# ElijahHyndman/PAPTeam_OpticalFlow

Hardware: AMD Instinct MI355X
Metric: Mpix/s per frame-pair (fixed SOR iters) at 1920x1080; max-abs d(u,v) vs ref (higher is better)
Workload: dtype f64

## Files before the change

papteam_opticalflow_amd/csrc/api.hip:

```cpp
#include <algorithm>
#include <chrono>
#include <cmath>
#include <cstdio>
#include <cstdlib>
#include <cstring>
#include <mutex>
#include <random>
#include <thread>

#include "common.h"
#include "flow_internal.h"

namespace papof {

namespace {
thread_local std::string g_last_error;
}

void set_last_error(const char* what, hipError_t e, const char* file, int line) {
    char buf[512];
    std::snprintf(buf, sizeof buf, "%s failed: %s (%s:%d)", what, hipGetErrorString(e), file, line);
    g_last_error = buf;
}
const char* last_error() { return g_last_error.c_str(); }
void set_last_error_text(const std::string& text) { g_last_error = text; }

static double wall() {
    return std::chrono::duration<double>(std::chrono::steady_clock::now().time_since_epoch()).count();
}

size_t arena_bytes_for(int H, int W, int C, int levels, int n_sor_max, double ratio) {
    const size_t np = (size_t)H * W;
    const int fc = (C == 3) ? 5 : (C == 1 ? 3 : C);
    size_t per_level = 0;
    {
        std::vector<Level> L;
        std::vector<PyrPlan> plan;
        if (levels >= 1 && pyramid_plan(H, W, ratio, levels, L, plan) == PAPOF_OK)
            for (const Level& l : L) per_level += ((size_t)l.w * l.h * fc * sizeof(double) + 256) * 3;
    }
    size_t sor_cells = 0, sor_cells_d = 0;
    skew_capacity(H, W, n_sor_max, sor_cells, sor_cells_d);
    size_t planes = 0;
    planes += (size_t)2 * C * 5;
    if (levels > 8) planes += (size_t)2 * C * levels;
    planes += (size_t)2 * C + 2 * C;
    planes += (size_t)7 * fc;
    planes += 8;
    planes += (size_t)3 * C + C;
    planes += (size_t)3 * fc;
    size_t bytes = planes * np * sizeof(double);
    bytes += 3 * (sor_cells + 2 * kLanes) * 16 + (sor_cells_d + 2 * kLanes) * 16 + 10 * np * sizeof(double);
    bytes += per_level + np * fc * sizeof(double);
    bytes += 8 * (std::min<size_t>(kTinyMaxCells, np) * sizeof(double) + 256);
    bytes += (size_t)64 * 4096;
    return bytes;
}

static size_t sor_scratch_bytes(int H, int W, int n_sor) {
    size_t cells = 0, cells_d = 0;
    skew_capacity(H, W, n_sor, cells, cells_d);
    return 4 * (cells + 128) * 16 + (cells_d + 128) * 16;
}

int ensure_arena(papof_handle* h, size_t bytes) {
    if (bytes <= h->arena.cap) return PAPOF_OK;
    PAPOF_HIP(hipStreamSynchronize(h->stream));
    if (h->arena.base) PAPOF_HIP(hipFree(h->arena.base));
    h->arena.base = nullptr;
    h->arena.cap = 0;
    void* p = nullptr;
    hipError_t e = hipMalloc(&p, bytes);
    if (e != hipSuccess) {
        set_last_error("hipMalloc(arena)", e, __FILE__, __LINE__);
        return PAPOF_ENOMEM;
    }
    h->arena.base = static_cast<char*>(p);
    h->arena.cap = bytes;
    return PAPOF_OK;
}

int check_params(const papof_params& P, int levels) {
    if (levels < 1) return PAPOF_EINVAL;
    if (P.n_inner < 1) return PAPOF_EINVAL;
    if (P.n_outer + 0 < 1 || P.n_sor < 1 || P.n_outer_per_level < 0 || P.n_sor_per_level < 0) return PAPOF_EINVAL;
    if (P.sor_mode < PAPOF_SOR_EXACT || P.sor_mode > PAPOF_SOR_JACOBI) return PAPOF_EINVAL;
    if (!(P.alpha > 0) || !(P.omega > 0)) return PAPOF_EINVAL;
    if (P.interpolation != PAPOF_INTERP_BILINEAR && P.interpolation != PAPOF_INTERP_BICUBIC) return PAPOF_EINVAL;
    if (P.noise_model != PAPOF_NOISE_LAPLACIAN && P.noise_model != PAPOF_NOISE_GMIXTURE) return PAPOF_EINVAL;
    return PAPOF_OK;
}

int pyramid_plan(int H, int W, double ratio, int nlev, std::vector<Level>& L, std::vector<PyrPlan>& plan) {
    if (ratio > 0.98 || ratio < 0.4) ratio = 0.75;
    const double base_sigma = 1 / ratio - 1;
    const int n = (int)(std::log(0.25) / std::log(ratio));
    const double n_sigma = base_sigma * n;
    L.assign(nlev, Level{});
    plan.assign(nlev, PyrPlan{});
    L[0].w = W;
    L[0].h = H;
    for (int i = 1; i < nlev; i++) {
        PyrPlan p;
        if (i <= n) {
            p.src_level = 0;
            p.sigma = base_sigma * i;
            p.fsize = (int)(p.sigma * 3);
            p.rate = std::pow(ratio, i);
        } else {
            p.src_level = i - n;
            p.sigma = n_sigma;
            p.fsize = (int)(n_sigma * 3);
            p.rate = (double)std::pow(ratio, i) * W / L[i - n].w;
        }
        p.sw = L[p.src_level].w;
        p.sh = L[p.src_level].h;
        if (p.fsize > kMaxFsize) return PAPOF_EINVAL;
        L[i].w = (int)((double)p.sw * p.rate);
        L[i].h = (int)((double)p.sh * p.rate);
        if (L[i].w < 1 || L[i].h < 1) return PAPOF_EINVAL;
        plan[i] = p;
    }
    return PAPOF_OK;
}

int smooth_and_resize(papof_handle* h, const double* src, double* dst, double* tmp_a, double* tmp_b, const PyrPlan& p, int C,
                      int dh, int dw) {
    const Taps g = gaussian_taps(p.sigma, p.fsize);
    if (g.fsize == 0 && g.t[0] == 1.0) return resize(h, src, dst, p.sh, p.sw, C, dh, dw, p.rate, p.rate, false, 0.0);
    PAPOF_TRY(filter_hv(h, src, tmp_b, tmp_a, p.sh, p.sw, C, g, g));
    return resize(h, tmp_b, dst, p.sh, p.sw, C, dh, dw, p.rate, p.rate, false, 0.0);
}

int reduce_init(papof_handle* h, const papof_tensor* a, const papof_tensor* b, int pairs_a, int pairs_b, int H, int W,
                const std::vector<Level>& L, const std::vector<PyrPlan>& plan, double ratio, double* X, double* Y, double* T,
                size_t t_planes, double*& out) {
    const size_t np0 = (size_t)H * W;
    const int planes = 2 * (pairs_a + pairs_b), levels = (int)L.size();
    double* const parts[2] = {X, X + (size_t)pairs_a * 2 * np0};
    const papof_tensor* const src[2] = {a, b};
    const int n[2] = {pairs_a, pairs_b};
    for (int i = 0; i < 2; i++) {
        if (n[i] == 0) continue;
        if (src[i])
            PAPOF_TRY(ingest_frames(h, *src[i], nullptr, parts[i], H, W, 2, n[i]));
        else
            PAPOF_HIP(hipMemsetAsync(parts[i], 0, (size_t)n[i] * 2 * np0 * sizeof(double), h->stream));
    }
    PAPOF_TRY(init_sanitize(h, X, (size_t)planes * np0));
    out = X;
    if (levels == 1) return PAPOF_OK;
    std::vector<int> chain;
    for (int i = levels - 1; i > 0; i = plan[i].src_level) chain.insert(chain.begin(), i);
    double s = 1.0;
    for (int i = 1; i < levels; i++) s *= ratio;
    double *cur = X, *other = Y;
    for (const int i : chain) {
        const PyrPlan& p = plan[i];
        const bool last = i == levels - 1;
        const Taps g = gaussian_taps(p.sigma, p.fsize);
        if (g.fsize == 0 && g.t[0] == 1.0) {
            PAPOF_TRY(resize(h, cur, other, p.sh, p.sw, planes, L[i].h, L[i].w, p.rate, p.rate, last, last ? s : 0.0));
            std::swap(cur, other);
            continue;
        }
        const size_t ns = (size_t)p.sw * p.sh;
        const int chunk = filter_hv_needs_tmp(g, g) ? (int)std::min<size_t>((size_t)planes, t_planes * np0 / ns) : planes;
        if (chunk < 1) return PAPOF_EINVAL;
        for (int c0 = 0; c0 < planes; c0 += chunk)
            PAPOF_TRY(filter_hv(h, cur + c0 * ns, other + c0 * ns, T, p.sh, p.sw, std::min(chunk, planes - c0), g, g));
        PAPOF_TRY(resize(h, other, cur, p.sh, p.sw, planes, L[i].h, L[i].w, p.rate, p.rate, last, last ? s : 0.0));
    }
    out = cur;
    return PAPOF_OK;
}

int build_pyramid(papof_handle* h, const std::vector<Level>& L, const std::vector<PyrPlan>& plan, int C, bool second,
                  double* tmp_a, double* tmp_b) {
    for (size_t i = 1; i < L.size(); i++) {
        const PyrPlan& p = plan[i];
        const double* src = second ? L[p.src_level].p2 : L[p.src_level].p1;
        double* dst = second ? L[i].p2 : L[i].p1;
        PAPOF_TRY(smooth_and_resize(h, src, dst, tmp_a, tmp_b, p, C, L[i].h, L[i].w));
    }
    return PAPOF_OK;
}

struct SolveBuffers {
    double *im1s, *tmp, *blend, *imdt, *phi;
    SorPlanes sp;
    SorPlanes sp_tiny{};
    double *bgx = nullptr, *bgy = nullptr, *bgxy = nullptr;
    double *gm = nullptr, *gm_scratch = nullptr;
};

int alloc_solve_buffers(Arena& A, int H, int W, int fc, int mode, int n_sor_cap, SolveBuffers& B) {
    const size_t np = (size_t)H * W;
    B.im1s = A.f64(np * fc);
    B.tmp = A.f64(np * fc);
    B.blend = A.f64(np * fc);
    B.imdt = A.f64(np * fc);
    B.phi = A.f64(np);
    PAPOF_TRY(sor_alloc_planes(A, H, W, mode, n_sor_cap, B.sp));
    if (mode == PAPOF_SOR_EXACT)
        PAPOF_TRY(sor_alloc_tiny_planes(A, std::min<size_t>(kTinyMaxCells, (size_t)H * W), B.sp_tiny));
    return A.overflow ? PAPOF_ENOMEM : PAPOF_OK;
}

int alloc_branch_buffers(papof_handle* h, Arena& A, int H, int W, int fc, int interpolation, int noise_model,
                         SolveBuffers& B) {
    const size_t np = (size_t)H * W;
    if (interpolation == PAPOF_INTERP_BICUBIC) {
        B.bgx = A.f64(np * fc);
        B.bgy = A.f64(np * fc);
        B.bgxy = A.f64(np * fc);
    }
    if (noise_model == PAPOF_NOISE_GMIXTURE) {
        B.gm = A.f64(5 * 8);
        B.gm_scratch = A.f64((size_t)gm_scratch_doubles());
        if (A.overflow || fc > 8) return fc > 8 ? PAPOF_EINVAL : PAPOF_ENOMEM;
        double init[40];
        for (int k = 0; k < fc; k++) {
            init[k] = 0.95;
            init[fc + k] = 0.05;
            init[2 * fc + k] = 0.5;
            init[3 * fc + k] = 0.05 * 0.05;
            init[4 * fc + k] = 0.5 * 0.5;
        }
        PAPOF_HIP(hipMemcpyAsync(B.gm, init, sizeof(double) * 5 * fc, hipMemcpyHostToDevice, h->stream));
        PAPOF_HIP(hipStreamSynchronize(h->stream));
    }
    return A.overflow ? PAPOF_ENOMEM : PAPOF_OK;
}

int bicubic_planes(papof_handle* h, const double* f2, int H, int W, int fc, SolveBuffers& B) {
    PAPOF_TRY(central3_planes(h, f2, B.bgx, B.bgy, B.bgxy, H, W, fc));
    return PAPOF_OK;
}

struct LapGuard {
    bool on = false;
    bool exact = false;
    bool collect = false;
    bool nz_known = false;
    unsigned* flags = nullptr;
    double* lap = nullptr;
    double* scratch = nullptr;
    unsigned epoch = 0;
    int slot = 0;
    std::vector<int> slot_level, slot_channels;
    unsigned* wit(int s) const { return on && collect && s >= 0 && s < kLapMaxSlots ? flags + lap_wit_word(s) : nullptr; }
    unsigned* nz(int level) const { return on && collect && nz_known ? flags + lap_nz_word(level) : nullptr; }
    const double* guard() const { return on && exact ? lap : nullptr; }
    int unknown(const unsigned* host_flags) const {
        if (!on || !collect) return 0;
        if (slot > kLapMaxSlots) return 1;
        int n = 0;
        for (int s = 0; s + 1 < slot; s++)
            for (int c = 0; c < slot_channels[s]; c++) {
                const unsigned w = host_flags[lap_wit_word(s) + c];
                const bool witness = w == epoch || w == (epoch ^ kLapNone);
                const bool all_zero = nz_known && host_flags[lap_nz_word(slot_level[s]) + c] != epoch;
                n += !(witness || all_zero);
                if (!(witness || all_zero) && std::getenv("PAPOF_LAP_TRACE"))
                    std::fprintf(stderr, "[lap guard] no proof: slot %d of %d, level %d, channel %d\n", s, slot, slot_level[s], c);
            }
        return n;
    }
};

int smooth_flow(papof_handle* h, const double* f1, const double* f2, double* warp, double*& u, double*& v, double*& ua,
                double*& va, int H, int W, int fc, double alpha, int n_outer, int n_inner, int n_sor, double omega,
                int mode, SolveBuffers& B, PhaseClock& clk, const double* im1s_ready = nullptr,
                bool final_warp = true, unsigned* prog = nullptr, size_t prog_per_solve = 0, double* out_u = nullptr,
                double* out_v = nullptr, bool fold_warp = false, LapGuard* lg = nullptr, int level = 0) {
    const Taps g = smooth5_taps();
    int solve_idx = 0;
    const bool tiny = mode == PAPOF_SOR_EXACT && B.sp_tiny.phi && sor_tiny_fits(h, H, W, n_sor);
    SorPlanes& SP = tiny ? B.sp_tiny : B.sp;
    const double* im1s = im1s_ready;
    if (!im1s) {
        clk.phase(PAPOF_T_PHASE1_GENERATE);
        PAPOF_TRY(filter_hv(h, f1, B.im1s, B.tmp, H, W, fc, g, g));
        im1s = B.im1s;
    }
    const char* const fused_sw = std::getenv("PAPOF_FUSED_SYSTEM");
    const bool fused_env = !(fused_sw && fused_sw[0] == '0');
    const bool fused_system = fused_env && fold_warp && n_inner == 1 && !B.gm && (fc == 5 || fc == 3) &&
                              !(lg && lg->guard()) && !(lg && lg->on && lap_one_block_level(H, W));
    for (int count = 0; count < n_outer; count++) {
        clk.phase(fused_system ? kTimerFused : (int)PAPOF_T_PHASE1_GENERATE);
        if (fused_system)
            PAPOF_TRY(flow_system(h, f1, f2, u, v, im1s, H, W, fc, alpha, omega, SP,
                                  lg && count > 0 ? lg->wit(lg->slot - 1) : nullptr));
        else if (fold_warp)
            PAPOF_TRY(warp_smooth_blend(h, f1, f2, u, v, im1s, B.blend, B.imdt, H, W, fc,
                                        lg && count > 0 && !B.gm ? lg->wit(lg->slot - 1) : nullptr,
                                        B.phi));
        else
            PAPOF_TRY(smooth_hv_blend(h, warp, im1s, B.blend, B.imdt, H, W, fc));
        for (int hh = 0; hh < n_inner; hh++) {
            const SorPlanes* prev = hh == 0 ? nullptr : &SP;
            if ((count == 0 && !fold_warp) || hh > 0) {
                clk.phase(PAPOF_T_PHASE2_DERIVATIVES);
                PAPOF_TRY(compute_phi(h, u, v, prev, B.phi, H, W));
            }
            if (!fused_system) clk.phase(PAPOF_T_PHASE4_LINEARSYSTEM);
            if (!fused_system)
                PAPOF_TRY(assemble_system(h, B.blend, B.imdt, B.phi, u, v, H, W, fc, alpha, omega, SP, nullptr, nullptr,
                                          prev, nullptr, B.gm, lg ? lg->guard() : nullptr));
            h->sor_mark = [](void* c, int on) {
                static_cast<PhaseClock*>(c)->phase(on ? PAPOF_T_PHASE5_SOR : PAPOF_T_PHASE6_UPDATE);
            };
            h->sor_mark_ctx = &clk;
            h->sor_prog_next = prog ? prog + (size_t)solve_idx * prog_per_solve : nullptr;
            solve_idx++;
            const int rc_solve = sor_solve(h, SP, H, W, alpha, omega, n_sor, mode);
            h->sor_prog_next = nullptr;
            h->sor_mark = nullptr;
            h->sor_mark_ctx = nullptr;
            PAPOF_TRY(rc_solve);
        }
        double* const phi_next = count + 1 < n_outer && !fold_warp ? B.phi : nullptr;
        const bool rewarp = !fold_warp && !B.bgx && (final_warp || count + 1 < n_outer || B.gm);
        const bool wit_later = fold_warp && count + 1 < n_outer;
        const bool wit_small = fold_warp && !wit_later && lap_one_block_level(H, W);
        unsigned* const wit = lg && !B.gm && !B.bgx && !wit_later && !wit_small ? lg->wit(lg->slot) : nullptr;
        if (out_u && out_v && count + 1 == n_outer) {
            PAPOF_TRY(update_warp_phi(h, SP, u, v, out_u, out_v, f1, f2, warp, phi_next, H, W, fc, rewarp, 0, -1, wit));
            u = out_u;
            v = out_v;
        } else {
            PAPOF_TRY(update_warp_phi(h, SP, u, v, ua, va, f1, f2, warp, phi_next, H, W, fc, rewarp, 0, -1, wit));
            std::swap(u, ua);
            std::swap(v, va);
        }
        if (B.bgx)
            PAPOF_TRY(bicubic_warp(h, f1, f2, B.bgx, B.bgy, B.bgxy, u, v, warp, H, W, fc, nullptr, true, true));
        if (lg && lg->on && !B.gm && wit_small && lg->wit(lg->slot))
            PAPOF_TRY(lap_small_check(h, f1, f2, u, v, H, W, fc, lg->wit(lg->slot)));
        if (lg && lg->on && !B.gm) {
            lg->slot_level.push_back(level);
            lg->slot_channels.push_back(fc);
            lg->slot++;
            if (lg->exact) {
                if (B.bgx)
                    PAPOF_TRY(est_laplacian_noise(h, f1, warp, nullptr, nullptr, H, W, fc, lg->lap, lg->scratch));
                else
                    PAPOF_TRY(est_laplacian_noise(h, f1, f2, u, v, H, W, fc, lg->lap, lg->scratch));
            }
        }
        if (B.gm) PAPOF_TRY(est_gaussian_mixture(h, f1, warp, H, W, fc, B.gm, B.gm_scratch));
    }
    clk.phase(-1);
    return PAPOF_OK;
}

int feature_channels(int C) { return C == 3 ? 5 : (C == 1 ? 3 : C); }

struct FrameIn {
    const void* d;
    bool u8;
    bool planar = false;
};
int load_frame(papof_handle* h, const FrameIn& f, double* planar, int H, int W, int C) {
    if (f.planar) {
        PAPOF_HIP(hipMemcpyAsync(planar, f.d, (size_t)H * W * C * sizeof(double), hipMemcpyDeviceToDevice, h->stream));
        return PAPOF_OK;
    }
    if (f.u8) return hwc_u8_to_planar(h, static_cast<const unsigned char*>(f.d), planar, H, W, C);
    return hwc_to_planar(h, static_cast<const double*>(f.d), planar, H, W, C);
}

enum SeqOp { kPair, kSeqPrime, kSeqNext };

bool seq_matches(const papof_handle* h, int H, int W, int C, int levels, double ratio, size_t need) {
    const papof_handle::Seq& q = h->seq;
    return q.valid && q.h == H && q.w == W && q.c == C && q.levels == levels && q.ratio == ratio &&
           q.arena_base == h->arena.base && need <= h->arena.cap;
}

int flow_pass(papof_handle* h, const FrameIn& fa, const FrameIn& fb, SeqOp op, int H, int W, int C, int levels,
              const papof_params& P, double* d_vx, double* d_vy, double* d_warp, double* timing, LapGuard* lg,
              const papof_tensor* init = nullptr) {
    const double t_entry = wall();
    PAPOF_TRY(check_params(P, levels));
    double ratio = P.ratio;
    if (ratio > 0.98 || ratio < 0.4) ratio = 0.75;
    std::vector<Level> L;
    std::vector<PyrPlan> plan;
    PAPOF_TRY(pyramid_plan(H, W, P.ratio, levels, L, plan));
    const int n_sor_max = P.n_sor + (levels - 1) * P.n_sor_per_level;
    const size_t need = arena_bytes_for(H, W, C, levels, n_sor_max, P.ratio);
    if (op == kSeqNext && !seq_matches(h, H, W, C, levels, ratio, need)) {
        g_last_error = "sequence push does not continue the primed sequence (shape, levels, ratio or arena changed)";
        return PAPOF_EINVAL;
    }
    const int slot1 = op == kSeqNext ? h->seq.slot : 0;
    h->seq.valid = false;
    PAPOF_TRY(ensure_arena(h, need));
    Arena& A = h->arena;
    A.off = 0;
    A.overflow = false;
    h->events_used = 0;
    const size_t np0 = (size_t)H * W;
    const int fc = feature_channels(C);
    double tm[PAPOF_N_TIMERS + 1];
    std::memset(tm, 0, sizeof tm);
    const size_t tm_bytes = PAPOF_N_TIMERS * sizeof(double);
    const auto keep_seq = [&](int slot) {
        h->seq.valid = true;
        h->seq.h = H;
        h->seq.w = W;
        h->seq.c = C;
        h->seq.levels = levels;
        h->seq.ratio = ratio;
        h->seq.slot = slot;
        h->seq.arena_base = A.base;
    };
    PhaseClock clk{h, true};
    PhaseClock pclk{h, true};
    PhaseClock total{h, true};
    clk.only_sor = pclk.only_sor = (!h->phase_events && P.phase_timing == 0) || P.phase_timing == 2;
    h->sor_launches = 0;
    h->sor_log.clear();
    clk.stamps = true;
    h->stamps_used = 0;
    h->next_stamp = nullptr;
    h->stamp_stream = h->stream;

    total.phase(PAPOF_T_TOTAL);
    for (int i = 0; i < levels; i++) {
        double* slot[2];
        slot[0] = A.f64((size_t)L[i].w * L[i].h * C);
        slot[1] = A.f64((size_t)L[i].w * L[i].h * C);
        L[i].p1 = slot[slot1];
        L[i].p2 = slot[slot1 ^ 1];
    }
    double* tmp_a = A.f64(np0 * C);
    double* tmp_b = A.f64(np0 * C);
    if (A.overflow) return PAPOF_ENOMEM;
    if (op == kSeqPrime) {
        PAPOF_TRY(load_frame(h, fa, L[0].p1, H, W, C));
        PAPOF_TRY(build_pyramid(h, L, plan, C, false, tmp_a, tmp_b));
        PAPOF_HIP(hipStreamSynchronize(h->stream));
        keep_seq(slot1);
        if (timing) std::memset(timing, 0, tm_bytes);
        return PAPOF_OK;
    }

    std::vector<double*> F1(levels), F2(levels), S1(levels);
    for (int k = 0; k < levels; k++) {
        const size_t n = (size_t)L[k].w * L[k].h * fc;
        F1[k] = A.f64(n);
        F2[k] = A.f64(n);
        S1[k] = A.f64(n);
    }
    double* prep_tmp = A.f64(np0 * fc);
    double* gx = A.f64(np0 * C);
    double* gy = A.f64(np0 * C);
    double* gxy = A.f64(np0 * C);
    double* warp = A.f64(np0 * fc);
    double* u = A.f64(2 * np0);
    double* v = u ? u + np0 : nullptr;
    double* u2 = A.f64(2 * np0);
    double* v2 = u2 ? u2 + np0 : nullptr;
    SolveBuffers B;
    {
        const int rc_alloc = alloc_solve_buffers(A, H, W, fc, P.sor_mode, n_sor_max, B);
        if (rc_alloc != PAPOF_OK || A.overflow) return rc_alloc != PAPOF_OK ? rc_alloc : PAPOF_ENOMEM;
    }
    PAPOF_TRY(alloc_branch_buffers(h, A, H, W, fc, P.interpolation, P.noise_model, B));

    struct LevelCounters {
        size_t prog_off = 0, prog_per = 0;
    };
    std::vector<LevelCounters> LP(levels);
    size_t prog_total = 0;
    const bool exact = P.sor_mode == PAPOF_SOR_EXACT;
    if (exact) {
        for (int k = 0; k < levels; k++) {
            LP[k].prog_per = sor_counters_words(L[k].h, L[k].w, P.n_sor + k * P.n_sor_per_level);
            LP[k].prog_off = prog_total;
            prog_total += LP[k].prog_per * (size_t)((P.n_outer + k * P.n_outer_per_level) * P.n_inner);
        }
        PAPOF_TRY(sor_counters_ensure(h, prog_total));
    }

    const bool overlap = h->overlap_prep && P.phase_timing != 1 && h->prep_stream != nullptr;
    hipStream_t const main_stream = h->stream, prep = overlap ? h->prep_stream : h->stream;
    while (h->sync_events.size() < (size_t)levels + 2) {
        hipEvent_t e;
        PAPOF_HIP(hipEventCreateWithFlags(&e, hipEventDisableTiming));
        h->sync_events.push_back(e);
    }
    struct StreamSwap {
        papof_handle* h;
        hipStream_t saved;
        StreamSwap(papof_handle* hh, hipStream_t s) : h(hh), saved(hh->stream) { h->stream = s; }
        ~StreamSwap() { h->stream = saved; }
    };
    bool from_level0 = true;
    for (int i = 1; i < levels; i++) from_level0 = from_level0 && plan[i].src_level == 0;
    const Taps g5 = smooth5_taps();
    const auto build_level = [&](int i, int second) -> int {
        if (i == 0) return PAPOF_OK;
        const PyrPlan& q = plan[i];
        const double* src = second ? L[q.src_level].p2 : L[q.src_level].p1;
        double* dst = second ? L[i].p2 : L[i].p1;
        return smooth_and_resize(h, src, dst, tmp_a, tmp_b, q, C, L[i].h, L[i].w);
    };
    const auto prepare = [&]() -> int {
        StreamSwap on_prep(h, prep);
        pclk.phase(PAPOF_T_ALLOCATION);
        if (exact && !sor_counters_clear(h, 0, prog_total)) return PAPOF_EDEVICE;
        pclk.phase(PAPOF_T_CONSTRUCTION);
        if (op != kSeqNext) PAPOF_TRY(load_frame(h, fa, L[0].p1, H, W, C));
        PAPOF_TRY(load_frame(h, fb, L[0].p2, H, W, C));
        const int first = op == kSeqNext ? 1 : 0;
        if (!from_level0)
            for (int i = 1; i < levels; i++)
                for (int second = first; second < 2; second++) PAPOF_TRY(build_level(i, second));
        for (int k = levels - 1; k >= 0; k--) {
            if (from_level0) {
                pclk.phase(PAPOF_T_CONSTRUCTION);
                for (int second = first; second < 2; second++) PAPOF_TRY(build_level(k, second));
            }
            pclk.phase(PAPOF_T_ALLOCATION);
            PAPOF_TRY(im2feature(h, L[k].p1, F1[k], L[k].h, L[k].w, C, lg ? lg->nz(k) : nullptr));
            PAPOF_TRY(im2feature(h, L[k].p2, F2[k], L[k].h, L[k].w, C, lg ? lg->nz(k) : nullptr));
            pclk.phase(PAPOF_T_PHASE1_GENERATE);
            PAPOF_TRY(filter_hv(h, F1[k], S1[k], prep_tmp, L[k].h, L[k].w, fc, g5, g5));
            pclk.phase(-1);
            if (overlap) PAPOF_HIP(hipEventRecord(h->sync_events[k], prep));
        }
        pclk.phase(PAPOF_T_POSTPROCESSING);
        PAPOF_TRY(central3_planes(h, L[0].p2, gx, gy, gxy, H, W, C));
        pclk.phase(-1);
        if (overlap) PAPOF_HIP(hipEventRecord(h->sync_events[levels], prep));
        return PAPOF_OK;
    };
    papof_handle::HostIO& io = h->hostio;
    const bool hostio = io.active && overlap && h->copy_stream && h->copy_events.size() >= 8;
    const auto prepare_hostio = [&]() -> int {
        StreamSwap on_prep(h, prep);
        hipStream_t const cs = h->copy_stream;
        pclk.phase(PAPOF_T_ALLOCATION);
        if (exact && !sor_counters_clear(h, 0, prog_total)) return PAPOF_EDEVICE;
        if (io.im1) {
            PAPOF_HIP(hipMemcpyAsync(const_cast<void*>(fa.d), io.im1, io.nb_in, hipMemcpyHostToDevice, cs));
            PAPOF_HIP(hipEventRecord(h->copy_events[0], cs));
            PAPOF_HIP(hipStreamWaitEvent(prep, h->copy_events[0], 0));
        }
        pclk.phase(PAPOF_T_CONSTRUCTION);
        if (op != kSeqNext) {
            PAPOF_TRY(load_frame(h, fa, L[0].p1, H, W, C));
            for (int i = 1; i < levels; i++) PAPOF_TRY(build_level(i, 0));
        }
        for (int k = levels - 1; k >= 0; k--) {
            pclk.phase(PAPOF_T_ALLOCATION);
            PAPOF_TRY(im2feature(h, L[k].p1, F1[k], L[k].h, L[k].w, C, lg ? lg->nz(k) : nullptr));
            pclk.phase(PAPOF_T_PHASE1_GENERATE);
            PAPOF_TRY(filter_hv(h, F1[k], S1[k], prep_tmp, L[k].h, L[k].w, fc, g5, g5));
        }
        pclk.phase(-1);
        if (io.im2) {
            PAPOF_HIP(hipMemcpyAsync(const_cast<void*>(fb.d), io.im2, io.nb_in, hipMemcpyHostToDevice, cs));
            PAPOF_HIP(hipEventRecord(h->copy_events[1], cs));
            PAPOF_HIP(hipStreamWaitEvent(prep, h->copy_events[1], 0));
        }
        pclk.phase(PAPOF_T_CONSTRUCTION);
        PAPOF_TRY(load_frame(h, fb, L[0].p2, H, W, C));
        if (!from_level0)
            for (int i = 1; i < levels; i++) PAPOF_TRY(build_level(i, 1));
        for (int k = levels - 1; k >= 0; k--) {
            if (from_level0) {
                pclk.phase(PAPOF_T_CONSTRUCTION);
                PAPOF_TRY(build_level(k, 1));
            }
            pclk.phase(PAPOF_T_ALLOCATION);
            PAPOF_TRY(im2feature(h, L[k].p2, F2[k], L[k].h, L[k].w, C, lg ? lg->nz(k) : nullptr));
            pclk.phase(-1);
            PAPOF_HIP(hipEventRecord(h->sync_events[k], prep));
        }
        pclk.phase(PAPOF_T_POSTPROCESSING);
        PAPOF_TRY(central3_planes(h, L[0].p2, gx, gy, gxy, H, W, C));
        pclk.phase(-1);
        PAPOF_HIP(hipEventRecord(h->sync_events[levels], prep));
        return PAPOF_OK;
    };
    if (io.active && !hostio) {
        if (io.im1) PAPOF_HIP(hipMemcpyAsync(const_cast<void*>(fa.d), io.im1, io.nb_in, hipMemcpyHostToDevice, main_stream));
        if (io.im2) PAPOF_HIP(hipMemcpyAsync(const_cast<void*>(fb.d), io.im2, io.nb_in, hipMemcpyHostToDevice, main_stream));
    }
    if (overlap) {
        PAPOF_HIP(hipEventRecord(h->sync_events[levels + 1], main_stream));
        PAPOF_HIP(hipStreamWaitEvent(prep, h->sync_events[levels + 1], 0));
    }
    {
        const int rc = hostio ? prepare_hostio() : prepare();
        if (rc != PAPOF_OK) {
            if (overlap) hipStreamSynchronize(prep);
            return rc;
        }
    }

    int pw = 0, ph = 0;
    const auto solve_levels = [&]() -> int {
        if (lg && lg->guard())
            PAPOF_HIP(hipMemcpyAsync(lg->lap, h->lap_init_dev, 8 * sizeof(double), hipMemcpyDeviceToDevice, main_stream));
        for (int k = levels - 1; k >= 0; k--) {
            const int lw = L[k].w, lh = L[k].h;
            const size_t np = (size_t)lw * lh;
            clk.phase(-1);
            if (overlap) PAPOF_HIP(hipStreamWaitEvent(main_stream, h->sync_events[k], 0));
            clk.phase(PAPOF_T_ALLOCATION);
            const double *f1 = F1[k], *f2 = F2[k];
            const int n_sor_k = P.n_sor + k * P.n_sor_per_level, n_outer_k = P.n_outer + k * P.n_outer_per_level;
            unsigned* prog_k = nullptr;
            if (exact) prog_k = h->sync_words + 32 + LP[k].prog_off;
            const bool tiny_k = exact && sor_tiny_fits(h, lh, lw, n_sor_k);
            if (!tiny_k) PAPOF_TRY(sor_bind(h, B.sp, lh, lw, n_sor_k));
            double* const out_u = k == 0 ? d_vx : nullptr;
            double* const out_v = k == 0 ? d_vy : nullptr;
            const bool fold_warp = !B.bgx && !B.gm;
            if (k == levels - 1 && init) {
                double* r = nullptr;
                PAPOF_TRY(reduce_init(h, init, nullptr, 1, 0, H, W, L, plan, ratio, u, u2, warp, (size_t)fc, r));
                if (r != u) std::swap(u, u2);
                v = u + np;
                v2 = u2 + np;
                if (B.bgx) {
                    PAPOF_TRY(bicubic_planes(h, f2, lh, lw, fc, B));
                    PAPOF_TRY(bicubic_warp(h, f1, f2, B.bgx, B.bgy, B.bgxy, u, v, warp, lh, lw, fc, nullptr, true, false));
                } else if (!fold_warp) {
                    PAPOF_TRY(warp_bilinear(h, f1, f2, u, v, warp, lh, lw, fc));
                }
            } else if (k == levels - 1) {
                v = u + np;
                v2 = u2 + np;
                PAPOF_HIP(hipMemsetAsync(u, 0, 2 * np * sizeof(double), h->stream));
                if (!fold_warp)
                    PAPOF_HIP(hipMemcpyAsync(warp, f2, np * fc * sizeof(double), hipMemcpyDeviceToDevice, h->stream));
                if (B.bgx) PAPOF_TRY(bicubic_planes(h, f2, lh, lw, fc, B));
            } else {
                const double xr = (double)lw / pw, yr = (double)lh / ph, inv = 1 / ratio;
                PAPOF_TRY(resize(h, u, u2, ph, pw, 2, lh, lw, xr, yr, true, inv));
                std::swap(u, u2);
                v = u + np;
                v2 = u2 + np;
                if (B.bgx) {
                    PAPOF_TRY(bicubic_planes(h, f2, lh, lw, fc, B));
                    PAPOF_TRY(bicubic_warp(h, f1, f2, B.bgx, B.bgy, B.bgxy, u, v, warp, lh, lw, fc, nullptr, true, false));
                } else if (!fold_warp) {
                    PAPOF_TRY(warp_bilinear(h, f1, f2, u, v, warp, lh, lw, fc));
                }
            }
            if (!tiny_k) PAPOF_TRY(sor_reset_planes(h, B.sp));
            PAPOF_TRY(smooth_flow(h, f1, f2, warp, u, v, u2, v2, lh, lw, fc, P.alpha, n_outer_k, P.n_inner, n_sor_k, P.omega,
                                  P.sor_mode, B, clk, S1[k], false, prog_k, exact ? LP[k].prog_per : 0, out_u, out_v,
                                  fold_warp, lg, k));
            pw = lw;
            ph = lh;
        }
        clk.phase(-1);
        if (overlap) PAPOF_HIP(hipStreamWaitEvent(main_stream, h->sync_events[levels], 0));
        clk.phase(PAPOF_T_POSTPROCESSING);
        if (hostio && io.early_out && u == d_vx && v == d_vy) {
            hipStream_t const cs = h->copy_stream;
            PAPOF_HIP(hipEventRecord(h->copy_events[2], main_stream));
            PAPOF_HIP(hipStreamWaitEvent(cs, h->copy_events[2], 0));
            PAPOF_HIP(hipMemcpyAsync(io.vx, d_vx, io.nb_flow, hipMemcpyDeviceToHost, cs));
            PAPOF_HIP(hipMemcpyAsync(io.vy, d_vy, io.nb_flow, hipMemcpyDeviceToHost, cs));
            constexpr int kChunks = 4;
            for (int q = 0; q < kChunks; q++) {
                const Rect rc{0, (int)((long long)H * q / kChunks), W, (int)((long long)H * (q + 1) / kChunks)};
                if (rc.empty()) continue;
                PAPOF_TRY(bicubic_warp(h, L[0].p1, L[0].p2, gx, gy, gxy, u, v, d_warp, H, W, C, &rc));
                PAPOF_HIP(hipEventRecord(h->copy_events[3 + q], main_stream));
                PAPOF_HIP(hipStreamWaitEvent(cs, h->copy_events[3 + q], 0));
                const size_t off = (size_t)rc.y0 * W * C, cnt = (size_t)rc.h() * W * C;
                PAPOF_HIP(hipMemcpyAsync(io.warp + off, d_warp + off, cnt * sizeof(double), hipMemcpyDeviceToHost, cs));
            }
            io.out_issued = true;
            return PAPOF_OK;
        }
        PAPOF_TRY(bicubic_warp(h, L[0].p1, L[0].p2, gx, gy, gxy, u, v, d_warp, H, W, C));
        if (u != d_vx) PAPOF_HIP(hipMemcpyAsync(d_vx, u, np0 * sizeof(double), hipMemcpyDeviceToDevice, h->stream));
        if (v != d_vy) PAPOF_HIP(hipMemcpyAsync(d_vy, v, np0 * sizeof(double), hipMemcpyDeviceToDevice, h->stream));
        return PAPOF_OK;
    };
    const int rc_main = solve_levels();
    if (rc_main != PAPOF_OK) {
        hipStreamSynchronize(main_stream);
        if (overlap) hipStreamSynchronize(prep);
        return rc_main;
    }
    clk.phase(-1);
    PAPOF_TRY(stamp_only(h));
    total.phase(-1);
    h->stamps_fetched = 0;
    {
        const bool flags = lg && lg->on && lg->collect;
        const size_t first = flags ? lap_wit_word(std::min(lg->slot, kLapMaxSlots) - 1) : kLapFlagWords;
        const size_t bytes = (kLapFlagWords - first) * sizeof(unsigned) + (size_t)h->stamps_used * sizeof(unsigned long long);
        if (bytes > 0)
            PAPOF_HIP(hipMemcpyAsync(h->lap_flags_host + first, h->lap_flags_dev + first, bytes, hipMemcpyDeviceToHost, h->stream));
        h->stamps_fetched = h->stamps_used;
    }
    const double t_enqueued = wall();
    PAPOF_HIP(hipStreamSynchronize(h->stream));
    h->host_enqueue_sec = t_enqueued - t_entry;
    h->host_wait_sec = wall() - t_enqueued;
    h->next_stamp = nullptr;
    if (P.sor_mode == PAPOF_SOR_EXACT) PAPOF_TRY(sor_check(h));
    if (clk.err != PAPOF_OK || pclk.err != PAPOF_OK || total.err != PAPOF_OK) return PAPOF_EDEVICE;
    clk.collect(tm);
    pclk.collect(tm);
    total.collect(tm);
    if (clk.sor_span_sec.size() == h->sor_log.size())
        for (size_t i = 0; i < h->sor_log.size(); i++) h->sor_log[i].sec = clk.sor_span_sec[i];
    {
        constexpr double kPsiShare = 0.3;
        const double fused = tm[PAPOF_T_PHASE4_LINEARSYSTEM];
        tm[PAPOF_T_PHASE3_PSIDATA] += kPsiShare * fused;
        tm[PAPOF_T_PHASE4_LINEARSYSTEM] = fused - kPsiShare * fused;
    }
    {
        constexpr double kPhiShare = 0.04;
        const double fused = tm[PAPOF_T_PHASE1_GENERATE];
        tm[PAPOF_T_PHASE2_DERIVATIVES] += kPhiShare * fused;
        tm[PAPOF_T_PHASE1_GENERATE] = fused - kPhiShare * fused;
    }
    {
        const double f = tm[kTimerFused];
        tm[PAPOF_T_PHASE1_GENERATE] += 0.51 * f;
        tm[PAPOF_T_PHASE2_DERIVATIVES] += 0.02 * f;
        tm[PAPOF_T_PHASE3_PSIDATA] += 0.14 * f;
        tm[PAPOF_T_PHASE4_LINEARSYSTEM] += f - 0.51 * f - 0.02 * f - 0.14 * f;
    }
    if (timing) std::memcpy(timing, tm, tm_bytes);
    if (op == kSeqNext) keep_seq(slot1 ^ 1);
    return PAPOF_OK;
}

int flow_device(papof_handle* h, const FrameIn& fa, const FrameIn& fb, SeqOp op, int H, int W, int C, int levels,
                const papof_params& P, double* d_vx, double* d_vy, double* d_warp, double* timing,
                const papof_tensor* init = nullptr) {
    LapGuard lg;
    const int fc = feature_channels(C);
    lg.on = h->lap_guard && op != kSeqPrime && P.noise_model == PAPOF_NOISE_LAPLACIAN && fc <= 8 && levels >= 1 &&
            h->lap_flags_dev != nullptr;
    if (!lg.on) return flow_pass(h, fa, fb, op, H, W, C, levels, P, d_vx, d_vy, d_warp, timing, nullptr, init);
    lg.flags = h->lap_flags_dev;
    lg.lap = h->lap_dev;
    lg.scratch = h->lap_scratch_dev;
    lg.nz_known = (C == 1 || C == 3) && (size_t)levels * 8 <= (size_t)kLapNzWords;
    const bool always_exact = P.interpolation == PAPOF_INTERP_BICUBIC;
    lg.collect = !always_exact;
    lg.exact = always_exact || h->lap_exact;
    const papof_handle::Seq seq0 = h->seq;
    double first_pass_total = 0.0;
    for (int pass = 0; pass < 2; pass++) {
        if (++h->lap_epoch >= kLapNone) {
            PAPOF_HIP(hipMemsetAsync(h->lap_flags_dev, 0, kLapFlagWords * sizeof(unsigned), h->stream));
            h->lap_epoch = 1u;
        }
        lg.epoch = h->lap_epoch;
        lg.slot = 0;
        lg.slot_level.clear();
        lg.slot_channels.clear();
        PAPOF_TRY(flow_pass(h, fa, fb, op, H, W, C, levels, P, d_vx, d_vy, d_warp, timing, &lg, init));
        if (pass == 1 && timing) timing[PAPOF_T_TOTAL] += first_pass_total;
        if (!lg.collect) return PAPOF_OK;
        const int unknown = lg.unknown(h->lap_flags_host);
        if (lg.exact) {
            if (pass == 0) h->lap_exact_calls++;
            h->lap_exact = unknown > 0;
            return PAPOF_OK;
        }
        if (unknown == 0) return PAPOF_OK;
        h->lap_reruns++;
        lg.exact = true;
        if (timing) first_pass_total = timing[PAPOF_T_TOTAL];
        if (h->copy_stream) PAPOF_HIP(hipStreamSynchronize(h->copy_stream));
        h->seq = seq0;
        h->hostio.im1 = nullptr;
        h->hostio.im2 = nullptr;
    }
    return PAPOF_OK;
}

int flow_device_planar(papof_handle* h, const double* f1, const double* f2, int H, int W, int C, int levels,
                       const papof_params& P, double* d_vx, double* d_vy, double* d_warp, double* timing,
                       const papof_tensor* init) {
    FrameIn a{f1, false}, b{f2, false};
    a.planar = b.planar = true;
    return flow_device(h, a, b, kPair, H, W, C, levels, P, d_vx, d_vy, d_warp, timing, init);
}

}

using namespace papof;

extern "C" {

int papof_version(void) { return PAPOF_VERSION; }

void papof_default_params(papof_params* p) {
    if (!p) return;
    p->alpha = 0.012;
    p->ratio = 0.75;
    p->n_outer = 7;
    p->n_outer_per_level = 1;
    p->n_inner = 1;
    p->n_sor = 30;
    p->n_sor_per_level = 3;
    p->omega = 1.8;
    p->sor_mode = PAPOF_SOR_EXACT;
    p->phase_timing = 0;
    p->interpolation = PAPOF_INTERP_BILINEAR;
    p->noise_model = PAPOF_NOISE_LAPLACIAN;
}

const char* papof_strerror(int code) {
    switch (code) {
        case PAPOF_OK: return "ok";
        case PAPOF_EINVAL: return "invalid argument";
        case PAPOF_ENODEVICE: return "no usable gfx950 device";
        case PAPOF_ENOMEM: return "out of memory";
        case PAPOF_EDEVICE: return "HIP runtime error";
        case PAPOF_ETIMEOUT: return "device-side wait timed out";
    }
    return "unknown error";
}

const char* papof_last_error(void) { return last_error(); }

const char* papof_timing_key(int i) {
    static const char* keys[PAPOF_N_TIMERS] = {"Allocation",         "Construction",        "Phase1_Generate",
// ... 43 lines not shown
        set_last_error("hipStreamCreate", e, __FILE__, __LINE__);
        papof_destroy(h);
        return PAPOF_ENODEVICE;
    }
    if (const char* cs = std::getenv("PAPOF_OVERLAP")) h->overlap_prep = std::atoi(cs) != 0;
    if (const char* cs = std::getenv("PAPOF_PHASE_EVENTS")) h->phase_events = std::atoi(cs) != 0;
    if (const char* cs = std::getenv("PAPOF_SOR_DEPTH")) h->sor_depth = std::max(4, std::atoi(cs));
    if (const char* cs = std::getenv("PAPOF_SOR_FUSE")) h->sor_fuse = std::max(1, std::atoi(cs));
    if (const char* cs = std::getenv("PAPOF_SOR_TINY")) h->sor_tiny = std::atoi(cs) != 0;
    if (const char* cs = std::getenv("PAPOF_SOR_GROUP")) h->sor_group = std::max(1, std::atoi(cs));
    if (const char* cs = std::getenv("PAPOF_SOR_XCD")) h->sor_xcd_affine = std::atoi(cs);
    if (const char* cs = std::getenv("PAPOF_RB_DEPTH")) h->rb_depth = std::max(0, std::atoi(cs));
    if (const char* cs = std::getenv("PAPOF_RB_SHAPE")) h->rb_shape = std::max(0, std::atoi(cs));
    if (const char* cs = std::getenv("PAPOF_SOR_RESIDENT")) h->sor_resident = std::max(0, std::atoi(cs));
    if (const char* cs = std::getenv("PAPOF_SOR_DEAD")) h->sor_skip_dead = std::atoi(cs) != 0 ? 1 : 0;
    int rc = sor_probe_dpp(h);
    if (rc != PAPOF_OK) {
        papof_destroy(h);
        return rc;
    }
    {
        const size_t flag_bytes = kLapFlagWords * sizeof(unsigned), bytes = flag_bytes + 4096 * sizeof(unsigned long long);
        const size_t lap_doubles = 16 + (size_t)lap_scratch_doubles();
        std::vector<double> init(8, 0.02);
        if (hipMalloc((void**)&h->lap_flags_dev, bytes) == hipSuccess &&
            hipHostMalloc((void**)&h->lap_flags_host, bytes, hipHostMallocDefault) == hipSuccess &&
            hipMalloc((void**)&h->lap_dev, lap_doubles * sizeof(double)) == hipSuccess &&
            hipMemset(h->lap_flags_dev, 0, flag_bytes) == hipSuccess &&
            hipMemcpy(h->lap_dev + 8, init.data(), 8 * sizeof(double), hipMemcpyHostToDevice) == hipSuccess) {
            h->stamps_dev = reinterpret_cast<unsigned long long*>(h->lap_flags_dev + kLapFlagWords);
            h->stamps = reinterpret_cast<unsigned long long*>(h->lap_flags_host + kLapFlagWords);
            h->stamps_cap = 4096;
            h->lap_init_dev = h->lap_dev + 8;
            h->lap_scratch_dev = h->lap_dev + 16;
            std::memset(h->lap_flags_host, 0, bytes);
        } else {
            g_last_error = "cannot allocate the flag / stamp block of the handle";
            papof_destroy(h);
            return PAPOF_ENOMEM;
        }
        const char* lgv = std::getenv("PAPOF_LAP_GUARD");
        h->lap_guard = !(lgv && lgv[0] == '0');
    }
    *out = h;
    return PAPOF_OK;
}

void papof_destroy(papof_handle* h) {
    if (!h) return;
    hipSetDevice(h->device);
    hipStreamSynchronize(h->stream);
    if (h->prep_stream) hipStreamSynchronize(h->prep_stream);
    for (hipEvent_t e : h->events) hipEventDestroy(e);
    for (hipEvent_t e : h->sync_events) hipEventDestroy(e);
    if (h->prep_stream) hipStreamDestroy(h->prep_stream);
    if (h->copy_stream) {
        hipStreamSynchronize(h->copy_stream);
        hipStreamDestroy(h->copy_stream);
    }
    for (hipEvent_t e : h->copy_events) hipEventDestroy(e);
    if (h->arena.base) hipFree(h->arena.base);
    if (h->sync_words) hipFree(h->sync_words);
    if (h->stage_dev) hipFree(h->stage_dev);
    if (h->tensor_scratch) hipFree(h->tensor_scratch);
    if (h->init_flag_dev) hipFree(h->init_flag_dev);
    if (h->entry_event) hipEventDestroy(h->entry_event);
    if (h->lap_flags_host) hipHostFree(h->lap_flags_host);
    if (h->lap_flags_dev) hipFree(h->lap_flags_dev);
    if (h->lap_dev) hipFree(h->lap_dev);
    hipStreamDestroy(h->stream);
    delete h;
}

void* papof_stream(papof_handle* h) { return h ? (void*)h->stream : nullptr; }

int papof_host_alloc(size_t bytes, void** out) {
    if (!out) return PAPOF_EINVAL;
    *out = nullptr;
    hipError_t e = hipHostMalloc(out, bytes ? bytes : 1, hipHostMallocDefault);
    if (e != hipSuccess) {
        set_last_error("hipHostMalloc", e, __FILE__, __LINE__);
        *out = nullptr;
        return e == hipErrorNoDevice || e == hipErrorInvalidDevice ? PAPOF_ENODEVICE : PAPOF_ENOMEM;
    }
    return PAPOF_OK;
}

int papof_host_free(void* p) {
    if (!p) return PAPOF_OK;
    PAPOF_HIP(hipHostFree(p));
    return PAPOF_OK;
}

int papof_dev_alloc(papof_handle* h, size_t bytes, void** out) {
    if (!h || !out) return PAPOF_EINVAL;
    PAPOF_HIP(hipSetDevice(h->device));
    hipError_t e = hipMalloc(out, bytes ? bytes : 1);
    if (e != hipSuccess) {
        set_last_error("hipMalloc", e, __FILE__, __LINE__);
        return PAPOF_ENOMEM;
    }
    return PAPOF_OK;
}

int papof_dev_free(papof_handle* h, void* p) {
    if (!h) return PAPOF_EINVAL;
    PAPOF_HIP(hipSetDevice(h->device));
    PAPOF_HIP(hipFree(p));
    return PAPOF_OK;
}

int papof_dev_upload(papof_handle* h, void* dst, const void* src, size_t bytes) {
    if (!h || !dst || !src) return PAPOF_EINVAL;
    PAPOF_HIP(hipSetDevice(h->device));
    PAPOF_HIP(hipMemcpyAsync(dst, src, bytes, hipMemcpyHostToDevice, h->stream));
    PAPOF_HIP(hipStreamSynchronize(h->stream));
    return PAPOF_OK;
}

int papof_dev_download(papof_handle* h, void* dst, const void* src, size_t bytes) {
    if (!h || !dst || !src) return PAPOF_EINVAL;
    PAPOF_HIP(hipSetDevice(h->device));
    PAPOF_HIP(hipMemcpyAsync(dst, src, bytes, hipMemcpyDeviceToHost, h->stream));
    PAPOF_HIP(hipStreamSynchronize(h->stream));
    return PAPOF_OK;
}

namespace {

int device_call(papof_handle* h, const FrameIn& fa, const FrameIn& fb, SeqOp op, int height, int width, int c,
                int pyramid_levels, const papof_params* params, double* d_vx, double* d_vy, double* d_warpI2,
                double* timing_sec) {
    if (!h || height < 1 || width < 1 || c < 1) return PAPOF_EINVAL;
    if (op != kSeqNext && !fa.d) return PAPOF_EINVAL;
    if (op != kSeqPrime && (!fb.d || !d_vx || !d_vy || !d_warpI2)) return PAPOF_EINVAL;
    papof_params P;
    if (params)
        P = *params;
    else
        papof_default_params(&P);
    PAPOF_HIP(hipSetDevice(h->device));
    return flow_device(h, fa, fb, op, height, width, c, pyramid_levels, P, d_vx, d_vy, d_warpI2, timing_sec);
}

SeqOp seq_op_for(papof_handle* h, int H, int W, int C, int levels, const papof_params* params) {
    papof_params P;
    if (params)
        P = *params;
    else
        papof_default_params(&P);
    double ratio = P.ratio;
    if (ratio > 0.98 || ratio < 0.4) ratio = 0.75;
    if (levels < 1) return kSeqPrime;
    const size_t need = arena_bytes_for(H, W, C, levels, P.n_sor + (levels - 1) * P.n_sor_per_level, P.ratio);
    return seq_matches(h, H, W, C, levels, ratio, need) ? kSeqNext : kSeqPrime;
}

}

int papof_flow_device(papof_handle* h, const double* d_im1, const double* d_im2, int height, int width, int c,
                      int pyramid_levels, const papof_params* params, double* d_vx, double* d_vy, double* d_warpI2,
                      double timing_sec[PAPOF_N_TIMERS]) {
    return device_call(h, FrameIn{d_im1, false}, FrameIn{d_im2, false}, kPair, height, width, c, pyramid_levels,
                       params, d_vx, d_vy, d_warpI2, timing_sec);
}

int papof_flow_device_u8(papof_handle* h, const unsigned char* d_im1, const unsigned char* d_im2, int height,
                         int width, int c, int pyramid_levels, const papof_params* params, double* d_vx,
                         double* d_vy, double* d_warpI2, double timing_sec[PAPOF_N_TIMERS]) {
    return device_call(h, FrameIn{d_im1, true}, FrameIn{d_im2, true}, kPair, height, width, c, pyramid_levels, params,
                       d_vx, d_vy, d_warpI2, timing_sec);
}

int papof_set_stream_overlap(papof_handle* h, int on) {
    if (!h) return PAPOF_EINVAL;
    h->overlap_prep = on != 0;
    return PAPOF_OK;
}

int papof_seq_reset(papof_handle* h) {
    if (!h) return PAPOF_EINVAL;
    h->seq.valid = false;
    return PAPOF_OK;
}

int papof_seq_push_device(papof_handle* h, const void* d_frame, int is_u8, int height, int width, int c,
                          int pyramid_levels, const papof_params* params, double* d_vx, double* d_vy,
                          double* d_warpI2, double timing_sec[PAPOF_N_TIMERS], int* have_flow) {
    if (!h || !d_frame || !have_flow) return PAPOF_EINVAL;
    *have_flow = 0;
    const SeqOp op = seq_op_for(h, height, width, c, pyramid_levels, params);
    const FrameIn f{d_frame, is_u8 != 0};
    PAPOF_TRY(device_call(h, f, f, op, height, width, c, pyramid_levels, params, d_vx, d_vy, d_warpI2, timing_sec));
    *have_flow = op == kSeqNext ? 1 : 0;
    return PAPOF_OK;
}

namespace {

int ensure_host_stage(papof_handle* h, size_t dev_bytes) {
    if (dev_bytes > h->stage_dev_bytes) {
        PAPOF_HIP(hipStreamSynchronize(h->stream));
        if (h->stage_dev) PAPOF_HIP(hipFree(h->stage_dev));
        h->stage_dev = nullptr;
        h->stage_dev_bytes = 0;
        hipError_t e = hipMalloc((void**)&h->stage_dev, dev_bytes);
        if (e != hipSuccess) {
            set_last_error("hipMalloc(stage)", e, __FILE__, __LINE__);
            return PAPOF_ENOMEM;
        }
        h->stage_dev_bytes = dev_bytes;
    }
    return PAPOF_OK;
}

int flow_host(papof_handle* h, const void* im1, const void* im2, bool u8, SeqOp op, int height, int width, int c,
              int pyramid_levels, const papof_params* params, double* vx, double* vy, double* warpI2,
              double* timing_sec) {
    if (!h || height < 1 || width < 1 || c < 1 || pyramid_levels < 1) return PAPOF_EINVAL;
    if (op != kSeqNext && !im1) return PAPOF_EINVAL;
    if (op != kSeqPrime && (!im2 || !vx || !vy || !warpI2)) return PAPOF_EINVAL;
    const double t0 = wall();
    PAPOF_HIP(hipSetDevice(h->device));
    const size_t np = (size_t)height * width, nb_img = np * c * sizeof(double), nb_flow = np * sizeof(double);
    const size_t nb_in = np * c * (u8 ? 1 : sizeof(double));
    PAPOF_TRY(ensure_host_stage(h, 3 * nb_img + 2 * nb_flow));
    double* d1 = h->stage_dev;
    double* d2 = d1 + np * c;
    double* dw = d2 + np * c;
    double* dx = dw + np * c;
    double* dy = dx + np;
    double tm[PAPOF_N_TIMERS];
    std::memset(tm, 0, sizeof tm);
    bool use_io = op != kSeqPrime && h->overlap_prep && h->prep_stream;
    if (use_io && !h->copy_stream) {
        if (hipStreamCreateWithFlags(&h->copy_stream, hipStreamNonBlocking) != hipSuccess) h->copy_stream = nullptr;
        while (h->copy_stream && h->copy_events.size() < 8) {
            hipEvent_t e = nullptr;
            if (hipEventCreateWithFlags(&e, hipEventDisableTiming) != hipSuccess) break;
            h->copy_events.push_back(e);
        }
    }
    use_io = use_io && h->copy_stream && h->copy_events.size() >= 8;
    if (use_io) {
        papof_params Pq;
        if (params)
            Pq = *params;
        else
            papof_default_params(&Pq);
        use_io = Pq.phase_timing != 1;
    }
    if (use_io) {
        h->hostio = papof_handle::HostIO{};
        h->hostio.active = true;
        h->hostio.im1 = op != kSeqNext ? im1 : nullptr;
        h->hostio.im2 = im2;
        h->hostio.nb_in = nb_in;
    } else {
        if (op != kSeqNext) PAPOF_HIP(hipMemcpyAsync(d1, im1, nb_in, hipMemcpyHostToDevice, h->stream));
        if (op != kSeqPrime) PAPOF_HIP(hipMemcpyAsync(d2, im2, nb_in, hipMemcpyHostToDevice, h->stream));
    }
    const auto is_pinned = [](const void* p) {
        hipPointerAttribute_t a;
        if (hipPointerGetAttributes(&a, p) != hipSuccess) {
            (void)hipGetLastError();
            return false;
        }
        return a.type == hipMemoryTypeHost;
    };
    std::thread prefault;
    const bool out_pinned = op != kSeqPrime && is_pinned(warpI2) && is_pinned(vx) && is_pinned(vy);
    if (use_io) {
        h->hostio.vx = vx;
        h->hostio.vy = vy;
        h->hostio.warp = warpI2;
        h->hostio.nb_flow = nb_flow;
        h->hostio.nb_img = nb_img;
        h->hostio.early_out = out_pinned;
    }
    if (op != kSeqPrime && np * sizeof(double) >= (size_t(1) << 20) && !out_pinned)
        prefault = std::thread([=] {
            const auto touch = [](double* p, size_t bytes) {
                volatile char* q = reinterpret_cast<volatile char*>(p);
                for (size_t o = 0; o < bytes; o += 4096) q[o] = 0;
                if (bytes) q[bytes - 1] = 0;
            };
            touch(warpI2, nb_img);
            touch(vx, nb_flow);
            touch(vy, nb_flow);
        });
    const int rc_dev = device_call(h, FrameIn{d1, u8}, FrameIn{d2, u8}, op, height, width, c, pyramid_levels, params, dx,
                                   dy, dw, tm);
    const bool out_issued = use_io && h->hostio.out_issued;
    h->hostio.active = false;
    if (use_io && h->copy_stream && hipStreamSynchronize(h->copy_stream) != hipSuccess && rc_dev == PAPOF_OK) {
        if (prefault.joinable()) prefault.join();
        return PAPOF_EDEVICE;
    }
    if (prefault.joinable()) prefault.join();
    PAPOF_TRY(rc_dev);
    if (out_issued) {
        if (timing_sec) {
            tm[PAPOF_T_TOTAL] = wall() - t0;
            std::memcpy(timing_sec, tm, sizeof tm);
        }
        return PAPOF_OK;
    }
// ... 732 lines not shown
```

papteam_opticalflow_amd/csrc/common.h:

```cpp
#pragma once
#include <cstdlib>

#include <hip/hip_runtime.h>

#include <algorithm>
#include <cmath>
#include <cstddef>
#include <cstdint>
#include <initializer_list>
#include <string>
#include <vector>

#include "../../include/papof.h"

namespace papof {

constexpr int kLanes = 64;
constexpr int kMaxFsize = 8;

struct Rect {
    int x0, y0, x1, y1;
    __host__ __device__ bool empty() const { return x1 <= x0 || y1 <= y0; }
    __host__ __device__ int w() const { return x1 - x0; }
    __host__ __device__ int h() const { return y1 - y0; }
// ... 17 lines not shown
    const double *a = im1 + o, *b = im2 + o;
    im1 = back ? b : a;
    im2 = back ? a : b;
    return back ? o + bk.fr : o;
}

struct Taps {
    double t[2 * kMaxFsize + 1];
    int fsize;
};

void set_last_error(const char* what, hipError_t e, const char* file, int line);
const char* last_error();

#define PAPOF_HIP(expr)                                              \
    do {                                                             \
        hipError_t _e = (expr);                                      \
        if (_e != hipSuccess) {                                      \
            ::papof::set_last_error(#expr, _e, __FILE__, __LINE__);  \
            return PAPOF_EDEVICE;                                    \
        }                                                            \
    } while (0)

#define PAPOF_TRY(expr)              \
    do {                             \
        int _rc = (expr);            \
        if (_rc != PAPOF_OK) return _rc; \
    } while (0)

struct Arena {
    char* base = nullptr;
    size_t cap = 0, off = 0, peak = 0;
    bool overflow = false;
    void* alloc(size_t bytes) {
        size_t o = (off + 255) & ~size_t(255);
        if (o + bytes > cap) {
            overflow = true;
            return nullptr;
        }
        off = o + bytes;
        if (off > peak) peak = off;
        return base + o;
    }
    double* f64(size_t n) { return static_cast<double*>(alloc(n * sizeof(double))); }
    size_t mark() const { return off; }
    void release(size_t m) { off = m; }
};

constexpr int kLapNzWords = 32 * 8, kLapMaxSlots = 1024;
constexpr size_t kLapFlagWords = (size_t)kLapMaxSlots * 8 + kLapNzWords;
inline size_t lap_wit_word(int slot) { return (size_t)(kLapMaxSlots - 1 - slot) * 8; }
inline size_t lap_nz_word(int level) { return (size_t)kLapMaxSlots * 8 + (size_t)level * 8; }
constexpr unsigned kLapNone = 0x80000000u;
constexpr int kSorMaxDepth = 32;
constexpr int kBandRows = kLanes - 2;

struct SkewDims {
    int nb;
    int ns;
    int rt, qt;
    int hp;
    int npos;
    size_t n;
    int n_sor;
    int npos_d;
    size_t nd;
    int group;
    int dpar;
    size_t nh;
    int fuse;
    int band_rows, koff, poff;
};
constexpr int kFusedRows = kLanes - 3;
inline SkewDims skew_dims(int h, int w, int n_sor, int group = 1, int fuse = 1) {
    SkewDims d;
    d.fuse = (fuse == 2 && group <= 1) ? 2 : 1;
    d.group = d.fuse == 2 ? 1 : (group < 1 ? 1 : group);
    d.ns = w + kLanes - 1;
    d.n_sor = n_sor;
    d.npos_d = d.ns + 2 * kSorMaxDepth + 72;
    if (d.fuse == 2) {
        const int last = (n_sor + 1) / 2 - 1;
        d.band_rows = kFusedRows;
        d.nb = (h + 2 * last + 1 + kFusedRows - 1) / kFusedRows;
        d.qt = n_sor + 3;
        d.rt = (d.qt + 7) / 8 * 8;
        d.hp = (d.rt + kFusedRows * d.nb + 4 + 7) / 8 * 8;
        d.npos = d.qt + d.ns + 2 * kSorMaxDepth + 2 + kFusedRows * (d.nb - 1) + 2;
        d.dpar = last & 1;
        d.koff = 2 * last + 1;
        d.poff = 3;
        d.nh = 0;
    } else {
        d.band_rows = kBandRows;
        d.nb = (h + n_sor - 1 + kBandRows - 1) / kBandRows;
        d.qt = n_sor + 1;
        d.rt = (d.qt + 7) / 8 * 8;
        d.hp = (d.rt + kBandRows * d.nb + 2 + 7) / 8 * 8;
        d.npos = d.qt + d.ns + 2 * kSorMaxDepth + 2 + kBandRows * (d.nb - 1) + 2;
        d.dpar = d.group == 1 ? ((n_sor - 1) & 1) : (((n_sor + d.group - 1) / d.group - 1) & 1);
        d.koff = n_sor - 1;
        d.poff = 1;
        d.nh = d.group == 1 ? 0 : (size_t)n_sor * d.nb * d.npos_d;
    }
    d.n = (size_t)d.npos * d.hp;
    d.nd = (size_t)2 * d.npos_d * d.nb * kLanes;
    return d;
}
inline void skew_capacity(int h, int w, int n_sor, size_t& cells, size_t& cells_d) {
    const SkewDims a = skew_dims(h, w, n_sor, 2), b = skew_dims(h, w, n_sor, 1, 2);
    cells = a.n > b.n ? a.n : b.n;
    cells_d = (a.nd + a.nh) > (b.nd + b.nh) ? (a.nd + a.nh) : (b.nd + b.nh);
}

struct SorPlanes {
    double *phi, *xy, *a1, *a2, *b1, *b2;
    double *du, *dv;
    double *du2, *dv2;
    bool skew;
    SkewDims sd;
    size_t cap_cells, cap_cells_d;
};

}

struct papof_handle {
    int device = 0;
    hipStream_t stream = nullptr;
    papof::Arena arena;
    unsigned* sync_words = nullptr;
    size_t sync_cap = 0;
    std::vector<hipEvent_t> events;
    size_t events_used = 0;
    int cu_count = 0;
    double* stage_dev = nullptr;
    size_t stage_dev_bytes = 0;
    double* tensor_scratch = nullptr;
    size_t tensor_scratch_bytes = 0;
    hipEvent_t entry_event = nullptr;
    unsigned* init_flag_dev = nullptr;
    bool use_dpp = false;
    int sor_depth = 0;
    unsigned long long* sor_dbg = nullptr;
    void (*sor_mark)(void*, int) = nullptr;
    void* sor_mark_ctx = nullptr;
    int sor_fuse = 0;
    int sor_group = 0;
    int rb_depth = 0;
    int rb_shape = 0;
    int sor_tiny = 1;
    int sor_resident = 0;
    int sor_skip_dead = 1;
    unsigned* sor_prog_next = nullptr;
    int sor_launches = 0;
    struct SorSolveLog {
        int H, W, n_sor, kind, depth, launches;
        double sec;
    };
    std::vector<SorSolveLog> sor_log;
    hipStream_t prep_stream = nullptr;
    unsigned* lap_flags_dev = nullptr;
    unsigned* lap_flags_host = nullptr;
    double* lap_dev = nullptr;
    double* lap_init_dev = nullptr;
    double* lap_scratch_dev = nullptr;
    bool lap_guard = true;
    bool lap_exact = false;
    unsigned lap_epoch = 0;
    int lap_reruns = 0, lap_exact_calls = 0;
    double host_enqueue_sec = 0.0, host_wait_sec = 0.0;
    struct HostIO {
        bool active = false;
        const void *im1 = nullptr, *im2 = nullptr;
        size_t nb_in = 0;
        double *vx = nullptr, *vy = nullptr, *warp = nullptr;
        size_t nb_flow = 0, nb_img = 0;
        bool early_out = false;
        bool out_issued = false;
    } hostio;
    hipStream_t copy_stream = nullptr;
    std::vector<hipEvent_t> copy_events;
    std::vector<hipEvent_t> sync_events;
    bool overlap_prep = true;
    unsigned long long* stamps_dev = nullptr;
    unsigned long long* stamps = nullptr;
    int stamps_cap = 0, stamps_used = 0, stamps_fetched = 0;
    unsigned long long* next_stamp = nullptr;
    hipStream_t stamp_stream = nullptr;
    bool phase_events = true;
    int sor_xcd_affine = 1;
    struct Seq {
        bool valid = false;
        int h = 0, w = 0, c = 0, levels = 0, slot = 0;
        double ratio = 0;
        const char* arena_base = nullptr;
    } seq;
};

namespace papof {

inline unsigned long long* take_stamp(papof_handle* h) {
    if (h->stamp_stream && h->stream != h->stamp_stream) return nullptr;
    unsigned long long* s = h->next_stamp;
    h->next_stamp = nullptr;
    return s;
}
int stamp_only(papof_handle* h);

inline bool described(const papof_tensor* t, std::initializer_list<int> dtypes, std::initializer_list<int> axes, bool positive) {
    if (!t || !t->data || std::find(dtypes.begin(), dtypes.end(), t->dtype) == dtypes.end()) return false;
    for (int i : axes)
        if (t->stride[i] < 0 || (positive && t->stride[i] == 0)) return false;
    return true;
}
inline bool valid_alphas(double a1, double a2) { return std::isfinite(a1) && std::isfinite(a2) && a1 >= 0 && a2 >= 0; }
inline long long dtype_bytes(int dtype) { return dtype == PAPOF_DTYPE_U8 ? 1 : dtype == PAPOF_DTYPE_F32 ? 4 : 8; }

int hwc_to_planar(papof_handle* h, const double* hwc, double* planar, int H, int W, int C, int frames = 1);
int hwc_u8_to_planar(papof_handle* h, const unsigned char* hwc, double* planar, int H, int W, int C, int frames = 1);
int planar_to_hwc(papof_handle* h, const double* planar, double* hwc, int H, int W, int C);
int ingest_frames(papof_handle* h, const papof_tensor& a, const papof_tensor* b, double* planar, int H, int W, int C,
                  int frames);
int emit_outputs(papof_handle* h, const double* src, const papof_tensor& dst, bool comp_major, int H, int W, int K, int pairs);
int init_check(papof_handle* h, const papof_tensor& t, int pairs, int H, int W, unsigned* flag);
int init_sanitize(papof_handle* h, double* planar, size_t n);
int fb_check(papof_handle* h, hipStream_t st, const papof_tensor& fw, const papof_tensor& bw, const papof_tensor& mask,
             int pairs, int H, int W, double a1, double a2);
int filter_h(papof_handle* h, const double* src, double* dst, int H, int W, int planes, const Taps& f,
             const Rect* rc = nullptr);
int filter_v(papof_handle* h, const double* src, double* dst, int H, int W, int planes, const Taps& f,
             const Rect* rc = nullptr);
int filter_hv(papof_handle* h, const double* src, double* dst, double* tmp, int H, int W, int planes, const Taps& fh,
              const Taps& fv);
bool filter_hv_needs_tmp(const Taps& fh, const Taps& fv);
int resize(papof_handle* h, const double* src, double* dst, int sh, int sw, int planes, int dh, int dw, double xr,
           double yr, bool use_post, double post, const Rect* rc = nullptr);
int im2feature(papof_handle* h, const double* im, double* feat, int H, int W, int C, unsigned* nz = nullptr, int frames = 1,
               size_t nz_stride = 0);
int central3_planes(papof_handle* h, const double* src, double* gx, double* gy, double* gxy, int H, int W, int planes);
int warp_bilinear(papof_handle* h, const double* im1, const double* im2, const double* vx, const double* vy,
                  double* out, int H, int W, int planes, const Rect* rc = nullptr);
int smooth_v_blend(papof_handle* h, const double* tmp, const double* im1s, double* blend, double* imdt, int H,
                   int W, int planes, const Rect* rc = nullptr);
int smooth_hv_blend(papof_handle* h, const double* warp, const double* im1s, double* blend, double* imdt, int H,
                    int W, int planes, int row0 = 0, int row1 = -1);
int warp_smooth_blend(papof_handle* h, const double* im1, const double* im2, const double* u, const double* v,
                      const double* im1s, double* blend, double* imdt, int H, int W, int planes, unsigned* wit = nullptr,
                      double* phi_out = nullptr);
int compute_phi(papof_handle* h, const double* u, const double* v, const SorPlanes* prev, double* phi, int H, int W,
                const Rect* rc = nullptr);
int assemble_system(papof_handle* h, const double* blend, const double* imdt, const double* phi, const double* u,
                    const double* v, int H, int W, int planes, double alpha, double omega, const SorPlanes& out,
                    double* opt_imdx2, double* opt_imdy2, const SorPlanes* prev, const Rect* rc = nullptr,
                    const double* gm = nullptr, const double* lap = nullptr);
int flow_system(papof_handle* h, const double* im1, const double* im2, const double* u, const double* v, const double* im1s,
                int H, int W, int planes, double alpha, double omega, const SorPlanes& out, unsigned* wit = nullptr,
                int row0 = 0, int row1 = -1,
                int batch = 1, const BatchK* bk = nullptr);
int lap_scratch_doubles();
int lap_rows_check(papof_handle* h, const double* im1, const double* im2, const double* u, const double* v, int H, int W,
                   int C, int r0, int r1, unsigned* wit, unsigned* val, unsigned mark);
bool lap_one_block_level(int H, int W);
int lap_small_check(papof_handle* h, const double* im1, const double* im2, const double* u, const double* v, int H, int W,
                    int C, unsigned* wit, int batch = 1, const BatchK* bk = nullptr);
int est_laplacian_noise(papof_handle* h, const double* im1, const double* im2, const double* u, const double* v, int H,
                        int W, int C, double* lap, double* scratch);
int gm_scratch_doubles();
int est_gaussian_mixture(papof_handle* h, const double* im1, const double* im2, int H, int W, int C, double* gm,
                         double* scratch);
int laplacian(papof_handle* h, const double* in, const double* weight, double* out, int H, int W);
int update_and_warp(papof_handle* h, const SorPlanes& sp, double* u, double* v, const double* im1,
                    const double* im2, double* warp, int H, int W, int planes, bool do_warp = true);
int bicubic_warp(papof_handle* h, const double* im1, const double* im2, const double* gx, const double* gy,
                 const double* gxy, const double* vx, const double* vy, double* out_hwc, int H, int W, int C,
                 const Rect* rc = nullptr, bool planar_out = false, bool clamp = true, int batch = 1, const BatchK* bk = nullptr);
int flow_quantize16(papof_handle* h, const double* vx, const double* vy, unsigned short* q, size_t n);
int flow_dequantize16(papof_handle* h, const unsigned short* q, double* vx, double* vy, size_t n);
int flow_to_bgr(papof_handle* h, const double* vx, const double* vy, size_t n, double* partial, unsigned char* bgr);
int update_warp_phi(papof_handle* h, const SorPlanes& sp, const double* u, const double* v, double* u_out, double* v_out,
                    const double* im1, const double* im2, double* warp, double* phi_out, int H, int W, int planes,
                    bool do_warp = true, int row0 = 0, int row1 = -1, unsigned* wit = nullptr, int batch = 1,
                    const BatchK* bk = nullptr);
int update_flow(papof_handle* h, const SorPlanes& sp, double* u, double* v, int H, int W, const Rect& r);
int sor_prep(papof_handle* h, const double* phi, const double* imdxy, const double* imdx2, const double* imdy2,
             const double* rhs1, const double* rhs2, int H, int W, double alpha, double omega, const SorPlanes& out);
int sor_unpack(papof_handle* h, const SorPlanes& sp, double* du, double* dv, int H, int W);
Taps gaussian_taps(double sigma, int fsize);
Taps smooth5_taps();
Taps deriv5_taps();
Taps central3_taps();

struct SorBatch {
    int n;
    size_t coef, d, prog, tiny;
};
int sor_solve(papof_handle* h, const SorPlanes& sp, int H, int W, double alpha, double omega, int n_sor, int mode,
              const SorBatch* bt = nullptr);
int sor_blocked_depth(const papof_handle* h, int mode, int H, int W);
int sor_blocked_launch(papof_handle* h, const SorPlanes& sp, int H, int W, double alpha, double omega, int mode, int g,
                       int hs0, const Rect& out, const double* su, const double* sv, double* du, double* dv);
int sor_plan(const papof_handle* h, int H, int W, int n_sor, int mode, int* launches, int* depth);
int sor_check(papof_handle* h);
bool sor_strips_supported(const papof_handle* h, const SorPlanes& sp, int n_sor);
int sor_strips_begin(papof_handle* h, const SorPlanes& sp, int n_sor, int n_solves);
struct SorSplit {
    double* peer_du;
    unsigned* peer_prog;
    bool top_cut, bot_cut;
};
int sor_solve_bands(papof_handle* h, const SorPlanes& sp, int H, int W, double alpha, double omega, int n_sor,
                    unsigned* prog, int b0, int b1, const SorSplit* split = nullptr);
int sor_bind_plain(papof_handle* h, SorPlanes& sp, int H, int W, int n_sor);
constexpr size_t kTinyMaxCells = 8192;
bool sor_tiny_fits(const papof_handle* h, int H, int W, int n_sor);
bool sor_tiny_shape(int H, int W, int* cells_per_tile, int* waves);
int sor_alloc_tiny_planes(Arena& A, size_t cells, SorPlanes& sp);
size_t sor_counters_words(int H, int W, int n_sor);
int sor_counters_ensure(papof_handle* h, size_t words);
unsigned* sor_counters_clear(papof_handle* h, size_t offset_words, size_t words);
int sor_alloc_planes(Arena& A, int H, int W, int mode, int n_sor_cap, SorPlanes& sp);
int sor_bind(papof_handle* h, SorPlanes& sp, int H, int W, int n_sor);
int sor_group_size(const papof_handle* h, int H, int W, int n_sor);
int sor_reset_planes(papof_handle* h, const SorPlanes& sp);
int sor_reset_planes_batch(papof_handle* h, const SorPlanes& sp, int batch, size_t stride);
int sor_probe_dpp(papof_handle* h);

}
```

papteam_opticalflow_amd/csrc/flow_internal.h:

```cpp
#pragma once

#include <string>
#include <utility>
#include <vector>

#include "common.h"

namespace papof {

void set_last_error_text(const std::string& text);

constexpr int kTimerFused = PAPOF_N_TIMERS;
struct PhaseClock {
    papof_handle* h;
    bool on;
    std::vector<std::pair<int, std::pair<size_t, size_t>>> spans;
    size_t open = 0;
    int open_idx = -1;
    int err = PAPOF_OK;
    bool only_sor = false;
    bool stamps = false;
    std::vector<std::pair<int, int>> marks;
    std::vector<double> sor_span_sec;
    std::vector<int> sor_owner;
    size_t new_event() {
        if (h->events_used == h->events.size()) {
            hipEvent_t e;
            if (hipEventCreate(&e) != hipSuccess) {
                err = PAPOF_EDEVICE;
                return 0;
            }
            h->events.push_back(e);
        }
        hipEventRecord(h->events[h->events_used], h->stream);
        return h->events_used++;
    }
    void phase(int idx) {
        if (!on) return;
        if (stamps) {
            if (open_idx == PAPOF_T_PHASE5_SOR) {
                const size_t e = new_event();
                spans.push_back({PAPOF_T_PHASE5_SOR, {open, e}});
            }
            if (idx == PAPOF_T_PHASE5_SOR) {
                open = new_event();
                sor_owner.push_back(marks.empty() ? PAPOF_T_PHASE4_LINEARSYSTEM : marks.back().second);
            }
            const bool sor_edge = idx == PAPOF_T_PHASE5_SOR;
            open_idx = idx;
            if (only_sor || !h->stamps_dev || sor_edge) return;
            if (h->next_stamp && !marks.empty()) {
                marks.back().second = idx;
            } else if (h->stamps_used < h->stamps_cap) {
                const int slot = h->stamps_used++;
                h->next_stamp = h->stamps_dev + slot;
                marks.push_back({slot, idx});
            }
            return;
        }
        if (only_sor && idx != PAPOF_T_PHASE5_SOR && idx != PAPOF_T_TOTAL) {
            if (open_idx < 0) return;
            idx = -1;
        }
        const size_t e = new_event();
        if (open_idx >= 0) spans.push_back({open_idx, {open, e}});
        open = e;
        open_idx = idx;
    }
    void collect(double* t) {
        if (!on) return;
        for (auto& s : spans) {
            float ms = 0;
            if (hipEventElapsedTime(&ms, h->events[s.second.first], h->events[s.second.second]) == hipSuccess)
                t[s.first] += ms * 1e-3;
            if (s.first == PAPOF_T_PHASE5_SOR) sor_span_sec.push_back(ms * 1e-3);
        }
        for (size_t i = 0; i + 1 < marks.size(); i++) {
            const int idx = marks[i].second;
            if (marks[i + 1].first >= h->stamps_fetched) break;
            const unsigned long long a = h->stamps[marks[i].first], b = h->stamps[marks[i + 1].first];
            if (idx >= 0 && idx != PAPOF_T_PHASE5_SOR && b >= a) t[idx] += (double)(b - a) * 1e-8;
        }
        if (stamps && !marks.empty()) {
            for (size_t i = 0; i < sor_span_sec.size() && i < sor_owner.size(); i++)
                if (sor_owner[i] >= 0) t[sor_owner[i]] -= sor_span_sec[i];
            for (int own : {(int)PAPOF_T_PHASE4_LINEARSYSTEM, kTimerFused})
                if (t[own] < 0.0) t[own] = 0.0;
        }
    }
};

struct Level {
    int w, h;
    double *p1, *p2;
};


struct PyrPlan {
    int sw, sh, src_level, fsize;
    double sigma, rate;
};


size_t arena_bytes_for(int H, int W, int C, int levels, int n_sor_max, double ratio);
int ensure_arena(papof_handle* h, size_t bytes);
int check_params(const papof_params& P, int levels);
int pyramid_plan(int H, int W, double ratio, int nlev, std::vector<Level>& L, std::vector<PyrPlan>& plan);
int build_pyramid(papof_handle* h, const std::vector<Level>& L, const std::vector<PyrPlan>& plan, int C, bool second,
                  double* tmp_a, double* tmp_b);
int smooth_and_resize(papof_handle* h, const double* src, double* dst, double* tmp_a, double* tmp_b, const PyrPlan& p, int C,
                      int dh, int dw);
int feature_channels(int C);
int flow_batch_host(papof_handle* h, int n_pairs, int sequence, const void* const* frames, bool u8, int H, int W, int C, int levels,
                    const papof_params* params, double* const* vx, double* const* vy, double* const* warpI2, double* timing_sec);
int flow_device_planar(papof_handle* h, const double* f1, const double* f2, int H, int W, int C, int levels,
                       const papof_params& P, double* d_vx, double* d_vy, double* d_warp, double* timing,
                       const papof_tensor* init = nullptr);
int reduce_init(papof_handle* h, const papof_tensor* a, const papof_tensor* b, int pairs_a, int pairs_b, int H, int W,
                const std::vector<Level>& L, const std::vector<PyrPlan>& plan, double ratio, double* X, double* Y, double* T,
                size_t t_planes, double*& out);

}
```

papteam_opticalflow_amd/csrc/kernels.hip:

```cpp
#include "common.h"
#include "sampler.h"

#include <cmath>

namespace papof {

namespace {

constexpr int BX = 64, BY = 4;

inline dim3 grid2d(int W, int H, int planes = 1) { return dim3((W + BX - 1) / BX, (H + BY - 1) / BY, planes); }
inline Rect region(const Rect* rc, int W, int H) { return rc ? *rc : Rect{0, 0, W, H}; }
inline dim3 grid2d(const Rect& r, int planes = 1) { return grid2d(r.x1 - r.x0, r.y1 - r.y0, planes); }

__device__ __forceinline__ void stamp_now(unsigned long long* s) {
    if (s && (blockIdx.x | blockIdx.y | blockIdx.z | threadIdx.x | threadIdx.y) == 0u) *s = __builtin_amdgcn_s_memrealtime();
}
__global__ void k_stamp(unsigned long long* s) { stamp_now(s); }

__device__ __forceinline__ int clampi(int x, int n) {
    x = x < 0 ? 0 : x;
    return x > n - 1 ? n - 1 : x;
}

// ... 184 lines not shown
        const int r = c / (BX + 2 * F), cc = c - r * (BX + 2 * F);
        raw[r][cc] = plane[(size_t)clampi(i0 + r - F, H) * W + clampi(j0 + cc - F, W)];
    }
    __syncthreads();
    for (int r = threadIdx.y; r < kHvsRows + 2 * F; r += BY) {
        double acc = 0.0;
#pragma unroll
        for (int l = -F; l <= F; l++) acc += raw[r][threadIdx.x + F + l] * fh.t[l + F];
        hs[r][threadIdx.x] = acc;
    }
    __syncthreads();
    const int j = j0 + threadIdx.x;
    if (j >= W) return;
    for (int r = threadIdx.y; r < kHvsRows; r += BY) {
        const int i = i0 + r;
        if (i >= H) break;
        double acc = 0.0;
#pragma unroll
        for (int l = -F; l <= F; l++) acc += hs[r + l + F][threadIdx.x] * fv.t[l + F];
        dst[blockIdx.z * np + (size_t)i * W + j] = acc;
    }
}

struct BilinearTaps {
    int o[4];
    double s[4];
};

__device__ __forceinline__ BilinearTaps bilinear_taps(int W, int H, double x, double y) {
    BilinearTaps b;
    const int xx = (int)x, yy = (int)y;
    double dx = x - xx, dy = y - yy;
    dx = dx > 1 ? 1.0 : dx;
    dx = dx < 0 ? 0.0 : dx;
    dy = dy > 1 ? 1.0 : dy;
    dy = dy < 0 ? 0.0 : dy;
#pragma unroll
    for (int m = 0; m <= 1; m++)
#pragma unroll
        for (int n = 0; n <= 1; n++) {
            const int u = clampi(xx + m, W), v = clampi(yy + n, H);
            b.o[m * 2 + n] = v * W + u;
            b.s[m * 2 + n] = fabs((double)(1 - m) - dx) * fabs((double)(1 - n) - dy);
        }
    return b;
}

__device__ __forceinline__ double bilinear_apply(const double* __restrict__ p, const BilinearTaps& b) {
    double acc = 0.0;
#pragma unroll
    for (int t = 0; t < 4; t++) acc += p[b.o[t]] * b.s[t];
    return acc;
}

__global__ void k_resize(const double* __restrict__ src, double* __restrict__ dst, int sh, int sw, int dh, int dw,
                         double xr, double yr, int use_post, double post, Rect rc, unsigned long long* stamp) {
    stamp_now(stamp);
    int tbx, tby;
    if (!xcd_tile((rc.x1 - rc.x0 + BX - 1) / BX, (rc.y1 - rc.y0 + BY - 1) / BY, tbx, tby)) return;
    const int j = rc.x0 + tbx * BX + threadIdx.x, i = rc.y0 + tby * BY + threadIdx.y;
    if (j >= rc.x1 || i >= rc.y1) return;
    const double x = (double)(j + 1) / xr - 1;
    const double y = (double)(i + 1) / yr - 1;
    const BilinearTaps b = bilinear_taps(sw, sh, x, y);
    double r = bilinear_apply(src + blockIdx.z * (size_t)sh * sw, b);
    if (use_post) r *= post;
    dst[blockIdx.z * (size_t)dh * dw + (size_t)i * dw + j] = r;
}

template <int C>
__device__ __forceinline__ double gray_at(const double* __restrict__ im, size_t np, size_t o) {
    if (C == 3) return im[o] * .299 + im[np + o] * .587 + im[2 * np + o] * .114;
    return im[o];
}

template <int C>
__global__ void k_im2feature(const double* __restrict__ im, double* __restrict__ feat, int H, int W, Taps d) {
    const int j = blockIdx.x * BX + threadIdx.x, i = blockIdx.y * BY + threadIdx.y;
    if (j >= W || i >= H) return;
    const size_t np = (size_t)H * W, o = (size_t)i * W + j;
    double gx = 0.0, gy = 0.0;
#pragma unroll
    for (int l = -2; l <= 2; l++) gx += gray_at<C>(im, np, (size_t)i * W + clampi(j + l, W)) * d.t[l + 2];
#pragma unroll
    for (int l = -2; l <= 2; l++) gy += gray_at<C>(im, np, (size_t)clampi(i + l, H) * W + j) * d.t[l + 2];
    feat[o] = gray_at<C>(im, np, o);
    feat[np + o] = gx;
    feat[2 * np + o] = gy;
    if (C == 3) {
        feat[3 * np + o] = im[np + o] - im[o];
        feat[4 * np + o] = im[np + o] - im[2 * np + o];
    }
}

#ifndef PAPOF_V_FEATROWS
#define PAPOF_V_FEATROWS 16
#endif
constexpr int kFeatRows = PAPOF_V_FEATROWS;
template <int C, bool BATCH = false>
__global__ __launch_bounds__(256) void k_im2feature_tiled(const double* __restrict__ im, double* __restrict__ feat, int H,
                                                          int W, Taps d, unsigned* __restrict__ nz, unsigned mark,
                                                          size_t b_im, size_t b_feat, size_t b_nz) {
    __shared__ double g[kFeatRows + 4][BX + 4];
    int tx, ty;
    if (!xcd_tile((W + BX - 1) / BX, (H + kFeatRows - 1) / kFeatRows, tx, ty)) return;
    const int j0 = tx * BX, i0 = ty * kFeatRows;
    const size_t np = (size_t)H * W;
    if (BATCH) {
        im += blockIdx.y * b_im;
        feat += blockIdx.y * b_feat;
        if (nz != nullptr) nz += blockIdx.y * b_nz;
    }
    for (int c = threadIdx.y * BX + threadIdx.x; c < (kFeatRows + 4) * (BX + 4); c += BX * BY) {
        const int r = c / (BX + 4), cc = c - r * (BX + 4);
        g[r][cc] = gray_at<C>(im, np, (size_t)clampi(i0 + r - 2, H) * W + clampi(j0 + cc - 2, W));
    }
    __syncthreads();
    const int j = j0 + threadIdx.x;
    bool any[5] = {false, false, false, false, false};
    if (j < W) {
        for (int r = threadIdx.y; r < kFeatRows; r += BY) {
            const int i = i0 + r;
            if (i >= H) break;
            const size_t o = (size_t)i * W + j;
            double gx = 0.0, gy = 0.0;
#pragma unroll
            for (int l = -2; l <= 2; l++) gx += g[r + 2][threadIdx.x + 2 + l] * d.t[l + 2];
#pragma unroll
            for (int l = -2; l <= 2; l++) gy += g[r + 2 + l][threadIdx.x + 2] * d.t[l + 2];
            const double f0 = g[r + 2][threadIdx.x + 2];
            feat[o] = f0;
            feat[np + o] = gx;
            feat[2 * np + o] = gy;
            any[0] |= f0 != 0.0;
            any[1] |= gx != 0.0;
            any[2] |= gy != 0.0;
            if (C == 3) {
                const double gg = im[np + o];
                const double f3 = gg - im[o], f4 = gg - im[2 * np + o];
                feat[3 * np + o] = f3;
                feat[4 * np + o] = f4;
                any[3] |= f3 != 0.0;
                any[4] |= f4 != 0.0;
            }
        }
    }
    if (nz != nullptr) {
#pragma unroll
        for (int k = 0; k < (C == 3 ? 5 : 3); k++)
            if (__ballot(any[k]) != 0ull && threadIdx.x == 0) nz[k] = mark;
    }
}

__global__ void k_central3_all(const double* __restrict__ src, double* __restrict__ gx, double* __restrict__ gy,
                               double* __restrict__ gxy, int H, int W, Taps c3) {
    int tbx, tby;
    if (!xcd_tile((W + BX - 1) / BX, (H + BY - 1) / BY, tbx, tby)) return;
    const int j = tbx * BX + threadIdx.x, i = tby * BY + threadIdx.y;
    if (j >= W || i >= H) return;
    const size_t np = (size_t)H * W;
    const double* p = src + blockIdx.z * np;
    const auto hrow = [&](int ii) {
        const double* row = p + (size_t)ii * W;
        double acc = 0.0;
#pragma unroll
        for (int l = -1; l <= 1; l++) acc += row[clampi(j + l, W)] * c3.t[l + 1];
        return acc;
    };
    const double hx[3] = {hrow(clampi(i - 1, H)), hrow(i), hrow(clampi(i + 1, H))};
    double vy = 0.0, vxy = 0.0;
#pragma unroll
    for (int l = -1; l <= 1; l++) vy += p[(size_t)clampi(i + l, H) * W + j] * c3.t[l + 1];
#pragma unroll
    for (int l = -1; l <= 1; l++) vxy += hx[l + 1] * c3.t[l + 1];
    const size_t o = blockIdx.z * np + (size_t)i * W + j;
    gx[o] = hx[1];
    gy[o] = vy;
    gxy[o] = vxy;
}

__device__ __forceinline__ void warp_pixel(const double* __restrict__ im1, const double* __restrict__ im2,
                                           double* __restrict__ out, double fx, double fy, int i, int j, int H,
                                           int W, int planes) {
    const size_t np = (size_t)H * W, o = (size_t)i * W + j;
    const double y = i + fy;
    const double x = j + fx;
    if (x < 0 || x > W - 1 || y < 0 || y > H - 1) {
        for (int k = 0; k < planes; k++) out[k * np + o] = im1[k * np + o];
        return;
    }
    const BilinearTaps b = bilinear_taps(W, H, x, y);
    for (int k = 0; k < planes; k++) out[k * np + o] = bilinear_apply(im2 + k * np, b);
}

__global__ void k_warp(const double* __restrict__ im1, const double* __restrict__ im2, const double* __restrict__ vx,
                       const double* __restrict__ vy, double* __restrict__ out, int H, int W, int planes, Rect rc,
                       unsigned long long* stamp) {
    stamp_now(stamp);
    const int j = rc.x0 + blockIdx.x * BX + threadIdx.x, i = rc.y0 + blockIdx.y * BY + threadIdx.y;
    if (j >= rc.x1 || i >= rc.y1) return;
    const size_t o = (size_t)i * W + j;
    warp_pixel(im1, im2, out, vx[o], vy[o], i, j, H, W, planes);
}

__global__ void k_smooth_v_blend(const double* __restrict__ tmp, const double* __restrict__ im1s,
                                 double* __restrict__ blend, double* __restrict__ imdt, int H, int W, Taps g, Rect rc) {
    const int j = rc.x0 + blockIdx.x * BX + threadIdx.x, i = rc.y0 + blockIdx.y * BY + threadIdx.y;
    if (j >= rc.x1 || i >= rc.y1) return;
    const size_t np = (size_t)H * W, o = blockIdx.z * np + (size_t)i * W + j;
    const double* p = tmp + blockIdx.z * np + j;
    double s2 = 0.0;
#pragma unroll
    for (int l = -2; l <= 2; l++) s2 += p[(size_t)clampi(i + l, H) * W] * g.t[l + 2];
    const double s1 = im1s[o];
    double t = s1;
    t *= 0.4;
    t += s2 * 0.6;
    blend[o] = t;
    imdt[o] = s2 - s1;
}

constexpr int kFuseRows = 16;
__global__ __launch_bounds__(256) void k_smooth_hv_blend(const double* __restrict__ warp,
                                                         const double* __restrict__ im1s,
                                                         double* __restrict__ blend, double* __restrict__ imdt, int H,
                                                         int W, Taps g, unsigned long long* stamp, int row0, int row1) {
    __shared__ double hs[kFuseRows + 4][BX];
    stamp_now(stamp);
    const int j = blockIdx.x * BX + threadIdx.x, i0 = row0 + blockIdx.y * kFuseRows;
    const size_t np = (size_t)H * W;
    const double* src = warp + blockIdx.z * np;
    if (j < W) {
        for (int r = threadIdx.y; r < kFuseRows + 4; r += BY) {
            const double* row = src + (size_t)clampi(i0 + r - 2, H) * W;
            double acc = 0.0;
#pragma unroll
            for (int l = -2; l <= 2; l++) acc += row[clampi(j + l, W)] * g.t[l + 2];
            hs[r][threadIdx.x] = acc;
        }
    }
    __syncthreads();
    if (j >= W) return;
    for (int r = threadIdx.y; r < kFuseRows; r += BY) {
        const int i = i0 + r;
        if (i >= row1) break;
        const size_t o = blockIdx.z * np + (size_t)i * W + j;
        double s2 = 0.0;
#pragma unroll
        for (int l = -2; l <= 2; l++) s2 += hs[r + l + 2][threadIdx.x] * g.t[l + 2];
        const double s1 = im1s[o];
        double t = s1;
        t *= 0.4;
        t += s2 * 0.6;
        blend[o] = t;
        imdt[o] = s2 - s1;
    }
}

__device__ __forceinline__ double warp_value(const double* __restrict__ im1, const double* __restrict__ im2, double fx,
                                             double fy, int i, int j, int H, int W) {
    const double y = i + fy;
    const double x = j + fx;
    if (x < 0 || x > W - 1 || y < 0 || y > H - 1) return im1[(size_t)i * W + j];
    return bilinear_apply(im2, bilinear_taps(W, H, x, y));
}
#ifndef PAPOF_V_WSROWS
#define PAPOF_V_WSROWS 16
#endif
#ifndef PAPOF_V_WSBATCH
#define PAPOF_V_WSBATCH 3
#endif
constexpr int kWsBatch = PAPOF_V_WSBATCH;
constexpr int kWsRows = PAPOF_V_WSROWS;
__global__ __launch_bounds__(256) void k_warp_smooth_blend(const double* __restrict__ im1, const double* __restrict__ im2,
                                                           const double* __restrict__ u, const double* __restrict__ v,
                                                           const double* __restrict__ im1s, double* __restrict__ blend,
                                                           double* __restrict__ imdt, int H, int W, Taps g,
                                                           unsigned long long* stamp, unsigned* __restrict__ wit,
                                                           double wit_thr, unsigned mark, double* __restrict__ phi_out) {
    __shared__ double raw[kWsRows + 4][BX + 4];
    __shared__ double hs[kWsRows + 4][BX];
    stamp_now(stamp);
    const int j0 = blockIdx.x * BX, i0 = blockIdx.y * kWsRows;
    const size_t np = (size_t)H * W;
    const double *p1 = im1 + blockIdx.z * np, *p2 = im2 + blockIdx.z * np;
    const bool exhaustive = wit != nullptr && gridDim.x == 1u && gridDim.y == 1u;
    bool ex_hit = false, ex_valid = false;
    const bool sampler = wit != nullptr && !exhaustive && threadIdx.y == 0u &&
                         (gridDim.x * gridDim.y <= 256u || ((blockIdx.x + 5u * blockIdx.y) & 15u) == 0u);
    constexpr int kWitStride = (kWsRows + 4) * (BX + 4) / 64;
    const int wr = (int)(threadIdx.x * kWitStride) / (BX + 4), wc = (int)(threadIdx.x * kWitStride) - wr * (BX + 4);
    double own1 = 0.0;
    if (sampler) own1 = p1[(size_t)clampi(i0 + wr - 2, H) * W + clampi(j0 + wc - 2, W)];
    constexpr int kCells = (kWsRows + 4) * (BX + 4), kPer = (kCells + BX * BY - 1) / (BX * BY);
    const int tid = threadIdx.y * BX + threadIdx.x;
#pragma unroll
    for (int q0 = 0; q0 < kPer; q0 += kWsBatch) {
        double fx[kWsBatch], fy[kWsBatch], val[kWsBatch][4];
        int off[kWsBatch];
#pragma unroll
        for (int q = 0; q < kWsBatch; q++) {
            const int c = min(tid + (q0 + q) * BX * BY, kCells - 1);
            const int r = c / (BX + 4), cc = c - r * (BX + 4);
            const int i = clampi(i0 + r - 2, H), j = clampi(j0 + cc - 2, W);
            off[q] = i * W + j;
            fx[q] = u[off[q]];
            fy[q] = v[off[q]];
        }
        bool outside[kWsBatch];
#pragma unroll
        for (int q = 0; q < kWsBatch; q++) {
            const int c = min(tid + (q0 + q) * BX * BY, kCells - 1);
            const int r = c / (BX + 4), cc = c - r * (BX + 4);
            const int i = clampi(i0 + r - 2, H), j = clampi(j0 + cc - 2, W);
            double y = i + fy[q], x = j + fx[q];
            outside[q] = x < 0 || x > W - 1 || y < 0 || y > H - 1;
            if (outside[q]) {
                x = j;
                y = i;
            }
            const int x0 = (int)x, y0 = (int)y;
            const int x1 = min(x0 + 1, W - 1), y1 = min(y0 + 1, H - 1);
            val[q][0] = p2[y0 * W + x0];
            val[q][1] = p2[y1 * W + x0];
            val[q][2] = p2[y0 * W + x1];
            val[q][3] = p2[y1 * W + x1];
            fx[q] = x - x0;
// ... 243 lines not shown
        } else if (I.lap != nullptr && I.lap[k] < 1E-20) {
            psi = 0.0;
        } else {
            psi = 1 / (2 * sqrt(t + 0.001 * 0.001));
        }
        const double pgx = psi * gx, pgy = psi * gy;
        if (planes == 1) {
            sxy = pgx * gy;
            sx2 = pgx * gx;
            sy2 = pgy * gy;
            stx = pgx * gt;
            sty = pgy * gt;
        } else {
            sxy += pgx * gy;
            sx2 += pgx * gx;
            sy2 += pgy * gy;
            stx += pgx * gt;
            sty += pgy * gt;
        }
    };
    if (PLANES > 0) {
#pragma unroll
        for (int k = 0; k < PLANES; k++) channel(k);
    } else {
#pragma unroll 1
        for (int k = 0; k < planes; k++) channel(k);
    }
    if (planes > 1) {
        sxy = sxy / planes;
        sx2 = sx2 / planes;
        sy2 = sy2 / planes;
        stx = stx / planes;
        sty = sty / planes;
    }
    SystemCell c;
    if (EDGE) {
        c.b1 = -stx - alpha * laplacian_at(u, phi, i, j, H, W);
        c.b2 = -sty - alpha * laplacian_at(v, phi, i, j, H, W);
        sor_diagonals(phi, i, j, H, W, sx2, sy2, alpha, omega, c.a1, c.a2);
    } else {
        const double pc = phi[o], pl = phi[o - 1], pu = phi[o - W];
        const double uc = u[o], vc = v[o];
        double lu = 0.0, lv = 0.0;
        lu -= (u[o + 1] - uc) * pc;
        lu += (uc - u[o - 1]) * pl;
        lu -= (u[o + W] - uc) * pc;
        lu += (uc - u[o - W]) * pu;
        lv -= (v[o + 1] - vc) * pc;
        lv += (vc - v[o - 1]) * pl;
        lv -= (v[o + W] - vc) * pc;
        lv += (vc - v[o - W]) * pu;
        c.b1 = -stx - alpha * lu;
        c.b2 = -sty - alpha * lv;
        double coeff = 0.0;
        coeff += pl;
        coeff += pc;
        coeff += pu;
        coeff += pc;
        coeff *= alpha;
        c.a1 = omega / (sx2 + alpha * 0.05 + coeff);
        c.a2 = omega / (sy2 + alpha * 0.05 + coeff);
    }
    c.phi = phi[o];
    c.xy = sxy;
    c.x2 = sx2;
    c.y2 = sy2;
    return c;
}

__global__ void k_assemble(const double* __restrict__ blend, const double* __restrict__ imdt,
                           const double* __restrict__ phi, const double* __restrict__ u,
                           const double* __restrict__ v, int H, int W, int planes, double alpha, double omega,
                           double* __restrict__ o_phi, double* __restrict__ o_xy, double* __restrict__ o_a1,
                           double* __restrict__ o_a2, double* __restrict__ o_b1, double* __restrict__ o_b2,
                           double* __restrict__ o_x2, double* __restrict__ o_y2, Taps d, Increment I, Rect rc,
                           unsigned long long* stamp) {
    stamp_now(stamp);
    const int j = rc.x0 + blockIdx.x * BX + threadIdx.x, i = rc.y0 + blockIdx.y * BY + threadIdx.y;
    if (j >= rc.x1 || i >= rc.y1) return;
    const size_t o = (size_t)i * W + j;
    const SystemCell c = assemble_cell(blend, imdt, phi, u, v, i, j, H, W, planes, alpha, omega, d, I);
    o_phi[o] = c.phi;
    o_xy[o] = c.xy;
    o_a1[o] = c.a1;
    o_a2[o] = c.a2;
    o_b1[o] = c.b1;
    o_b2[o] = c.b2;
    if (o_x2) o_x2[o] = c.x2;
    if (o_y2) o_y2[o] = c.y2;
}

#ifndef PAPOF_V_ASMCOLS
#define PAPOF_V_ASMCOLS 16
#endif
constexpr int kTileJ = PAPOF_V_ASMCOLS;
#ifndef PAPOF_V_ASMROWS
#define PAPOF_V_ASMROWS 16
#endif
constexpr int kAsmRows = PAPOF_V_ASMROWS;
struct double2s {
    double x, y;
};
template <int PLANES, bool FAST>
__global__ __launch_bounds__(256) void k_assemble_skew(const double* __restrict__ blend,
                                                       const double* __restrict__ imdt,
                                                       const double* __restrict__ phi, const double* __restrict__ u,
                                                       const double* __restrict__ v, int H, int W, int planes,
                                                       double alpha, double omega, SkewIdx sk,
                                                       double2s* __restrict__ pa, double2s* __restrict__ pb,
                                                       double2s* __restrict__ pc, double* __restrict__ o_x2,
                                                       double* __restrict__ o_y2, Taps d, Increment I,
                                                       unsigned long long* stamp, int row0, int row1) {
    __shared__ double stage[6][kAsmRows][kTileJ + 1];
    stamp_now(stamp);
    const int ib = row0 + blockIdx.y * kAsmRows, j0 = blockIdx.x * kTileJ, tid = threadIdx.x;
    const bool interior = ib >= 2 && ib + kAsmRows + 2 <= H && j0 >= 2 && j0 + kTileJ + 2 <= W;
    for (int c = tid; c < kAsmRows * kTileJ; c += 256) {
        const int r = c / kTileJ, jj = c - r * kTileJ;
        const int i = ib + r, j = j0 + jj;
        if (i < row1 && j < W) {
            const SystemCell s =
                interior ? assemble_cell<false, PLANES, FAST>(blend, imdt, phi, u, v, i, j, H, W, planes, alpha, omega, d, I)
                         : assemble_cell<true, PLANES, FAST>(blend, imdt, phi, u, v, i, j, H, W, planes, alpha, omega, d, I);
            stage[0][r][jj] = s.phi;
            stage[1][r][jj] = s.xy;
            stage[2][r][jj] = s.a1;
            stage[3][r][jj] = s.a2;
            stage[4][r][jj] = s.b1;
            stage[5][r][jj] = s.b2;
            if (o_x2) o_x2[(size_t)i * W + j] = s.x2;
            if (o_y2) o_y2[(size_t)i * W + j] = s.y2;
        }
    }
    __syncthreads();
    const int g = tid / kTileJ, jj = tid - g * kTileJ;
    const int j = j0 + jj;
    if (j >= W) return;
    for (int pp = g; pp <= kAsmRows + kTileJ - 2; pp += 256 / kTileJ) {
        const int r = pp - jj;
        if (r < 0 || r >= kAsmRows) continue;
        const int i = ib + r;
        if (i >= row1) continue;
        const size_t q = skew_cell(i, j, sk);
        pa[q] = double2s{stage[0][r][jj], stage[1][r][jj]};
        pb[q] = double2s{stage[2][r][jj], stage[3][r][jj]};
        pc[q] = double2s{stage[4][r][jj], stage[5][r][jj]};
    }
}

constexpr int kFT = 16, kFH = 4, kFW = kFT + 2 * kFH;
struct SixPlanes {
    double* q[6];
};
template <int PLANES, bool SKEW, bool BATCH = false>
__global__ __launch_bounds__(256, 1) void k_flow_system(const double* __restrict__ im1, const double* __restrict__ im2,
                                                     const double* __restrict__ u, const double* __restrict__ v,
                                                     const double* __restrict__ im1s, int H, int W, double alpha,
                                                     double omega, SkewIdx sk, SixPlanes out, Taps g, Taps d,
                                                     unsigned long long* stamp, unsigned* __restrict__ wit, double wit_thr,
                                                     unsigned mark, int row0, int row1, BatchK bk) {
    if (BATCH) {
        const size_t p = blockIdx.y;
        im1s += batch_frames(bk, p, im1, im2);
        u += p * bk.uv;
        v += p * bk.uv;
        if (wit != nullptr) wit += p * bk.wit;
#pragma unroll
        for (int q = 0; q < 6; q++) out.q[q] += p * bk.sp;
    }
    constexpr int NT = kFT * kFT, HWc = kFT + 2 * kFH;
    __shared__ double raw[kFW][HWc + 1];
    __shared__ double hs[kFW][kFT + 4 + 1];
    __shared__ double bl[kFT + 4][kFT + 4 + 1];
    __shared__ double it[kFT][kFT + 1];
    __shared__ double ph[kFT + 1][kFT + 1 + 1];
    __shared__ double stage[6][kFT][kFT + 1];
    stamp_now(stamp);
    const int ntx = (W + kFT - 1) / kFT, ntiles = ntx * ((row1 - row0 + kFT - 1) / kFT), per = (ntiles + 7) >> 3;
    const int vt = (int)(blockIdx.x & 7u) * per + (int)(blockIdx.x >> 3);
    if ((int)(blockIdx.x >> 3) >= per || vt >= ntiles) return;
    const int tby = vt / ntx, tbx = vt - tby * ntx;
    const int ib = row0 + tby * kFT, j0 = tbx * kFT, tid = threadIdx.x;
    const size_t np = (size_t)H * W;
    const int vy0 = max(0, row0 - kFH), vy1 = min(H, row1 + kFH);
    const bool interior = ib >= vy0 + kFH && ib + kFT <= row1 && ib + kFT + kFH <= vy1 && j0 >= kFH && j0 + kFT + kFH <= W;
    constexpr int kPer = (kFW * HWc + NT - 1) / NT;
    int t_o[kPer], t_x0[kPer], t_y0[kPer];
    double t_dx[kPer], t_dy[kPer];
    bool t_in[kPer], t_out[kPer];
#pragma unroll
    for (int q = 0; q < kPer; q++) {
        const int c = tid + q * NT, r = c / HWc, cc = c - r * HWc;
        const int i = ib - kFH + r, j = j0 - kFH + cc;
        t_in[q] = c < kFW * HWc && i >= vy0 && i < vy1 && j >= 0 && j < W;
        t_o[q] = t_in[q] ? i * W + j : 0;
        double x = 0.0, y = 0.0;
        t_out[q] = false;
        if (t_in[q]) {
            y = i + v[t_o[q]];
            x = j + u[t_o[q]];
            t_out[q] = x < 0 || x > W - 1 || y < 0 || y > H - 1;
            if (t_out[q]) {
                x = j;
                y = i;
            }
        }
        t_x0[q] = (int)x;
        t_y0[q] = (int)y;
        t_dx[q] = x - t_x0[q];
        t_dy[q] = y - t_y0[q];
    }
    for (int c = tid; c < (kFT + 1) * (kFT + 1); c += NT) {
        const int r = c / (kFT + 1), cc = c - r * (kFT + 1);
        const int i = ib - 1 + r, j = j0 - 1 + cc;
        if (i < 0 || i >= min(H, row1) || j < 0 || j >= W) continue;
        const size_t o = (size_t)i * W + j;
        const double uc = u[o], vc = v[o];
        double ur = 0.0, vr = 0.0, ud = 0.0, vd = 0.0;
        if (j < W - 1) {
            ur = u[o + 1];
            vr = v[o + 1];
        }
        if (i < H - 1) {
            ud = u[o + W];
            vd = v[o + W];
        }
        const double ux = j < W - 1 ? ur - uc : 0.0;
        const double uy = i < H - 1 ? ud - uc : 0.0;
        const double vx = j < W - 1 ? vr - vc : 0.0;
        const double vy = i < H - 1 ? vd - vc : 0.0;
        const double tt = ux * ux + uy * uy + vx * vx + vy * vy;
        ph[r][cc] = 0.5 / sqrt(tt + 0.001 * 0.001);
    }
    const int orow = tid / kFT, ocol = tid - orow * kFT;
    const int oi = ib + orow, oj = j0 + ocol;
    const bool own = oi < row1 && oj < W;
    double sxy = 0.0, sx2 = 0.0, sy2 = 0.0, stx = 0.0, sty = 0.0;
    const bool sampler = wit != nullptr && tid < 64 &&
                         (ntiles <= 256 || ((tbx + 5 * tby) & 15) == 0);
    constexpr int kP3 = ((kFT + 4) * (kFT + 4) + NT - 1) / NT;
    double gv[kPer][4], s1v[kP3], wv = 0.0;
    const auto load_gathers = [&](int k) {
        const double *p1 = im1 + k * np, *p2 = im2 + k * np;
#pragma unroll
        for (int q = 0; q < kPer; q++) {
            const double* src = t_out[q] ? p1 : p2;
            const int x0 = t_x0[q], y0 = t_y0[q], x1 = min(x0 + 1, W - 1), y1 = min(y0 + 1, H - 1);
            gv[q][0] = src[y0 * W + x0];
            gv[q][1] = src[y1 * W + x0];
            gv[q][2] = src[y0 * W + x1];
            gv[q][3] = src[y1 * W + x1];
        }
        if (sampler) wv = p1[t_o[0]];
    };
    const auto load_s1 = [&](int k) {
        const double* ps = im1s + k * np;
#pragma unroll
        for (int q = 0; q < kP3; q++) {
            const int c = min(tid + q * NT, (kFT + 4) * (kFT + 4) - 1), r = c / (kFT + 4), cc = c - r * (kFT + 4);
            s1v[q] = ps[(size_t)clampi(ib - 2 + r, H) * W + clampi(j0 - 2 + cc, W)];
        }
    };
    load_gathers(0);
    load_s1(0);
#pragma unroll 1
    for (int k = 0; k < PLANES; k++) {
        bool hit = false;
#pragma unroll
        for (int q = 0; q < kPer; q++) {
            const int c = tid + q * NT, r = c / HWc, cc = c - r * HWc;
            const double dx = t_dx[q], dy = t_dy[q], ex = 1.0 - dx, ey = 1.0 - dy;
            double res = 0.0;
            res += gv[q][0] * (ex * ey);
            res += gv[q][1] * (ex * dy);
            res += gv[q][2] * (dx * ey);
            res += gv[q][3] * (dx * dy);
            res = t_out[q] ? gv[q][0] : res;
            if (t_in[q]) raw[r][cc] = res;
            if (sampler && q == 0) {
                const double dd = fabs(wv - res);
                hit = t_in[q] && dd >= wit_thr && dd < 1000000;
            }
        }
        if (sampler) {
            const unsigned long long hits = __ballot(hit);
            if (hits != 0ull && tid == 0) wit[k] = mark;
        }
        if (k + 1 < PLANES) load_gathers(k + 1);
        __syncthreads();
        if (interior) {
            for (int c = tid; c < kFW * (kFT + 4); c += NT) {
                const int r = c / (kFT + 4), cc = c - r * (kFT + 4);
                double acc = 0.0;
#pragma unroll
                for (int l = -2; l <= 2; l++) acc += raw[r][cc + 2 + l] * g.t[l + 2];
                hs[r][cc] = acc;
            }
        } else {
            for (int c = tid; c < kFW * (kFT + 4); c += NT) {
                const int r = c / (kFT + 4), cc = c - r * (kFT + 4);
                const int i = ib - kFH + r, j = j0 - 2 + cc;
                if (i < 0 || i >= H || j < 0 || j >= W) continue;
                double acc = 0.0;
#pragma unroll
                for (int l = -2; l <= 2; l++) acc += raw[r][clampi(j + l, W) - (j0 - kFH)] * g.t[l + 2];
                hs[r][cc] = acc;
            }
        }
        __syncthreads();
#pragma unroll
        for (int q = 0; q < kP3; q++) {
            const int c = tid + q * NT, r = c / (kFT + 4), cc = c - r * (kFT + 4);
            const int i = ib - 2 + r, j = j0 - 2 + cc;
            if (c >= (kFT + 4) * (kFT + 4) || i < 0 || i >= H || j < 0 || j >= W) continue;
            double s2 = 0.0;
            if (interior) {
#pragma unroll
                for (int l = -2; l <= 2; l++) s2 += hs[r + 2 + l][cc] * g.t[l + 2];
            } else {
#pragma unroll
                for (int l = -2; l <= 2; l++) s2 += hs[clampi(i + l, H) - (ib - kFH)][cc] * g.t[l + 2];
            }
            const double s1 = s1v[q];
            double t = s1;
            t *= 0.4;
            t += s2 * 0.6;
            bl[r][cc] = t;
            if (r >= 2 && r < kFT + 2 && cc >= 2 && cc < kFT + 2) it[r - 2][cc - 2] = s2 - s1;
        }
        if (k + 1 < PLANES) load_s1(k + 1);
        __syncthreads();
        if (own) {
            double gx = 0.0, gy = 0.0;
            if (interior) {
#pragma unroll
                for (int l = -2; l <= 2; l++) gx += bl[orow + 2][ocol + 2 + l] * d.t[l + 2];
#pragma unroll
                for (int l = -2; l <= 2; l++) gy += bl[orow + 2 + l][ocol + 2] * d.t[l + 2];
            } else {
#pragma unroll
                for (int l = -2; l <= 2; l++) gx += bl[orow + 2][clampi(oj + l, W) - (j0 - 2)] * d.t[l + 2];
#pragma unroll
                for (int l = -2; l <= 2; l++) gy += bl[clampi(oi + l, H) - (ib - 2)][ocol + 2] * d.t[l + 2];
            }
            const double gt = it[orow][ocol];
            double t = gt;
            t *= t;
            const double psi = 1 / (2 * sqrt(t + 0.001 * 0.001));
            const double pgx = psi * gx, pgy = psi * gy;
            if (PLANES == 1) {
                sxy = pgx * gy;
                sx2 = pgx * gx;
                sy2 = pgy * gy;
                stx = pgx * gt;
                sty = pgy * gt;
            } else {
                sxy += pgx * gy;
                sx2 += pgx * gx;
                sy2 += pgy * gy;
                stx += pgx * gt;
                sty += pgy * gt;
            }
        }
    }
    if (own) {
        if (PLANES > 1) {
            sxy = sxy / PLANES;
            sx2 = sx2 / PLANES;
            sy2 = sy2 / PLANES;
            stx = stx / PLANES;
            sty = sty / PLANES;
        }
        const int i = oi, j = oj;
        const size_t o = (size_t)i * W + j;
        const double pc_ = ph[orow + 1][ocol + 1];
        const double pl = j > 0 ? ph[orow + 1][ocol] : 0.0, pu = i > 0 ? ph[orow][ocol + 1] : 0.0;
        const double uc = u[o], vc = v[o];
        double lu = 0.0, lv = 0.0;
        if (j < W - 1) {
            lu -= (u[o + 1] - uc) * pc_;
            if (j > 0) lu += (uc - u[o - 1]) * pl;
        }
        if (i < H - 1) {
            lu -= (u[o + W] - uc) * pc_;
            if (i > 0) lu += (uc - u[o - W]) * pu;
        }
        if (j < W - 1) {
            lv -= (v[o + 1] - vc) * pc_;
            if (j > 0) lv += (vc - v[o - 1]) * pl;
        }
        if (i < H - 1) {
            lv -= (v[o + W] - vc) * pc_;
            if (i > 0) lv += (vc - v[o - W]) * pu;
        }
        double coeff = 0.0;
        if (j > 0) coeff += pl;
        if (j < W - 1) coeff += pc_;
        if (i > 0) coeff += pu;
        if (i < H - 1) coeff += pc_;
        coeff *= alpha;
        const double a1 = omega / (sx2 + alpha * 0.05 + coeff), a2 = omega / (sy2 + alpha * 0.05 + coeff);
        const double b1 = -stx - alpha * lu, b2 = -sty - alpha * lv;
        if (SKEW) {
            stage[0][orow][ocol] = pc_;
            stage[1][orow][ocol] = sxy;
            stage[2][orow][ocol] = a1;
            stage[3][orow][ocol] = a2;
            stage[4][orow][ocol] = b1;
            stage[5][orow][ocol] = b2;
        } else {
            out.q[0][o] = pc_;
            out.q[1][o] = sxy;
            out.q[2][o] = a1;
            out.q[3][o] = a2;
            out.q[4][o] = b1;
            out.q[5][o] = b2;
        }
    }
    if (!SKEW) return;
    double2s* const pa = reinterpret_cast<double2s*>(out.q[0]);
    double2s* const pb = reinterpret_cast<double2s*>(out.q[2]);
    double2s* const pc = reinterpret_cast<double2s*>(out.q[4]);
    __syncthreads();
    const int grp = tid / kFT, jj = tid - grp * kFT, j = j0 + jj;
    if (j >= W) return;
    for (int pp = grp; pp <= 2 * kFT - 2; pp += kFT) {
        const int r = pp - jj;
        if (r < 0 || r >= kFT) continue;
        const int i = ib + r;
        if (i >= row1) continue;
        const size_t q = skew_cell(i, j, sk);
        pa[q] = double2s{stage[0][r][jj], stage[1][r][jj]};
        pb[q] = double2s{stage[2][r][jj], stage[3][r][jj]};
        pc[q] = double2s{stage[4][r][jj], stage[5][r][jj]};
    }
}

template <bool SKEW>
__global__ void k_sor_prep(const double* __restrict__ phi, const double* __restrict__ imdxy,
                           const double* __restrict__ imdx2, const double* __restrict__ imdy2,
                           const double* __restrict__ rhs1, const double* __restrict__ rhs2, int H, int W,
                           double alpha, double omega, SkewIdx sk, double* __restrict__ o_phi,
                           double* __restrict__ o_xy, double* __restrict__ o_a1, double* __restrict__ o_a2,
                           double* __restrict__ o_b1, double* __restrict__ o_b2) {
    const int j = blockIdx.x * BX + threadIdx.x, i = blockIdx.y * BY + threadIdx.y;
    if (j >= W || i >= H) return;
    const size_t o = (size_t)i * W + j;
    double a1, a2;
    sor_diagonals(phi, i, j, H, W, imdx2[o], imdy2[o], alpha, omega, a1, a2);
    const size_t q = sor_index<SKEW>(i, j, W, sk);
    o_phi[q] = phi[o];
    o_xy[q] = imdxy[o];
    o_a1[q] = a1;
    o_a2[q] = a2;
    o_b1[q] = rhs1[o];
    o_b2[q] = rhs2[o];
}

template <bool SKEW>
__global__ void k_sor_unpack(const double* __restrict__ sdu, const double* __restrict__ sdv,
                             double* __restrict__ du, double* __restrict__ dv, int H, int W, SkewIdx sk) {
    const int j = blockIdx.x * BX + threadIdx.x, i = blockIdx.y * BY + threadIdx.y;
    if (j >= W || i >= H) return;
    const size_t o = (size_t)i * W + j;
    if (SKEW) {
        const size_t q = 2 * dudv_cell(i, j, sk);
        du[o] = sdu[q];
        dv[o] = sdu[q + 1];
    } else {
        du[o] = sdu[o];
        dv[o] = sdv[o];
    }
}

__global__ void k_update_warp(const double* __restrict__ sdu, const double* __restrict__ sdv, double* __restrict__ u,
                              double* __restrict__ v, const double* __restrict__ im1,
                              const double* __restrict__ im2, double* __restrict__ warp, int H, int W, int planes, Rect rc,
                              int do_warp, unsigned long long* stamp) {
    stamp_now(stamp);
    const int j = rc.x0 + blockIdx.x * BX + threadIdx.x, i = rc.y0 + blockIdx.y * BY + threadIdx.y;
    if (j >= rc.x1 || i >= rc.y1) return;
    const size_t o = (size_t)i * W + j;
    double fu = u[o], fv = v[o];
    fu += sdu[o];
    fv += sdv[o];
    u[o] = fu;
    v[o] = fv;
    if (do_warp) warp_pixel(im1, im2, warp, fu, fv, i, j, H, W, planes);
}

template <bool SKEW, bool BATCH = false>
__global__ void k_update_warp_phi(const double* __restrict__ sdu, const double* __restrict__ sdv, SkewIdx sk,
                                  const double* __restrict__ u, const double* __restrict__ v,
                                  double* __restrict__ u_out, double* __restrict__ v_out,
                                  const double* __restrict__ im1, const double* __restrict__ im2,
                                  double* __restrict__ warp, double* __restrict__ phi_out, int H, int W, int planes,
                                  int do_warp, unsigned long long* stamp, int row0, int row1, unsigned* __restrict__ wit,
                                  double wit_thr, unsigned mark, BatchK bk) {
    stamp_now(stamp);
    if (BATCH) {
        const size_t p = blockIdx.y;
        sdu += p * bk.d;
        sdv += p * bk.d;
        u += p * bk.uv;
        v += p * bk.uv;
        u_out += p * bk.uv;
        v_out += p * bk.uv;
        batch_frames(bk, p, im1, im2);
        if (wit != nullptr) wit += p * bk.wit;
    }
    int tbx, tby;
    if (!xcd_tile((W + BX - 1) / BX, (row1 - row0 + BY - 1) / BY, tbx, tby)) return;
    const int j = tbx * BX + threadIdx.x, i = row0 + tby * BY + threadIdx.y;
    if (j >= W || i >= row1) return;
    const size_t o = (size_t)i * W + j;
    const auto inc = [&](int ii, int jj, double& a, double& b) {
        if (SKEW) {
            const double2s c = reinterpret_cast<const double2s*>(sdu)[dudv_cell(ii, jj, sk)];
            a = c.x;
            b = c.y;
        } else {
            a = sdu[(size_t)ii * W + jj];
            b = sdv[(size_t)ii * W + jj];
        }
    };
    double a, b;
    inc(i, j, a, b);
    double fu = u[o], fv = v[o];
    fu += a;
    fv += b;
    u_out[o] = fu;
    v_out[o] = fv;
    if (wit != nullptr) {
        const int bw = min(W - tbx * BX, BX), bh = min(row1 - (row0 + tby * BY), BY);
        const int lin = threadIdx.y * bw + threadIdx.x;
        const size_t np = (size_t)H * W;
        if (np <= 65536) {
            for (int k = bw * bh >= planes ? lin % planes : lin; k < planes; k += bw * bh) {
                const double w = warp_value(im1 + k * np, im2 + k * np, fu, fv, i, j, H, W);
                const double d = fabs(im1[k * np + o] - w);
                if (d >= wit_thr && d < 1000000) wit[k] = mark;
            }
        } else if (((tbx + 5 * tby) & 15) == 0)
        for (int k = lin; k < planes; k += bw * bh) {
            const double w = warp_value(im1 + k * np, im2 + k * np, fu, fv, i, j, H, W);
            const double d = fabs(im1[k * np + o] - w);
            if (d >= wit_thr && d < 1000000) wit[k] = mark;
        }
    }
    if (phi_out != nullptr) {
        double ur = 0.0, vr = 0.0, ud = 0.0, vd = 0.0;
        if (j < W - 1) {
            inc(i, j + 1, a, b);
            ur = u[o + 1];
            vr = v[o + 1];
            ur += a;
            vr += b;
        }
        if (i < H - 1) {
            inc(i + 1, j, a, b);
            ud = u[o + W];
            vd = v[o + W];
            ud += a;
            vd += b;
        }
        const double ux = j < W - 1 ? ur - fu : 0.0;
        const double uy = i < H - 1 ? ud - fu : 0.0;
        const double vx = j < W - 1 ? vr - fv : 0.0;
        const double vy = i < H - 1 ? vd - fv : 0.0;
        const double t = ux * ux + uy * uy + vx * vx + vy * vy;
        phi_out[o] = 0.5 / sqrt(t + 0.001 * 0.001);
    }
    if (do_warp) warp_pixel(im1, im2, warp, fu, fv, i, j, H, W, planes);
}

__global__ void k_update_warp_skew(const double2s* __restrict__ pd, double* __restrict__ u, double* __restrict__ v,
                                   const double* __restrict__ im1, const double* __restrict__ im2,
                                   double* __restrict__ warp, int H, int W, int planes, SkewIdx sk,
                                   unsigned long long* stamp, int do_warp) {
    stamp_now(stamp);
    const int j = blockIdx.x * BX + threadIdx.x, i = blockIdx.y * BY + threadIdx.y;
    if (j >= W || i >= H) return;
    const size_t o = (size_t)i * W + j;
    const double2s c = pd[dudv_cell(i, j, sk)];
    double fu = u[o], fv = v[o];
    fu += c.x;
    fv += c.y;
    u[o] = fu;
    v[o] = fv;
    if (do_warp) warp_pixel(im1, im2, warp, fu, fv, i, j, H, W, planes);
}

template <bool BATCH>
__global__ void k_bicubic(const double* __restrict__ im1, const double* __restrict__ im2,
                          const double* __restrict__ gx, const double* __restrict__ gy,
                          const double* __restrict__ gxy, const double* __restrict__ vx,
                          const double* __restrict__ vy, double* __restrict__ out, int H, int W, int C, Rect rc,
                          unsigned long long* stamp, int planar_out, int clamp, BatchK bk) {
    if (BATCH) {
        const size_t p = blockIdx.y;
        const ptrdiff_t o1 = (ptrdiff_t)batch_frames(bk, p, im1, im2);
        const ptrdiff_t o2 = bk.bw != 0 && p >= bk.bw ? o1 - 2 * (ptrdiff_t)bk.fr : o1;
        gx += o2;
        gy += o2;
        gxy += o2;
        vx += p * bk.uv;
        vy += p * bk.uv;
        out += p * bk.out;
    }
    stamp_now(stamp);
    int tbx, tby;
    if (!xcd_tile((rc.x1 - rc.x0 + BX - 1) / BX, (rc.y1 - rc.y0 + BY - 1) / BY, tbx, tby)) return;
    const int j = rc.x0 + tbx * BX + threadIdx.x, i = rc.y0 + tby * BY + threadIdx.y;
    if (j >= rc.x1 || i >= rc.y1) return;
    const size_t np = (size_t)H * W, o = (size_t)i * W + j;
    const size_t ostride = planar_out ? np : 1, obase = planar_out ? o : o * C;
    const double x = j + vx[o];
    const double y = i + vy[o];
    if (x < 0 || x > W - 1 || y < 0 || y > H - 1) {
        for (int k = 0; k < C; k++) {
            double r = im1[k * np + o];
            if (clamp) {
                r = r < 0 ? 0.0 : r;
                r = r > 1 ? 1.0 : r;
            }
            out[obase + k * ostride] = r;
        }
        return;
    }
    int x0 = (int)x, y0 = (int)y;
    int x1 = x0 + 1, y1 = y0 + 1;
    x0 = clampi(x0, W);
    x1 = clampi(x1, W);
    y0 = clampi(y0, H);
    y1 = clampi(y1, H);
    const double dx = x - x0, dy = y - y0;
    const double dx2 = dx * dx, dy2 = dy * dy;
    const double dx3 = dx * dx2, dy3 = dy * dy2;
    const size_t a = (size_t)y0 * W + x0, b = (size_t)y0 * W + x1, c = (size_t)y1 * W + x0, d = (size_t)y1 * W + x1;
    for (int k = 0; k < C; k++) {
        const double *f = im2 + k * np, *px = gx + k * np, *py = gy + k * np, *pz = gxy + k * np;
        const double fA = f[a], fB = f[b], fC = f[c], fD = f[d];
        const double xA = px[a], xB = px[b], xC = px[c], xD = px[d];
        const double yA = py[a], yB = py[b], yC = py[c], yD = py[d];
        const double zA = pz[a], zB = pz[b], zC = pz[c], zD = pz[d];
        const double c00 = fA;
        const double c10 = xA;
        const double c20 = -3 * fA + 3 * fB - 2 * xA - xB;
        const double c30 = 2 * fA - 2 * fB + xA + xB;
        const double c01 = yA;
        const double c11 = zA;
        const double c21 = -3 * yA + 3 * yB - 2 * zA - zB;
        const double c31 = 2 * yA - 2 * yB + zA + zB;
        const double c02 = -3 * fA + 3 * fC - 2 * yA - yC;
        const double c12 = -3 * xA + 3 * xC - 2 * zA - zC;
        const double c22 = 9 * fA - 9 * fB - 9 * fC + 9 * fD + 6 * xA + 3 * xB - 6 * xC - 3 * xD + 6 * yA - 6 * yB +
                           3 * yC - 3 * yD + 4 * zA + 2 * zB + 2 * zC + zD;
        const double c32 = -6 * fA + 6 * fB + 6 * fC - 6 * fD - 3 * xA - 3 * xB + 3 * xC + 3 * xD - 4 * yA + 4 * yB -
                           2 * yC + 2 * yD - 2 * zA - 2 * zB - zC - zD;
        const double c03 = 2 * fA - 2 * fC + yA + yC;
        const double c13 = 2 * xA - 2 * xC + zA + zC;
        const double c23 = -6 * fA + 6 * fB + 6 * fC - 6 * fD - 4 * xA - 2 * xB + 4 * xC + 2 * xD - 3 * yA + 3 * yB -
                           3 * yC + 3 * yD - 2 * zA - zB - 2 * zC - zD;
        const double c33 = 4 * fA - 4 * fB - 4 * fC + 4 * fD + 2 * xA + 2 * xB - 2 * xC - 2 * xD + 2 * yA - 2 * yB +
                           2 * yC - 2 * yD + zA + zB + zC + zD;
        double r = c00 + c01 * dy + c02 * dy2 + c03 * dy3 + c10 * dx + c11 * dx * dy + c12 * dx * dy2 +
                   c13 * dx * dy3 + c20 * dx2 + c21 * dx2 * dy + c22 * dx2 * dy2 + c23 * dx2 * dy3 + c30 * dx3 +
                   c31 * dx3 * dy + c32 * dx3 * dy2 + c33 * dx3 * dy3;
        if (clamp) {
            r = r < 0 ? 0.0 : r;
            r = r > 1 ? 1.0 : r;
        }
        out[obase + k * ostride] = r;
    }
}

__global__ void k_flow_quantize16(const double* __restrict__ vx, const double* __restrict__ vy,
                                  unsigned short* __restrict__ q, size_t n) {
    const size_t i = (size_t)blockIdx.x * blockDim.x + threadIdx.x;
    if (i >= n) return;
    double a = vx[i], b = vy[i];
    a = (a < -200) ? -200.0 : a;
    a = (a > 200) ? 200.0 : a;
    b = (b < -200) ? -200.0 : b;
    b = (b > 200) ? 200.0 : b;
    q[i * 2] = (unsigned short)((a + 200) * 160);
    q[i * 2 + 1] = (unsigned short)((b + 200) * 160);
}

__global__ void k_flow_dequantize16(const unsigned short* __restrict__ q, double* __restrict__ vx,
                                    double* __restrict__ vy, size_t n) {
    const size_t i = (size_t)blockIdx.x * blockDim.x + threadIdx.x;
    if (i >= n) return;
    vx[i] = (double)q[i * 2] / 160 - 200;
    vy[i] = (double)q[i * 2 + 1] / 160 - 200;
}

__global__ void k_flow_mag_minmax(const double* __restrict__ vx, const double* __restrict__ vy, size_t n,
                                  double* __restrict__ partial) {
    __shared__ double smin[256], smax[256];
    double lo = INFINITY, hi = -INFINITY;
    for (size_t i = (size_t)blockIdx.x * blockDim.x + threadIdx.x; i < n; i += (size_t)gridDim.x * blockDim.x) {
        const double m = sqrt(vx[i] * vx[i] + vy[i] * vy[i]);
        lo = m < lo ? m : lo;
        hi = m > hi ? m : hi;
    }
    smin[threadIdx.x] = lo;
    smax[threadIdx.x] = hi;
    __syncthreads();
    for (int s = 128; s > 0; s >>= 1) {
        if ((int)threadIdx.x < s) {
            smin[threadIdx.x] = fmin(smin[threadIdx.x], smin[threadIdx.x + s]);
            smax[threadIdx.x] = fmax(smax[threadIdx.x], smax[threadIdx.x + s]);
        }
        __syncthreads();
    }
    if (threadIdx.x == 0) {
        partial[2 * blockIdx.x] = smin[0];
        partial[2 * blockIdx.x + 1] = smax[0];
    }
}

__global__ void k_flow_bgr(const double* __restrict__ vx, const double* __restrict__ vy, size_t n,
                           const double* __restrict__ partial, int nblocks, unsigned char* __restrict__ bgr) {
    const size_t i = (size_t)blockIdx.x * blockDim.x + threadIdx.x;
    if (i >= n) return;
    double lo = INFINITY, hi = -INFINITY;
    for (int b = 0; b < nblocks; b++) {
        lo = fmin(lo, partial[2 * b]);
        hi = fmax(hi, partial[2 * b + 1]);
    }
    const double x = vx[i], y = vy[i];
    const double mag = sqrt(x * x + y * y);
    double ang = atan2(y, x);
    if (ang < 0) ang += 2 * M_PI;
    const unsigned char H = (unsigned char)(int)(ang * 180 / M_PI / 2);
    const double scale = hi > lo ? 255.0 / (hi - lo) : 0.0;
    const unsigned char V = (unsigned char)(int)((mag - lo) * scale);
    const float v = V * (1.f / 255.f);
    float h = H * (6.f / 180.f);
    int sector = (int)floorf(h);
    h -= sector;
    sector = ((sector % 6) + 6) % 6;
    const float tab[4] = {v, 0.f, v * (1.f - h), v * h};
    const int sd[6][3] = {{1, 3, 0}, {1, 0, 2}, {3, 0, 1}, {0, 2, 1}, {0, 1, 3}, {2, 1, 0}};
    bgr[i * 3] = (unsigned char)(int)rintf(tab[sd[sector][0]] * 255.f);
    bgr[i * 3 + 1] = (unsigned char)(int)rintf(tab[sd[sector][1]] * 255.f);
    bgr[i * 3 + 2] = (unsigned char)(int)rintf(tab[sd[sector][2]] * 255.f);
}

}

Taps gaussian_taps(double sigma, int fsize) {
    Taps f{};
    f.fsize = fsize;
    double sum = 0;
    const double s2 = sigma * sigma * 2;
    for (int i = -fsize; i <= fsize; i++) {
        f.t[i + fsize] = std::exp(-(double)(i * i) / s2);
        sum += f.t[i + fsize];
    }
    for (int i = 0; i < 2 * fsize + 1; i++) f.t[i] /= sum;
    return f;
}

Taps smooth5_taps() {
    Taps f{};
    f.fsize = 2;
    const double g[5] = {0.02, 0.11, 0.74, 0.11, 0.02};
    for (int i = 0; i < 5; i++) f.t[i] = g[i];
    return f;
}

Taps deriv5_taps() {
    Taps f{};
    f.fsize = 2;
    const double d[5] = {1, -8, 0, 8, -1};
    for (int i = 0; i < 5; i++) {
        f.t[i] = d[i];
        f.t[i] /= 12;
    }
    return f;
}

Taps central3_taps() {
    Taps f{};
    f.fsize = 1;
    f.t[0] = -0.5;
    f.t[1] = 0;
    f.t[2] = 0.5;
    return f;
}

#define LAUNCH_CHECK() PAPOF_HIP(hipGetLastError())

int hwc_to_planar(papof_handle* h, const double* hwc, double* planar, int H, int W, int C, int frames) {
    hipLaunchKernelGGL(k_hwc_to_planar, grid2d(W, H, frames), dim3(BX, BY), 0, h->stream, hwc, planar, H, W, C);
    LAUNCH_CHECK();
    return PAPOF_OK;
}

int hwc_u8_to_planar(papof_handle* h, const unsigned char* hwc, double* planar, int H, int W, int C, int frames) {
    hipLaunchKernelGGL(k_hwc_u8_to_planar, grid2d(W, H, frames), dim3(BX, BY), 0, h->stream, hwc, planar, H, W, C);
    LAUNCH_CHECK();
    return PAPOF_OK;
}

int ingest_frames(papof_handle* h, const papof_tensor& a, const papof_tensor* b, double* planar, int H, int W, int C,
                  int frames) {
    const long long total = (long long)frames * H * W * C, blocks = (total + 255) / 256;
    if (total <= 0) return PAPOF_OK;
    if (blocks > 0x7fffffffLL) return PAPOF_EINVAL;
    hipLaunchKernelGGL(k_ingest_frames, dim3((unsigned)blocks), dim3(256), 0, h->stream, a, b ? *b : a, b ? 1 : 0, planar,
                       (long long)H, (long long)W, (long long)C, total);
    LAUNCH_CHECK();
    return PAPOF_OK;
}

int init_check(papof_handle* h, const papof_tensor& t, int pairs, int H, int W, unsigned* flag) {
    const long long total = (long long)pairs * H * W * 2, blocks = (total + 255) / 256;
    if (total <= 0) return PAPOF_OK;
    if (blocks > 0x7fffffffLL) return PAPOF_EINVAL;
    hipLaunchKernelGGL(k_init_check, dim3((unsigned)blocks), dim3(256), 0, h->stream, t, (long long)H, (long long)W, total,
                       flag);
    LAUNCH_CHECK();
    return PAPOF_OK;
// ... 67 lines not shown
    LAUNCH_CHECK();
    return PAPOF_OK;
}

int filter_hv(papof_handle* h, const double* src, double* dst, double* tmp, int H, int W, int planes, const Taps& fh,
              const Taps& fv) {
    if (fh.fsize > kHvMaxF || fv.fsize > kHvMaxF) {
        if (!tmp) return PAPOF_EINVAL;
        PAPOF_TRY(filter_h(h, src, tmp, H, W, planes, fh));
        return filter_v(h, tmp, dst, H, W, planes, fv);
    }
    const dim3 grid((W + BX - 1) / BX, (H + kHvRows - 1) / kHvRows, planes), block(BX, BY);
    const int f = fh.fsize == fv.fsize ? fh.fsize : -1;
    if (PAPOF_V_HVSTAGED && f >= 1 && f <= 3) {
        const dim3 sgrid(xcd_grid((W + BX - 1) / BX, (H + kHvsRows - 1) / kHvsRows), 1, planes);
        if (f == 1)
            hipLaunchKernelGGL(k_filter_hv_staged<1>, sgrid, block, 0, h->stream, src, dst, H, W, fh, fv);
        else if (f == 2)
            hipLaunchKernelGGL(k_filter_hv_staged<2>, sgrid, block, 0, h->stream, src, dst, H, W, fh, fv);
        else
            hipLaunchKernelGGL(k_filter_hv_staged<3>, sgrid, block, 0, h->stream, src, dst, H, W, fh, fv);
        LAUNCH_CHECK();
        return PAPOF_OK;
    }
    if (f == 1)
        hipLaunchKernelGGL(k_filter_hv<1>, grid, block, 0, h->stream, src, dst, H, W, fh, fv);
    else if (f == 2)
        hipLaunchKernelGGL(k_filter_hv<2>, grid, block, 0, h->stream, src, dst, H, W, fh, fv);
    else if (f == 3)
        hipLaunchKernelGGL(k_filter_hv<3>, grid, block, 0, h->stream, src, dst, H, W, fh, fv);
    else
        hipLaunchKernelGGL(k_filter_hv<-1>, grid, block, 0, h->stream, src, dst, H, W, fh, fv);
    LAUNCH_CHECK();
    return PAPOF_OK;
}

int resize(papof_handle* h, const double* src, double* dst, int sh, int sw, int planes, int dh, int dw, double xr,
           double yr, bool use_post, double post, const Rect* rc) {
    const Rect r = region(rc, dw, dh);
    if (r.empty()) return PAPOF_OK;
    hipLaunchKernelGGL(k_resize, dim3(xcd_grid((r.x1 - r.x0 + BX - 1) / BX, (r.y1 - r.y0 + BY - 1) / BY), 1, planes), dim3(BX, BY), 0, h->stream, src, dst, sh, sw, dh, dw, xr, yr,
                       use_post ? 1 : 0, post, r, take_stamp(h));
    LAUNCH_CHECK();
    return PAPOF_OK;
}

int im2feature(papof_handle* h, const double* im, double* feat, int H, int W, int C, unsigned* nz, int frames, size_t nz_stride) {
    const size_t np = (size_t)H * W;
    if (C == 3) {
        hipLaunchKernelGGL((frames > 1 ? k_im2feature_tiled<3, true> : k_im2feature_tiled<3, false>), dim3(xcd_grid((W + BX - 1) / BX, (H + kFeatRows - 1) / kFeatRows), frames), dim3(BX, BY), 0,
                           h->stream, im, feat, H, W, deriv5_taps(), nz, h->lap_epoch, 3 * np, 5 * np, nz_stride);
    } else if (C == 1) {
        hipLaunchKernelGGL((frames > 1 ? k_im2feature_tiled<1, true> : k_im2feature_tiled<1, false>), dim3(xcd_grid((W + BX - 1) / BX, (H + kFeatRows - 1) / kFeatRows), frames), dim3(BX, BY), 0,
                           h->stream, im, feat, H, W, deriv5_taps(), nz, h->lap_epoch, np, 3 * np, nz_stride);
    } else {
        if (frames != 1) return PAPOF_EINVAL;
        PAPOF_HIP(hipMemcpyAsync(feat, im, sizeof(double) * (size_t)H * W * C, hipMemcpyDeviceToDevice, h->stream));
        return PAPOF_OK;
    }
    LAUNCH_CHECK();
    return PAPOF_OK;
}

int warp_bilinear(papof_handle* h, const double* im1, const double* im2, const double* vx, const double* vy,
                  double* out, int H, int W, int planes, const Rect* rc) {
    const Rect r = region(rc, W, H);
    if (r.empty()) return PAPOF_OK;
    hipLaunchKernelGGL(k_warp, grid2d(r), dim3(BX, BY), 0, h->stream, im1, im2, vx, vy, out, H, W, planes, r,
                       take_stamp(h));
    LAUNCH_CHECK();
    return PAPOF_OK;
}

int smooth_v_blend(papof_handle* h, const double* tmp, const double* im1s, double* blend, double* imdt, int H,
                   int W, int planes, const Rect* rc) {
    const Rect r = region(rc, W, H);
    if (r.empty()) return PAPOF_OK;
    hipLaunchKernelGGL(k_smooth_v_blend, grid2d(r, planes), dim3(BX, BY), 0, h->stream, tmp, im1s, blend, imdt, H, W,
                       smooth5_taps(), r);
    LAUNCH_CHECK();
    return PAPOF_OK;
}

static SkewIdx skew_idx(const SorPlanes& sp) {
    return SkewIdx{sp.sd.hp, sp.sd.qt, sp.sd.rt, sp.sd.nb, sp.sd.npos_d, sp.sd.dpar, sp.sd.band_rows, sp.sd.koff, sp.sd.poff};
}

static Increment increment_of(const SorPlanes* prev, const double* gm = nullptr, const double* lap = nullptr) {
    if (!prev) return Increment{nullptr, nullptr, 0, SkewIdx{0, 0, 0, 0, 0, 0, 0}, gm, lap};
    return Increment{prev->du, prev->dv, prev->skew ? 1 : 0, prev->skew ? skew_idx(*prev) : SkewIdx{0, 0, 0, 0, 0, 0, 0},
                     gm, lap};
}

int smooth_hv_blend(papof_handle* h, const double* warp, const double* im1s, double* blend, double* imdt, int H,
                    int W, int planes, int row0, int row1) {
    if (row1 < 0) row1 = H;
    if (row0 < 0 || row1 > H) return PAPOF_EINVAL;
    if (row1 <= row0) return PAPOF_OK;
    hipLaunchKernelGGL(k_smooth_hv_blend, dim3((W + BX - 1) / BX, (row1 - row0 + kFuseRows - 1) / kFuseRows, planes),
                       dim3(BX, BY), 0, h->stream, warp, im1s, blend, imdt, H, W, smooth5_taps(), take_stamp(h), row0,
                       row1);
    LAUNCH_CHECK();
    return PAPOF_OK;
}

int warp_smooth_blend(papof_handle* h, const double* im1, const double* im2, const double* u, const double* v,
                      const double* im1s, double* blend, double* imdt, int H, int W, int planes, unsigned* wit,
                      double* phi_out) {
    hipLaunchKernelGGL(k_warp_smooth_blend, dim3((W + BX - 1) / BX, (H + kWsRows - 1) / kWsRows, planes), dim3(BX, BY), 0,
                       h->stream, im1, im2, u, v, im1s, blend, imdt, H, W, smooth5_taps(), take_stamp(h), wit,
                       2e-20 * (double)H * (double)W, h->lap_epoch, phi_out);
    LAUNCH_CHECK();
    return PAPOF_OK;
}

int compute_phi(papof_handle* h, const double* u, const double* v, const SorPlanes* prev, double* phi, int H, int W,
                const Rect* rc) {
    const Rect r = region(rc, W, H);
    if (r.empty()) return PAPOF_OK;
    hipLaunchKernelGGL(k_phi, grid2d(r), dim3(BX, BY), 0, h->stream, u, v, increment_of(prev), phi, H, W, r,
                       take_stamp(h));
    LAUNCH_CHECK();
    return PAPOF_OK;
}

int assemble_system(papof_handle* h, const double* blend, const double* imdt, const double* phi, const double* u,
                    const double* v, int H, int W, int planes, double alpha, double omega, const SorPlanes& out,
                    double* opt_imdx2, double* opt_imdy2, const SorPlanes* prev, const Rect* rc, const double* gm,
                    const double* lap) {
    const Increment I = increment_of(prev, gm, lap);
    const Rect r = region(rc, W, H);
    if (r.empty()) return PAPOF_OK;
    if (out.skew) {
        if (rc && (r.x0 != 0 || r.x1 != W)) return PAPOF_EINVAL;
        const bool fast = I.du == nullptr && I.gm == nullptr && I.lap == nullptr;
        const auto kern = planes == 5   ? (fast ? k_assemble_skew<5, true> : k_assemble_skew<5, false>)
                          : planes == 3 ? (fast ? k_assemble_skew<3, true> : k_assemble_skew<3, false>)
                                        : k_assemble_skew<0, false>;
        hipLaunchKernelGGL(kern, dim3((W + kTileJ - 1) / kTileJ, (r.y1 - r.y0 + kAsmRows - 1) / kAsmRows),
                           dim3(256), 0, h->stream, blend, imdt, phi, u, v, H, W, planes, alpha, omega, skew_idx(out),
                           (double2s*)out.phi, (double2s*)out.a1, (double2s*)out.b1, opt_imdx2, opt_imdy2,
                           deriv5_taps(), I, take_stamp(h), r.y0, r.y1);
    } else {
        hipLaunchKernelGGL(k_assemble, grid2d(r), dim3(BX, BY), 0, h->stream, blend, imdt, phi, u, v, H, W, planes,
                           alpha, omega, out.phi, out.xy, out.a1, out.a2, out.b1, out.b2, opt_imdx2, opt_imdy2,
                           deriv5_taps(), I, r, take_stamp(h));
    }
    LAUNCH_CHECK();
    return PAPOF_OK;
}

int flow_system(papof_handle* h, const double* im1, const double* im2, const double* u, const double* v, const double* im1s,
                int H, int W, int planes, double alpha, double omega, const SorPlanes& out, unsigned* wit, int row0, int row1,
                int batch, const BatchK* bk) {
    if (planes != 5 && planes != 3) return PAPOF_EINVAL;
    if (row1 < 0) row1 = H;
    if (row0 < 0 || row1 > H) return PAPOF_EINVAL;
    if (row1 <= row0) return PAPOF_OK;
    const int ntiles = ((W + kFT - 1) / kFT) * ((row1 - row0 + kFT - 1) / kFT);
    const dim3 grid(8 * ((ntiles + 7) / 8), batch);
    const SixPlanes six{{out.phi, out.xy, out.a1, out.a2, out.b1, out.b2}};
    const BatchK bk0{0, 0, 0, 0, 0, 0};
    const auto kern = batch > 1 ? (out.skew ? (planes == 5 ? k_flow_system<5, true, true> : k_flow_system<3, true, true>)
                                            : (planes == 5 ? k_flow_system<5, false, true> : k_flow_system<3, false, true>))
                                : (out.skew ? (planes == 5 ? k_flow_system<5, true> : k_flow_system<3, true>)
                                            : (planes == 5 ? k_flow_system<5, false> : k_flow_system<3, false>));
    hipLaunchKernelGGL(kern, grid, dim3(kFT * kFT), 0, h->stream, im1, im2, u, v, im1s, H, W, alpha, omega,
                       out.skew ? skew_idx(out) : SkewIdx{0, 0, 0, 0, 0, 0, 0, 0, 0}, six, smooth5_taps(), deriv5_taps(),
                       take_stamp(h), wit, 2e-20 * (double)H * (double)W, h->lap_epoch, row0, row1, bk ? *bk : bk0);
    LAUNCH_CHECK();
    return PAPOF_OK;
}

int laplacian(papof_handle* h, const double* in, const double* weight, double* out, int H, int W) {
    hipLaunchKernelGGL(k_laplacian, grid2d(W, H), dim3(BX, BY), 0, h->stream, in, weight, out, H, W);
    LAUNCH_CHECK();
    return PAPOF_OK;
}

int update_and_warp(papof_handle* h, const SorPlanes& sp, double* u, double* v, const double* im1,
                    const double* im2, double* warp, int H, int W, int planes, bool do_warp) {
    if (sp.skew) {
        hipLaunchKernelGGL(k_update_warp_skew, grid2d(W, H), dim3(BX, BY), 0, h->stream, (const double2s*)sp.du, u, v,
                           im1, im2, warp, H, W, planes, skew_idx(sp), take_stamp(h), do_warp ? 1 : 0);
    } else {
        hipLaunchKernelGGL(k_update_warp, grid2d(W, H), dim3(BX, BY), 0, h->stream, sp.du, sp.dv, u, v, im1, im2, warp,
                           H, W, planes, Rect{0, 0, W, H}, do_warp ? 1 : 0, take_stamp(h));
    }
    LAUNCH_CHECK();
    return PAPOF_OK;
}

int update_warp_phi(papof_handle* h, const SorPlanes& sp, const double* u, const double* v, double* u_out, double* v_out,
                    const double* im1, const double* im2, double* warp, double* phi_out, int H, int W, int planes,
                    bool do_warp, int row0, int row1, unsigned* wit, int batch, const BatchK* bk) {
    const double wit_thr = 2e-20 * (double)H * (double)W;
    const BatchK bk0{0, 0, 0, 0, 0, 0};
    if (batch > 1 && (warp || phi_out || do_warp)) return PAPOF_EINVAL;
    if (u == u_out || v == v_out) return PAPOF_EINVAL;
    if (row1 < 0) row1 = H;
    if (row0 < 0 || row1 > H) return PAPOF_EINVAL;
    if (row1 <= row0) return PAPOF_OK;
    const dim3 grid(xcd_grid((W + BX - 1) / BX, (row1 - row0 + BY - 1) / BY), batch);
    if (sp.skew)
        hipLaunchKernelGGL((batch > 1 ? k_update_warp_phi<true, true> : k_update_warp_phi<true, false>), grid, dim3(BX, BY), 0,
                           h->stream, sp.du, sp.dv, skew_idx(sp),
                           u, v, u_out, v_out, im1, im2, warp, phi_out, H, W, planes, do_warp ? 1 : 0, take_stamp(h),
                           row0, row1, wit, wit_thr, h->lap_epoch, bk ? *bk : bk0);
    else
        hipLaunchKernelGGL((batch > 1 ? k_update_warp_phi<false, true> : k_update_warp_phi<false, false>), grid, dim3(BX, BY), 0, h->stream, sp.du, sp.dv,
                           SkewIdx{0, 0, 0, 0, 0, 0, 0, 0, 0}, u, v, u_out, v_out, im1, im2, warp, phi_out, H, W, planes,
                           do_warp ? 1 : 0, take_stamp(h), row0, row1, wit, wit_thr, h->lap_epoch, bk ? *bk : bk0);
    LAUNCH_CHECK();
    return PAPOF_OK;
}

int update_flow(papof_handle* h, const SorPlanes& sp, double* u, double* v, int H, int W, const Rect& r) {
    if (sp.skew) return PAPOF_EINVAL;
    if (r.empty()) return PAPOF_OK;
    hipLaunchKernelGGL(k_update_warp, grid2d(r), dim3(BX, BY), 0, h->stream, sp.du, sp.dv, u, v, nullptr, nullptr, nullptr,
                       H, W, 0, r, 0, take_stamp(h));
    LAUNCH_CHECK();
    return PAPOF_OK;
}

int flow_quantize16(papof_handle* h, const double* vx, const double* vy, unsigned short* q, size_t n) {
    if (!n) return PAPOF_OK;
    hipLaunchKernelGGL(k_flow_quantize16, dim3((unsigned)((n + 255) / 256)), dim3(256), 0, h->stream, vx, vy, q, n);
    LAUNCH_CHECK();
    return PAPOF_OK;
}

int flow_dequantize16(papof_handle* h, const unsigned short* q, double* vx, double* vy, size_t n) {
    if (!n) return PAPOF_OK;
    hipLaunchKernelGGL(k_flow_dequantize16, dim3((unsigned)((n + 255) / 256)), dim3(256), 0, h->stream, q, vx, vy, n);
    LAUNCH_CHECK();
    return PAPOF_OK;
}

int flow_to_bgr(papof_handle* h, const double* vx, const double* vy, size_t n, double* partial ,
                unsigned char* bgr) {
    if (!n) return PAPOF_OK;
    const int nblocks = 256;
    hipLaunchKernelGGL(k_flow_mag_minmax, dim3(nblocks), dim3(256), 0, h->stream, vx, vy, n, partial);
    hipLaunchKernelGGL(k_flow_bgr, dim3((unsigned)((n + 255) / 256)), dim3(256), 0, h->stream, vx, vy, n, partial,
                       nblocks, bgr);
    LAUNCH_CHECK();
    return PAPOF_OK;
}

int bicubic_warp(papof_handle* h, const double* im1, const double* im2, const double* gx, const double* gy,
                 const double* gxy, const double* vx, const double* vy, double* out_hwc, int H, int W, int C,
                 const Rect* rc, bool planar_out, bool clamp, int batch, const BatchK* bk) {
    const Rect r = region(rc, W, H);
    if (r.empty()) return PAPOF_OK;
    const BatchK bk0{0, 0, 0, 0, 0, 0};
    hipLaunchKernelGGL(batch > 1 ? k_bicubic<true> : k_bicubic<false>, dim3(xcd_grid((r.x1 - r.x0 + BX - 1) / BX, (r.y1 - r.y0 + BY - 1) / BY), batch), dim3(BX, BY), 0, h->stream, im1, im2, gx, gy, gxy, vx, vy, out_hwc, H, W,
                       C, r, take_stamp(h), planar_out ? 1 : 0, clamp ? 1 : 0, bk ? *bk : bk0);
    LAUNCH_CHECK();
    return PAPOF_OK;
}

constexpr int kGmBlocks = 256, kGmThreads = 256, kGmMaxC = 8;
static __global__ __launch_bounds__(kGmThreads) void k_gm_partial(const double* __restrict__ im1,
                                                           const double* __restrict__ im2, size_t np, int C,
                                                           const double* __restrict__ gm, double* __restrict__ partial) {
    __shared__ double red[kGmThreads];
    double acc[kGmMaxC][4];
    for (int k = 0; k < kGmMaxC; k++) acc[k][0] = acc[k][1] = acc[k][2] = acc[k][3] = 0.0;
    for (size_t o = (size_t)blockIdx.x * kGmThreads + threadIdx.x; o < np; o += (size_t)kGmBlocks * kGmThreads) {
#pragma unroll
        for (int k = 0; k < kGmMaxC; k++) {
            if (k >= C) break;
            double t = im1[k * np + o] - im2[k * np + o];
            t *= t;
            const double alpha_k = gm[k], sigma = gm[C + k], beta = gm[2 * C + k], s2 = gm[3 * C + k], b2 = gm[4 * C + k];
            double w1 = exp(-t / (2 * s2)) / (2 * 3.1415927 * sigma) * alpha_k;
            double w2 = exp(-t / (2 * b2)) / (2 * 3.1415927 * beta) * (1 - alpha_k);
            const double s = w1 + w2;
            w1 /= s;
            w2 /= s;
            acc[k][0] += w1;
            acc[k][1] += w2;
            acc[k][2] += w1 * t;
            acc[k][3] += w2 * t;
        }
    }
    for (int k = 0; k < C; k++)
        for (int q = 0; q < 4; q++) {
            red[threadIdx.x] = acc[k][q];
            __syncthreads();
            for (int s = kGmThreads / 2; s > 0; s >>= 1) {
                if ((int)threadIdx.x < s) red[threadIdx.x] += red[threadIdx.x + s];
                __syncthreads();
            }
            if (threadIdx.x == 0) partial[((size_t)blockIdx.x * kGmMaxC + k) * 4 + q] = red[0];
            __syncthreads();
        }
}

static __global__ void k_gm_mstep(const double* __restrict__ partial, int C, double prior, double* __restrict__ gm) {
    const int k = threadIdx.x;
    if (k >= C) return;
    double t1 = 0.0, t2 = 0.0, s1 = 0.05, s2 = 0.5;
    for (int b = 0; b < kGmBlocks; b++) {
        const double* p = partial + ((size_t)b * kGmMaxC + k) * 4;
        t1 += p[0];
        t2 += p[1];
        s1 += p[2];
        s2 += p[3];
    }
    const double alpha = t1 / (t1 + t2) * (1 - prior) + 0.95 * prior;
    const double sigma = sqrt(s1 / t1);
    const double beta = sqrt(s2 / t2) * (1 - prior) + 0.3 * prior;
    gm[k] = alpha;
    gm[C + k] = sigma;
    gm[2 * C + k] = beta;
    gm[3 * C + k] = sigma * sigma;
    gm[4 * C + k] = beta * beta;
}

int gm_scratch_doubles() { return kGmBlocks * kGmMaxC * 4; }

int est_gaussian_mixture(papof_handle* h, const double* im1, const double* im2, int H, int W, int C, double* gm,
                         double* scratch) {
    if (C > kGmMaxC) return PAPOF_EINVAL;
    for (int it = 0; it < 3; it++) {
        hipLaunchKernelGGL(k_gm_partial, dim3(kGmBlocks), dim3(kGmThreads), 0, h->stream, im1, im2, (size_t)H * W, C, gm,
                           scratch);
        hipLaunchKernelGGL(k_gm_mstep, dim3(1), dim3(64), 0, h->stream, scratch, C, 0.9, gm);
    }
    LAUNCH_CHECK();
    return PAPOF_OK;
}

constexpr int kLapBlocks = 256, kLapThreads = 256, kLapMaxC = 8;
static __global__ __launch_bounds__(kLapThreads) void k_lap_partial(const double* __restrict__ im1,
                                                             const double* __restrict__ im2,
                                                             const double* __restrict__ u, const double* __restrict__ v,
                                                             int H, int W, int C, double* __restrict__ partial) {
    __shared__ double red[kLapThreads];
    const size_t np = (size_t)H * W;
    double acc[kLapMaxC][2];
    for (int k = 0; k < kLapMaxC; k++) acc[k][0] = acc[k][1] = 0.0;
    for (size_t o = (size_t)blockIdx.x * kLapThreads + threadIdx.x; o < np; o += (size_t)kLapBlocks * kLapThreads) {
        const int i = (int)(o / W), j = (int)(o - (size_t)i * W);
        const double fu = u ? u[o] : 0.0, fv = u ? v[o] : 0.0;
#pragma unroll
        for (int k = 0; k < kLapMaxC; k++) {
            if (k >= C) break;
            const double w = u ? warp_value(im1 + k * np, im2 + k * np, fu, fv, i, j, H, W) : im2[k * np + o];
            const double d = fabs(im1[k * np + o] - w);
            if (d > 0 && d < 1000000) {
                acc[k][0] += d;
                acc[k][1] += 1.0;
            }
        }
    }
    for (int k = 0; k < C; k++)
        for (int q = 0; q < 2; q++) {
            red[threadIdx.x] = acc[k][q];
            __syncthreads();
            for (int s = kLapThreads / 2; s > 0; s >>= 1) {
                if ((int)threadIdx.x < s) red[threadIdx.x] += red[threadIdx.x + s];
                __syncthreads();
            }
            if (threadIdx.x == 0) partial[((size_t)blockIdx.x * kLapMaxC + k) * 2 + q] = red[0];
            __syncthreads();
        }
}
static __global__ void k_lap_finish(const double* __restrict__ partial, int C, double* __restrict__ lap) {
    const int k = threadIdx.x;
    if (k >= C) return;
    double s = 0.0, n = 0.0;
    for (int b = 0; b < kLapBlocks; b++) {
        s += partial[((size_t)b * kLapMaxC + k) * 2];
        n += partial[((size_t)b * kLapMaxC + k) * 2 + 1];
    }
    lap[k] = n == 0 ? 0.001 : s / n;
}
static __global__ __launch_bounds__(256) void k_lap_small(const double* __restrict__ im1, const double* __restrict__ im2,
                                                       const double* __restrict__ u, const double* __restrict__ v, int H,
                                                       int W, unsigned* __restrict__ wit, double wit_thr, unsigned mark,
                                                       BatchK bk) {
    const int np = H * W;
    {
        const size_t p = blockIdx.y;
        batch_frames(bk, p, im1, im2);
        u += p * bk.uv;
        v += p * bk.uv;
        wit += p * bk.wit;
    }
    const double *p1 = im1 + (size_t)blockIdx.x * np, *p2 = im2 + (size_t)blockIdx.x * np;
    bool hit = false, valid = false;
    for (int o = threadIdx.x; o < np; o += 256) {
        const int i = o / W, j = o - i * W;
        const double d = fabs(p1[o] - warp_value(p1, p2, u[o], v[o], i, j, H, W));
        valid = valid || (d > 0 && d < 1000000);
        hit = hit || (d >= wit_thr && d < 1000000);
    }
    const int any_hit = __syncthreads_or(hit ? 1 : 0), any_valid = __syncthreads_or(valid ? 1 : 0);
    if (threadIdx.x == 0 && (any_hit || !any_valid)) wit[blockIdx.x] = any_hit ? mark : (mark ^ kLapNone);
}
static __global__ __launch_bounds__(256) void k_lap_rows(const double* __restrict__ im1, const double* __restrict__ im2,
                                                      const double* __restrict__ u, const double* __restrict__ v, int H,
                                                      int W, int r0, int r1, unsigned* __restrict__ wit,
                                                      unsigned* __restrict__ val, double wit_thr, unsigned mark) {
    const size_t np = (size_t)H * W;
    const double *p1 = im1 + blockIdx.y * np, *p2 = im2 + blockIdx.y * np;
    bool hit = false, valid = false;
    const int n = (r1 - r0) * W;
    for (int c = blockIdx.x * 256 + threadIdx.x; c < n; c += gridDim.x * 256) {
        const int i = r0 + c / W, j = c - (c / W) * W;
        const size_t o = (size_t)i * W + j;
        const double d = fabs(p1[o] - warp_value(p1, p2, u[o], v[o], i, j, H, W));
// ... 72 lines not shown
```

papteam_opticalflow_amd/csrc/sor.hip:

```cpp
#include <algorithm>
#include <cstdio>
#include <cstdlib>
#include <cstring>
#include <type_traits>

#include "common.h"

namespace papof {

namespace {

#ifndef PAPOF_V_DM6
#define PAPOF_V_DM6 4
#endif
#ifndef PAPOF_V_DM8
#define PAPOF_V_DM8 5
#endif
#ifndef PAPOF_V_FDM6
#define PAPOF_V_FDM6 3
#endif
#ifndef PAPOF_V_FDM8
#define PAPOF_V_FDM8 4
#endif
#ifndef PAPOF_V_FMIDPOLL
// ... 1444 lines not shown
            PAPOF_BLOCKED(PAPOF_SOR_JACOBI, 4, 6);
        else
            PAPOF_BLOCKED(PAPOF_SOR_JACOBI, 8, 4);
    }
#undef PAPOF_BLOCKED
    PAPOF_HIP(hipGetLastError());
    return PAPOF_OK;
}


struct TinyShape {
    int c, nw;
    int waves;
};
#define PAPOF_TINY_SHAPES(X) X(1, 16) X(2, 16) X(3, 12) X(5, 8) X(6, 8)
static bool tiny_shape(int H, int W, TinyShape& best) {
#define PAPOF_TINY_CAND(CC, NWW) {CC, NWW, 0},
    static const TinyShape cand[] = {PAPOF_TINY_SHAPES(PAPOF_TINY_CAND)};
#undef PAPOF_TINY_CAND
    if (H < 1 || W < 1 || (size_t)H * W > kTinyMaxCells) return false;
    for (TinyShape t : cand) {
        const int Q = (W + t.c - 1) / t.c, QP = (Q + 1) / 2;
        if ((long long)H * QP > t.nw * 64) continue;
        if ((size_t)(H + 2) * 2 * t.c * (QP + 2) * 16 > (size_t)150 * 1024) continue;
        t.waves = (H * QP + 63) / 64;
        best = t;
        return true;
    }
    return false;
}

bool sor_tiny_shape(int H, int W, int* cells_per_tile, int* waves) {
    TinyShape t{0, 0, 0};
    const bool ok = tiny_shape(H, W, t);
    if (cells_per_tile) *cells_per_tile = ok ? t.c : 0;
    if (waves) *waves = ok ? t.waves : 0;
    return ok;
}

bool sor_tiny_fits(const papof_handle* h, int H, int W, int n_sor) {
    TinyShape t;
    return (!h || h->sor_tiny) && n_sor >= 1 && tiny_shape(H, W, t);
}

static int sor_tiny_solve(papof_handle* h, const SorPlanes& sp, int H, int W, double alpha, double omega, int n_sor,
                          int batch = 1, size_t bstride = 0) {
    TinyShape t;
    if (sp.skew || n_sor < 1 || !tiny_shape(H, W, t)) return PAPOF_EINVAL;
    TinyArgs A;
    A.phi = sp.phi;
    A.xy = sp.xy;
    A.a1 = sp.a1;
    A.a2 = sp.a2;
    A.b1 = sp.b1;
    A.b2 = sp.b2;
    A.du = sp.du;
    A.dv = sp.dv;
    A.H = H;
    A.W = W;
    A.K = n_sor;
    A.Q = (W + t.c - 1) / t.c;
    A.QP = (A.Q + 1) / 2;
    A.nalpha = -alpha;
    A.om1 = 1 - omega;
    A.bstride = batch > 1 ? bstride : 0;
    const size_t lds = (size_t)(H + 2) * 2 * t.c * (A.QP + 2) * 16;
#define PAPOF_TINY(CC, NWW)                                                                                           \
    do {                                                                                                              \
        static bool attr_set = false;                                                                                 \
        if (!attr_set) {                                                                                              \
            PAPOF_HIP(hipFuncSetAttribute((const void*)k_sor_tiny<CC, NWW>, hipFuncAttributeMaxDynamicSharedMemorySize, \
                                          150 * 1024));                                                               \
            attr_set = true;                                                                                          \
        }                                                                                                             \
        hipLaunchKernelGGL((k_sor_tiny<CC, NWW>), dim3(batch), dim3(t.waves * 64), lds, h->stream, A);                    \
    } while (0)
#define PAPOF_TINY_CASE(CC, NWW) \
    if (t.c == CC) PAPOF_TINY(CC, NWW);
    PAPOF_TINY_SHAPES(PAPOF_TINY_CASE)
#undef PAPOF_TINY_CASE
#undef PAPOF_TINY
    PAPOF_HIP(hipGetLastError());
    return PAPOF_OK;
}

int sor_group_size(const papof_handle* h, int H, int W, int n_sor);
static int sor_fuse_size(const papof_handle* h, int H, int W, int n_sor, int group);

struct BlockedPlan {
    int q, n_launch, base, rem;
};
static BlockedPlan blocked_plan(const papof_handle* h, int mode, int H, int W, int units) {
    const BlockedShape bs = blocked_shape(h, mode, H, W);
    const bool one_block = W <= 2 * kLanes && H <= bs.nw * bs.rpt;
    BlockedPlan p;
    p.q = (mode == PAPOF_SOR_REDBLACK && units % 2 == 0) ? 2 : 1;
    const int n_units = units / p.q;
    const int depth = one_block ? n_units : std::max(1, sor_blocked_depth(h, mode, H, W) / p.q);
    p.n_launch = (n_units + depth - 1) / depth;
    p.base = n_units / p.n_launch;
    p.rem = n_units % p.n_launch;
    return p;
}

static int sor_blocked_solve(papof_handle* h, const SorPlanes& sp, int H, int W, double alpha, double omega, int mode,
                             int units) {
    if (!sp.du2 || !sp.dv2) return PAPOF_EINVAL;
    const BlockedPlan bp = blocked_plan(h, mode, H, W, units);
    const Rect all{0, 0, W, H};
    const double *su = nullptr, *sv = nullptr;
    bool to_main = (bp.n_launch & 1) != 0;
    int done = 0;
    for (int l = 0; l < bp.n_launch; l++) {
        const int g = bp.q * (bp.base + (l < bp.rem ? 1 : 0));
        double *du = to_main ? sp.du : sp.du2, *dv = to_main ? sp.dv : sp.dv2;
        PAPOF_TRY(sor_blocked_launch(h, sp, H, W, alpha, omega, mode, g, done, all, su, sv, du, dv));
        su = du;
        sv = dv;
        done += g;
        to_main = !to_main;
    }
    return PAPOF_OK;
}

int sor_plan(const papof_handle* h, int H, int W, int n_sor, int mode, int* launches, int* depth) {
    if (!h || H < 1 || W < 1 || n_sor < 1) return PAPOF_EINVAL;
    int nl = 0, d = 0;
    if (mode == PAPOF_SOR_EXACT) {
        const int group = sor_group_size(h, H, W, n_sor);
        const SkewDims sd = skew_dims(H, W, n_sor, group, sor_fuse_size(h, H, W, n_sor, group));
        const bool aff = h->sor_xcd_affine && (sd.nb <= 8 || (h->sor_xcd_affine > 1 && sd.group == 1));
        const int per = aff ? 8 * ((sd.nb + 7) / 8) : sd.nb;
        const int units = sd.group > 1 ? (n_sor + sd.group - 1) / sd.group : (sd.fuse == 2 ? (n_sor + 1) / 2 : n_sor);
        const int chunk = std::max(1, resident_tasks(h) / (per * std::max(1, sd.group)));
        nl = (units + chunk - 1) / chunk;
        d = sd.fuse == 2 ? 2 : sd.group;
    } else if (mode == PAPOF_SOR_REDBLACK || mode == PAPOF_SOR_JACOBI) {
        const BlockedPlan bp = blocked_plan(h, mode, H, W, mode == PAPOF_SOR_REDBLACK ? 2 * n_sor : n_sor);
        nl = bp.n_launch;
        d = bp.q * (bp.base + (bp.rem ? 1 : 0));
    } else {
        return PAPOF_EINVAL;
    }
    if (launches) *launches = nl;
    if (depth) *depth = d;
    return PAPOF_OK;
}

int sor_solve(papof_handle* h, const SorPlanes& sp, int H, int W, double alpha, double omega, int n_sor, int mode,
              const SorBatch* bt) {
    const double nalpha = -alpha, om1 = 1 - omega;
    if (n_sor <= 0) return PAPOF_EINVAL;
    const int batch = bt ? bt->n : 1;
    if (batch < 1 || (bt && mode != PAPOF_SOR_EXACT)) return PAPOF_EINVAL;
    const auto mark = [&](int on) {
        if (h->sor_mark) h->sor_mark(h->sor_mark_ctx, on);
    };
    const auto log_solve = [&](int kind, int depth, int launches) {
        if (h->sor_log.size() >= 4096) h->sor_log.clear();
        h->sor_log.push_back(papof_handle::SorSolveLog{H, W, n_sor, kind, depth, launches, 0.0});
    };
    if (mode == PAPOF_SOR_EXACT && !sp.skew) {
        mark(1);
        PAPOF_TRY(sor_tiny_solve(h, sp, H, W, alpha, omega, n_sor, batch, bt ? bt->tiny : 0));
        mark(0);
        log_solve(6, 0, 1);
        return PAPOF_OK;
    }
    if (mode == PAPOF_SOR_EXACT) {
        const SkewDims sd = skew_dims(H, W, n_sor, sp.sd.group, sp.sd.fuse);
        if (sd.fuse != sp.sd.fuse || sd.hp != sp.sd.hp || sd.npos != sp.sd.npos || sd.qt != sp.sd.qt || sd.nb != sp.sd.nb ||
            sd.n_sor != sp.sd.n_sor || sd.n > sp.cap_cells || sd.nd + sd.nh > sp.cap_cells_d)
            return PAPOF_EINVAL;
        if ((sd.n + kLanes) * 16 >= (size_t(1) << 30) || (sd.nd + sd.nh) * 16 >= (size_t(1) << 30))
            return PAPOF_EINVAL;
        if (bt && (sd.fuse != 1 || sd.group != 1 || !h->sor_prog_next)) return PAPOF_EINVAL;
        const size_t words = (size_t)sd.nb * n_sor * kProgStride + kProgStride;
        if (!bt && words > h->sync_cap) {
            PAPOF_HIP(hipStreamSynchronize(h->stream));
            if (h->sync_words) PAPOF_HIP(hipFree(h->sync_words));
            h->sync_words = nullptr;
            h->sync_cap = 0;
            const size_t cap = (words + 1023) & ~size_t(1023);
            PAPOF_HIP(hipMalloc((void**)&h->sync_words, cap * sizeof(unsigned)));
            h->sync_cap = cap;
            PAPOF_HIP(hipMemsetAsync(h->sync_words, 0, cap * sizeof(unsigned), h->stream));
        }
        unsigned* prog = h->sync_words + kProgStride;
        if (h->sor_prog_next) {
            prog = h->sor_prog_next;
            h->sor_prog_next = nullptr;
        } else {
            const size_t nbytes = (size_t)sd.nb * n_sor * kProgStride * sizeof(unsigned);
            PAPOF_HIP(hipMemsetAsync(prog, 0, nbytes, h->stream));
        }
        ExactArgs A;
        A.phi = sp.phi;
        A.xy = sp.xy;
        A.a1 = sp.a1;
        A.a2 = sp.a2;
        A.b1 = sp.b1;
        A.b2 = sp.b2;
        A.du = sp.du;
        A.dv = sp.dv;
        A.prog = prog;
        A.abort = h->sync_words;
        A.H = H;
        A.W = W;
        A.nb = sd.nb;
        A.ns = sd.ns;
        A.hp = sd.hp;
        A.npos = sd.npos;
        A.qt = sd.qt;
        A.rt = sd.rt;
        A.npos_d = sd.npos_d;
        A.n_sor = n_sor;
        A.nalpha = nalpha;
        A.om1 = om1;
        A.k0 = 0;
        A.b0 = 0;
        A.nbl = sd.nb;
        A.peer_du = nullptr;
        A.peer_prog = nullptr;
        A.top_cut = A.bot_cut = 0;
        A.skip_dead = h->sor_skip_dead;
        A.bs_coef = bt ? bt->coef : 0;
        A.bs_d = bt ? bt->d : 0;
        A.bs_prog = bt ? bt->prog : 0;
        A.dbg = bt ? nullptr : h->sor_dbg;
        if (std::getenv("PAPOF_SOR_INJECT_ABORT")) PAPOF_HIP(hipMemsetAsync(h->sync_words, 1, sizeof(unsigned), h->stream));
        if (bt) {
            PAPOF_TRY(fill_pairs(h, sp.du, bt->d * sizeof(double), sd.nd * 16, batch));
        } else {
            PAPOF_HIP(hipMemsetAsync(sp.du, 0, (sd.nd + sd.nh) * 16, h->stream));
        }
        mark(1);
        if (sd.group > 1) {
            GroupArgs Ga;
            Ga.phi = sp.phi;
            Ga.a1 = sp.a1;
            Ga.b1 = sp.b1;
            Ga.du = sp.du;
            Ga.prog = prog;
            Ga.abort = h->sync_words;
            Ga.nb = sd.nb;
            Ga.ns = sd.ns;
            Ga.hp = sd.hp;
            Ga.npos = sd.npos;
            Ga.qt = sd.qt;
            Ga.rt = sd.rt;
            Ga.npos_d = sd.npos_d;
            Ga.n_sor = n_sor;
            Ga.halo_off = (unsigned)(sd.nd * 16);
            Ga.dbg = h->sor_dbg;
            Ga.nalpha = nalpha;
            Ga.om1 = om1;
            Ga.g0 = 0;
            const int groups = (n_sor + sd.group - 1) / sd.group;
            Ga.xcd_affine = (h->sor_xcd_affine && sd.nb <= 8) ? 1 : 0;
            const int per_g = Ga.xcd_affine ? 8 * ((sd.nb + 7) / 8) : sd.nb;
            const int Rg = h->sor_depth > 0 ? h->sor_depth : (sd.nb >= 9 ? 10 : 8);
            const int chunk = std::max(1, resident_tasks(h) / (per_g * sd.group));
            for (int g0 = 0; g0 < groups; g0 += chunk) {
                Ga.g0 = g0;
                h->sor_launches++;
                Ga.stamp = nullptr;
                const dim3 ggrid(per_g * std::min(chunk, groups - g0));
                if (sd.group == 4 && Rg >= 12)
                    hipLaunchKernelGGL((k_sor_group<12, 4, true>), ggrid, dim3(kLanes * 4), 0, h->stream, Ga);
                else if (sd.group == 4 && Rg >= 10)
                    hipLaunchKernelGGL((k_sor_group<10, 4, true>), ggrid, dim3(kLanes * 4), 0, h->stream, Ga);
                else if (sd.group == 4 && Rg >= 8)
                    hipLaunchKernelGGL((k_sor_group<8, 4, true>), ggrid, dim3(kLanes * 4), 0, h->stream, Ga);
                else if (sd.group == 4)
                    hipLaunchKernelGGL((k_sor_group<6, 4, true>), ggrid, dim3(kLanes * 4), 0, h->stream, Ga);
                else if (sd.group == 2)
                    hipLaunchKernelGGL((k_sor_group<8, 2, true>), ggrid, dim3(kLanes * 2), 0, h->stream, Ga);
                else
                    return PAPOF_EINVAL;
            }
            PAPOF_HIP(hipGetLastError());
            mark(0);
            log_solve(2, Rg, (groups + chunk - 1) / chunk);
            return PAPOF_OK;
        }
        if (sd.fuse == 2) {
            const int pairs = (n_sor + 1) / 2;
            A.xcd_affine = (h->sor_xcd_affine && (sd.nb <= 8 || h->sor_xcd_affine > 1)) ? 1 : 0;
            const int per_q = A.xcd_affine ? 8 * ((sd.nb + 7) / 8) : sd.nb;
            const int Rf = h->sor_depth > 0 ? h->sor_depth : 8;
            const int chunk = std::max(1, resident_tasks(h) / per_q);
            for (int q0 = 0; q0 < pairs; q0 += chunk) {
                A.k0 = q0;
                h->sor_launches++;
                A.stamp = nullptr;
                const dim3 fgrid(per_q * std::min(chunk, pairs - q0));
                if (Rf <= 6)
                    hipLaunchKernelGGL((k_sor_fused<6, true>), fgrid, dim3(kLanes), 0, h->stream, A);
                else if (Rf <= 8)
                    hipLaunchKernelGGL((k_sor_fused<8, true>), fgrid, dim3(kLanes), 0, h->stream, A);
                else if (Rf <= 10)
                    hipLaunchKernelGGL((k_sor_fused<10, true>), fgrid, dim3(kLanes), 0, h->stream, A);
                else
                    hipLaunchKernelGGL((k_sor_fused<12, true>), fgrid, dim3(kLanes), 0, h->stream, A);
            }
            PAPOF_HIP(hipGetLastError());
            mark(0);
            log_solve(1, Rf, (pairs + chunk - 1) / chunk);
            return PAPOF_OK;
        }
        A.xcd_affine = (h->sor_xcd_affine && (sd.nb <= 8 || h->sor_xcd_affine > 1)) ? 1 : 0;
        if (bt) A.xcd_affine = 0;
        const int per_k = A.xcd_affine ? 8 * ((sd.nb + 7) / 8) : sd.nb;
        const dim3 block(kLanes);
        const int R = h->sor_depth > 0 ? h->sor_depth : (sd.nb >= 8 ? 8 : 6);
        const int chunk = std::max(1, resident_tasks(h) / (per_k * batch));
        for (int k0 = 0; k0 < n_sor; k0 += chunk) {
            A.k0 = k0;
            h->sor_launches++;
            A.stamp = nullptr;
            const dim3 grid(per_k * std::min(chunk, n_sor - k0), batch);
            if (!h->use_dpp)
                hipLaunchKernelGGL((k_sor_exact<8, false>), grid, block, 0, h->stream, A);
            else if (R <= 4)
                hipLaunchKernelGGL((k_sor_exact<4, true>), grid, block, 0, h->stream, A);
            else if (R <= 6)
                hipLaunchKernelGGL((k_sor_exact<6, true>), grid, block, 0, h->stream, A);
            else if (R <= 8)
                hipLaunchKernelGGL((k_sor_exact<8, true>), grid, block, 0, h->stream, A);
            else if (R <= 10)
                hipLaunchKernelGGL((k_sor_exact<10, true>), grid, block, 0, h->stream, A);
            else
                hipLaunchKernelGGL((k_sor_exact<12, true>), grid, block, 0, h->stream, A);
        }
        PAPOF_HIP(hipGetLastError());
        mark(0);
        log_solve(0, R, (n_sor + chunk - 1) / chunk);
        return PAPOF_OK;
    }
    if (sp.skew) return PAPOF_EINVAL;
    mark(1);
    PAPOF_TRY(sor_blocked_solve(h, sp, H, W, alpha, omega, mode, mode == PAPOF_SOR_REDBLACK ? 2 * n_sor : n_sor));
    mark(0);
    const BlockedPlan bp = blocked_plan(h, mode, H, W, mode == PAPOF_SOR_REDBLACK ? 2 * n_sor : n_sor);
    log_solve(mode == PAPOF_SOR_REDBLACK ? 3 : 4, bp.q * (bp.base + (bp.rem ? 1 : 0)), bp.n_launch);
    return PAPOF_OK;
}

__global__ __launch_bounds__(256) void k_fill_pairs(uint4* __restrict__ d, size_t stride16, size_t n16) {
    uint4* const p = d + (size_t)blockIdx.y * stride16;
    for (size_t c = (size_t)blockIdx.x * 256 + threadIdx.x; c < n16; c += (size_t)gridDim.x * 256) p[c] = uint4{0u, 0u, 0u, 0u};
}
static int fill_pairs(papof_handle* h, void* base, size_t stride_bytes, size_t bytes, int batch) {
    if ((stride_bytes | bytes | (size_t)(uintptr_t)base) & 15) return PAPOF_EINVAL;
    const size_t n16 = bytes / 16;
    const unsigned gx = (unsigned)std::min<size_t>((n16 + 1023) / 1024, 2048);
    hipLaunchKernelGGL(k_fill_pairs, dim3(std::max(1u, gx), batch), dim3(256), 0, h->stream, (uint4*)base, stride_bytes / 16, n16);
    PAPOF_HIP(hipGetLastError());
    return PAPOF_OK;
}

__global__ void k_sor_clear_bands(uint4* __restrict__ d, int nb, int b0, int nbl, unsigned n16) {
    const unsigned t = blockIdx.x * blockDim.x + threadIdx.x;
    if (t >= n16) return;
    const unsigned per = (unsigned)nbl * kLanes, pos = t / per, r = t - pos * per;
    d[((size_t)pos * nb + b0) * kLanes + r] = uint4{0u, 0u, 0u, 0u};
}

bool sor_strips_supported(const papof_handle* h, const SorPlanes& sp, int n_sor) {
    if (!sp.skew || sp.sd.group > 1 || !h->use_dpp || n_sor < 3) return false;
    if (h->sor_xcd_affine && (sp.sd.nb <= 8 || h->sor_xcd_affine > 1)) return false;
    const int per = sp.sd.nb, tasks = per * (sp.sd.fuse == 2 ? (n_sor + 1) / 2 : n_sor);
    return tasks <= resident_tasks(h);
}

size_t sor_counters_words(int H, int W, int n_sor) {
    const int nb = std::max(skew_dims(H, W, n_sor, 1, 1).nb, skew_dims(H, W, n_sor, 1, 2).nb);
    return (size_t)nb * n_sor * kProgStride;
}

int sor_counters_ensure(papof_handle* h, size_t words) {
    const size_t need = words + kProgStride;
    if (need <= h->sync_cap) return PAPOF_OK;
    PAPOF_HIP(hipStreamSynchronize(h->stream));
    if (h->sync_words) PAPOF_HIP(hipFree(h->sync_words));
    h->sync_words = nullptr;
// ... 257 lines not shown
```

Baseline: 205.9.

## Compute bicubic derivatives inline in final warp and fold SOR du clear into flow system

Adds a direct bicubic warp kernel that computes the central-difference x, y and xy derivatives from a 4x4 neighbourhood on the fly. This removes the separate central3_planes pass and its three gradient planes, and is on by default. Behind an opt-in environment switch, the k_flow_system kernel can also zero the SOR du buffer so that sor_solve skips its memset. The zero-start memset of u/v is moved earlier, before the wait on the prep stream. The direct warp repeats derivative arithmetic for every output pixel, in exchange for less memory traffic and one fewer kernel launch.

Result: no change. 206.3, median of 3 (+0.2%).

```diff
diff --git a/papteam_opticalflow_amd/csrc/api.hip b/papteam_opticalflow_amd/csrc/api.hip
--- a/papteam_opticalflow_amd/csrc/api.hip
+++ b/papteam_opticalflow_amd/csrc/api.hip
@@ -29,7 +29,7 @@
     return std::chrono::duration<double>(std::chrono::steady_clock::now().time_since_epoch()).count();
 }
 
-size_t arena_bytes_for(int H, int W, int C, int levels, int n_sor_max, double ratio) {
+size_t arena_bytes_for(int H, int W, int C, int levels, int n_sor_max, double ratio, bool warp_planes) {
     const size_t np = (size_t)H * W;
     const int fc = (C == 3) ? 5 : (C == 1 ? 3 : C);
     size_t per_level = 0;
@@ -47,7 +47,7 @@
     planes += (size_t)2 * C + 2 * C;
     planes += (size_t)7 * fc;
     planes += 8;
-    planes += (size_t)3 * C + C;
+    planes += (size_t)(warp_planes ? 3 : 0) * C + C;
     planes += (size_t)3 * fc;
     size_t bytes = planes * np * sizeof(double);
     bytes += 3 * (sor_cells + 2 * kLanes) * 16 + (sor_cells_d + 2 * kLanes) * 16 + 10 * np * sizeof(double);
@@ -288,11 +288,15 @@
     const bool fused_env = !(fused_sw && fused_sw[0] == '0');
     const bool fused_system = fused_env && fold_warp && n_inner == 1 && !B.gm && (fc == 5 || fc == 3) &&
                               !(lg && lg->guard()) && !(lg && lg->on && lap_one_block_level(H, W));
+    const char* const fold_sw = std::getenv("PAPOF_FOLD_CLEAR");
+    const bool fold_clear = fused_system && SP.skew && mode == PAPOF_SOR_EXACT && fold_sw && fold_sw[0] == '1' &&
+                            SP.sd.nd + SP.sd.nh <= SP.cap_cells_d;
     for (int count = 0; count < n_outer; count++) {
         clk.phase(fused_system ? kTimerFused : (int)PAPOF_T_PHASE1_GENERATE);
         if (fused_system)
             PAPOF_TRY(flow_system(h, f1, f2, u, v, im1s, H, W, fc, alpha, omega, SP,
-                                  lg && count > 0 ? lg->wit(lg->slot - 1) : nullptr));
+                                  lg && count > 0 ? lg->wit(lg->slot - 1) : nullptr, 0, -1, 1, nullptr,
+                                  fold_clear ? SP.du : nullptr, fold_clear ? SP.sd.nd + SP.sd.nh : 0));
         else if (fold_warp)
             PAPOF_TRY(warp_smooth_blend(h, f1, f2, u, v, im1s, B.blend, B.imdt, H, W, fc,
                                         lg && count > 0 && !B.gm ? lg->wit(lg->slot - 1) : nullptr,
@@ -314,9 +318,11 @@
             };
             h->sor_mark_ctx = &clk;
             h->sor_prog_next = prog ? prog + (size_t)solve_idx * prog_per_solve : nullptr;
+            h->sor_dudv_clear_next = fold_clear;
             solve_idx++;
             const int rc_solve = sor_solve(h, SP, H, W, alpha, omega, n_sor, mode);
             h->sor_prog_next = nullptr;
+            h->sor_dudv_clear_next = false;
             h->sor_mark = nullptr;
             h->sor_mark_ctx = nullptr;
             PAPOF_TRY(rc_solve);
@@ -380,6 +386,11 @@
            q.arena_base == h->arena.base && need <= h->arena.cap;
 }
 
+bool warp_direct_on() {
+    const char* const sw = std::getenv("PAPOF_WARP_DIRECT");
+    return !(sw && sw[0] == '0');
+}
+
 int flow_pass(papof_handle* h, const FrameIn& fa, const FrameIn& fb, SeqOp op, int H, int W, int C, int levels,
               const papof_params& P, double* d_vx, double* d_vy, double* d_warp, double* timing, LapGuard* lg,
               const papof_tensor* init = nullptr) {
@@ -391,7 +402,8 @@
     std::vector<PyrPlan> plan;
     PAPOF_TRY(pyramid_plan(H, W, P.ratio, levels, L, plan));
     const int n_sor_max = P.n_sor + (levels - 1) * P.n_sor_per_level;
-    const size_t need = arena_bytes_for(H, W, C, levels, n_sor_max, P.ratio);
+    const bool warp_direct = warp_direct_on();
+    const size_t need = arena_bytes_for(H, W, C, levels, n_sor_max, P.ratio, !warp_direct);
     if (op == kSeqNext && !seq_matches(h, H, W, C, levels, ratio, need)) {
         g_last_error = "sequence push does not continue the primed sequence (shape, levels, ratio or arena changed)";
         return PAPOF_EINVAL;
@@ -457,9 +469,9 @@
         S1[k] = A.f64(n);
     }
     double* prep_tmp = A.f64(np0 * fc);
-    double* gx = A.f64(np0 * C);
-    double* gy = A.f64(np0 * C);
-    double* gxy = A.f64(np0 * C);
+    double* gx = warp_direct ? nullptr : A.f64(np0 * C);
+    double* gy = warp_direct ? nullptr : A.f64(np0 * C);
+    double* gxy = warp_direct ? nullptr : A.f64(np0 * C);
     double* warp = A.f64(np0 * fc);
     double* u = A.f64(2 * np0);
     double* v = u ? u + np0 : nullptr;
@@ -534,6 +546,7 @@
             pclk.phase(-1);
             if (overlap) PAPOF_HIP(hipEventRecord(h->sync_events[k], prep));
         }
+        if (warp_direct) return PAPOF_OK;
         pclk.phase(PAPOF_T_POSTPROCESSING);
         PAPOF_TRY(central3_planes(h, L[0].p2, gx, gy, gxy, H, W, C));
         pclk.phase(-1);
@@ -583,6 +596,7 @@
             pclk.phase(-1);
             PAPOF_HIP(hipEventRecord(h->sync_events[k], prep));
         }
+        if (warp_direct) return PAPOF_OK;
         pclk.phase(PAPOF_T_POSTPROCESSING);
         PAPOF_TRY(central3_planes(h, L[0].p2, gx, gy, gxy, H, W, C));
         pclk.phase(-1);
@@ -613,6 +627,8 @@
             const int lw = L[k].w, lh = L[k].h;
             const size_t np = (size_t)lw * lh;
             clk.phase(-1);
+            const bool zero_start = k == levels - 1 && !init;
+            if (zero_start) PAPOF_HIP(hipMemsetAsync(u, 0, 2 * np * sizeof(double), h->stream));
             if (overlap) PAPOF_HIP(hipStreamWaitEvent(main_stream, h->sync_events[k], 0));
             clk.phase(PAPOF_T_ALLOCATION);
             const double *f1 = F1[k], *f2 = F2[k];
@@ -639,7 +655,6 @@
             } else if (k == levels - 1) {
                 v = u + np;
                 v2 = u2 + np;
-                PAPOF_HIP(hipMemsetAsync(u, 0, 2 * np * sizeof(double), h->stream));
                 if (!fold_warp)
                     PAPOF_HIP(hipMemcpyAsync(warp, f2, np * fc * sizeof(double), hipMemcpyDeviceToDevice, h->stream));
                 if (B.bgx) PAPOF_TRY(bicubic_planes(h, f2, lh, lw, fc, B));
@@ -664,8 +679,12 @@
             ph = lh;
         }
         clk.phase(-1);
-        if (overlap) PAPOF_HIP(hipStreamWaitEvent(main_stream, h->sync_events[levels], 0));
+        if (overlap && !warp_direct) PAPOF_HIP(hipStreamWaitEvent(main_stream, h->sync_events[levels], 0));
         clk.phase(PAPOF_T_POSTPROCESSING);
+        const auto final_warp = [&](const Rect* rc) -> int {
+            return warp_direct ? bicubic_warp_direct(h, L[0].p1, L[0].p2, u, v, d_warp, H, W, C, rc)
+                               : bicubic_warp(h, L[0].p1, L[0].p2, gx, gy, gxy, u, v, d_warp, H, W, C, rc);
+        };
         if (hostio && io.early_out && u == d_vx && v == d_vy) {
             hipStream_t const cs = h->copy_stream;
             PAPOF_HIP(hipEventRecord(h->copy_events[2], main_stream));
@@ -676,7 +695,7 @@
             for (int q = 0; q < kChunks; q++) {
                 const Rect rc{0, (int)((long long)H * q / kChunks), W, (int)((long long)H * (q + 1) / kChunks)};
                 if (rc.empty()) continue;
-                PAPOF_TRY(bicubic_warp(h, L[0].p1, L[0].p2, gx, gy, gxy, u, v, d_warp, H, W, C, &rc));
+                PAPOF_TRY(final_warp(&rc));
                 PAPOF_HIP(hipEventRecord(h->copy_events[3 + q], main_stream));
                 PAPOF_HIP(hipStreamWaitEvent(cs, h->copy_events[3 + q], 0));
                 const size_t off = (size_t)rc.y0 * W * C, cnt = (size_t)rc.h() * W * C;
@@ -685,7 +704,7 @@
             io.out_issued = true;
             return PAPOF_OK;
         }
-        PAPOF_TRY(bicubic_warp(h, L[0].p1, L[0].p2, gx, gy, gxy, u, v, d_warp, H, W, C));
+        PAPOF_TRY(final_warp(nullptr));
         if (u != d_vx) PAPOF_HIP(hipMemcpyAsync(d_vx, u, np0 * sizeof(double), hipMemcpyDeviceToDevice, h->stream));
         if (v != d_vy) PAPOF_HIP(hipMemcpyAsync(d_vy, v, np0 * sizeof(double), hipMemcpyDeviceToDevice, h->stream));
         return PAPOF_OK;
@@ -1035,7 +1054,7 @@
     double ratio = P.ratio;
     if (ratio > 0.98 || ratio < 0.4) ratio = 0.75;
     if (levels < 1) return kSeqPrime;
-    const size_t need = arena_bytes_for(H, W, C, levels, P.n_sor + (levels - 1) * P.n_sor_per_level, P.ratio);
+    const size_t need = arena_bytes_for(H, W, C, levels, P.n_sor + (levels - 1) * P.n_sor_per_level, P.ratio, !warp_direct_on());
     return seq_matches(h, H, W, C, levels, ratio, need) ? kSeqNext : kSeqPrime;
 }
 
diff --git a/papteam_opticalflow_amd/csrc/common.h b/papteam_opticalflow_amd/csrc/common.h
--- a/papteam_opticalflow_amd/csrc/common.h
+++ b/papteam_opticalflow_amd/csrc/common.h
@@ -193,6 +193,7 @@
     int sor_resident = 0;
     int sor_skip_dead = 1;
     unsigned* sor_prog_next = nullptr;
+    bool sor_dudv_clear_next = false;
     int sor_launches = 0;
     struct SorSolveLog {
         int H, W, n_sor, kind, depth, launches;
@@ -297,7 +298,8 @@
 int flow_system(papof_handle* h, const double* im1, const double* im2, const double* u, const double* v, const double* im1s,
                 int H, int W, int planes, double alpha, double omega, const SorPlanes& out, unsigned* wit = nullptr,
                 int row0 = 0, int row1 = -1,
-                int batch = 1, const BatchK* bk = nullptr);
+                int batch = 1, const BatchK* bk = nullptr,
+                void* clear = nullptr, size_t clear_n16 = 0);
 int lap_scratch_doubles();
 int lap_rows_check(papof_handle* h, const double* im1, const double* im2, const double* u, const double* v, int H, int W,
                    int C, int r0, int r1, unsigned* wit, unsigned* val, unsigned mark);
@@ -315,6 +317,8 @@
 int bicubic_warp(papof_handle* h, const double* im1, const double* im2, const double* gx, const double* gy,
                  const double* gxy, const double* vx, const double* vy, double* out_hwc, int H, int W, int C,
                  const Rect* rc = nullptr, bool planar_out = false, bool clamp = true, int batch = 1, const BatchK* bk = nullptr);
+int bicubic_warp_direct(papof_handle* h, const double* im1, const double* im2, const double* vx, const double* vy,
+                        double* out_hwc, int H, int W, int C, const Rect* rc = nullptr);
 int flow_quantize16(papof_handle* h, const double* vx, const double* vy, unsigned short* q, size_t n);
 int flow_dequantize16(papof_handle* h, const unsigned short* q, double* vx, double* vy, size_t n);
 int flow_to_bgr(papof_handle* h, const double* vx, const double* vy, size_t n, double* partial, unsigned char* bgr);
diff --git a/papteam_opticalflow_amd/csrc/flow_internal.h b/papteam_opticalflow_amd/csrc/flow_internal.h
--- a/papteam_opticalflow_amd/csrc/flow_internal.h
+++ b/papteam_opticalflow_amd/csrc/flow_internal.h
@@ -102,7 +102,8 @@
 };
 
 
-size_t arena_bytes_for(int H, int W, int C, int levels, int n_sor_max, double ratio);
+size_t arena_bytes_for(int H, int W, int C, int levels, int n_sor_max, double ratio,
+                       bool warp_planes = true);
 int ensure_arena(papof_handle* h, size_t bytes);
 int check_params(const papof_params& P, int levels);
 int pyramid_plan(int H, int W, double ratio, int nlev, std::vector<Level>& L, std::vector<PyrPlan>& plan);
diff --git a/papteam_opticalflow_amd/csrc/kernels.hip b/papteam_opticalflow_amd/csrc/kernels.hip
--- a/papteam_opticalflow_amd/csrc/kernels.hip
+++ b/papteam_opticalflow_amd/csrc/kernels.hip
@@ -360,6 +360,14 @@
     }
 }
 
+__device__ __forceinline__ double central3_acc(double lo, double mid, double hi, const Taps& c3) {
+    double acc = 0.0;
+    acc += lo * c3.t[0];
+    acc += mid * c3.t[1];
+    acc += hi * c3.t[2];
+    return acc;
+}
+
 __global__ void k_central3_all(const double* __restrict__ src, double* __restrict__ gx, double* __restrict__ gy,
                                double* __restrict__ gxy, int H, int W, Taps c3) {
     int tbx, tby;
@@ -368,19 +376,15 @@
     if (j >= W || i >= H) return;
     const size_t np = (size_t)H * W;
     const double* p = src + blockIdx.z * np;
+    const int jl = clampi(j - 1, W), jr = clampi(j + 1, W);
     const auto hrow = [&](int ii) {
         const double* row = p + (size_t)ii * W;
-        double acc = 0.0;
-#pragma unroll
-        for (int l = -1; l <= 1; l++) acc += row[clampi(j + l, W)] * c3.t[l + 1];
-        return acc;
+        return central3_acc(row[jl], row[j], row[jr], c3);
     };
-    const double hx[3] = {hrow(clampi(i - 1, H)), hrow(i), hrow(clampi(i + 1, H))};
-    double vy = 0.0, vxy = 0.0;
-#pragma unroll
-    for (int l = -1; l <= 1; l++) vy += p[(size_t)clampi(i + l, H) * W + j] * c3.t[l + 1];
-#pragma unroll
-    for (int l = -1; l <= 1; l++) vxy += hx[l + 1] * c3.t[l + 1];
+    const int iu = clampi(i - 1, H), id = clampi(i + 1, H);
+    const double hx[3] = {hrow(iu), hrow(i), hrow(id)};
+    const double vy = central3_acc(p[(size_t)iu * W + j], p[(size_t)i * W + j], p[(size_t)id * W + j], c3);
+    const double vxy = central3_acc(hx[0], hx[1], hx[2], c3);
     const size_t o = blockIdx.z * np + (size_t)i * W + j;
     gx[o] = hx[1];
     gy[o] = vy;
@@ -930,13 +934,23 @@
 struct SixPlanes {
     double* q[6];
 };
+#ifndef PAPOF_CLEAR_AT_END
+#define PAPOF_CLEAR_AT_END 0
+#endif
+__device__ __forceinline__ void clear_slice(uint4* __restrict__ p, unsigned n16, unsigned nblocks) {
+    const unsigned lines = (n16 + 7u) >> 3, per = (lines + nblocks - 1) / nblocks;
+    const unsigned lo = min(blockIdx.x * per * 8u, n16), hi = min(lo + per * 8u, n16);
+    for (unsigned c = lo + threadIdx.x; c < hi; c += kFT * kFT) p[c] = uint4{0u, 0u, 0u, 0u};
+}
 template <int PLANES, bool SKEW, bool BATCH = false>
 __global__ __launch_bounds__(256, 1) void k_flow_system(const double* __restrict__ im1, const double* __restrict__ im2,
                                                      const double* __restrict__ u, const double* __restrict__ v,
                                                      const double* __restrict__ im1s, int H, int W, double alpha,
                                                      double omega, SkewIdx sk, SixPlanes out, Taps g, Taps d,
                                                      unsigned long long* stamp, unsigned* __restrict__ wit, double wit_thr,
-                                                     unsigned mark, int row0, int row1, BatchK bk) {
+                                                     unsigned mark, int row0, int row1, BatchK bk,
+                                                     uint4* __restrict__ clr, unsigned clr_n16) {
+    constexpr bool kClear = SKEW && !BATCH;
     if (BATCH) {
         const size_t p = blockIdx.y;
         im1s += batch_frames(bk, p, im1, im2);
@@ -956,7 +970,9 @@
     stamp_now(stamp);
     const int ntx = (W + kFT - 1) / kFT, ntiles = ntx * ((row1 - row0 + kFT - 1) / kFT), per = (ntiles + 7) >> 3;
     const int vt = (int)(blockIdx.x & 7u) * per + (int)(blockIdx.x >> 3);
-    if ((int)(blockIdx.x >> 3) >= per || vt >= ntiles) return;
+    const bool padding = (int)(blockIdx.x >> 3) >= per || vt >= ntiles;
+    if (kClear && clr != nullptr && (padding || !PAPOF_CLEAR_AT_END)) clear_slice(clr, clr_n16, 8u * per);
+    if (padding) return;
     const int tby = vt / ntx, tbx = vt - tby * ntx;
     const int ib = row0 + tby * kFT, j0 = tbx * kFT, tid = threadIdx.x;
     const size_t np = (size_t)H * W;
@@ -1201,17 +1217,18 @@
     double2s* const pc = reinterpret_cast<double2s*>(out.q[4]);
     __syncthreads();
     const int grp = tid / kFT, jj = tid - grp * kFT, j = j0 + jj;
-    if (j >= W) return;
-    for (int pp = grp; pp <= 2 * kFT - 2; pp += kFT) {
-        const int r = pp - jj;
-        if (r < 0 || r >= kFT) continue;
-        const int i = ib + r;
-        if (i >= row1) continue;
-        const size_t q = skew_cell(i, j, sk);
-        pa[q] = double2s{stage[0][r][jj], stage[1][r][jj]};
-        pb[q] = double2s{stage[2][r][jj], stage[3][r][jj]};
-        pc[q] = double2s{stage[4][r][jj], stage[5][r][jj]};
-    }
+    if (j < W)
+        for (int pp = grp; pp <= 2 * kFT - 2; pp += kFT) {
+            const int r = pp - jj;
+            if (r < 0 || r >= kFT) continue;
+            const int i = ib + r;
+            if (i >= row1) continue;
+            const size_t q = skew_cell(i, j, sk);
+            pa[q] = double2s{stage[0][r][jj], stage[1][r][jj]};
+            pb[q] = double2s{stage[2][r][jj], stage[3][r][jj]};
+            pc[q] = double2s{stage[4][r][jj], stage[5][r][jj]};
+        }
+    if (kClear && PAPOF_CLEAR_AT_END && clr != nullptr) clear_slice(clr, clr_n16, 8u * per);
 }
 
 template <bool SKEW>
@@ -1369,6 +1386,35 @@
     if (do_warp) warp_pixel(im1, im2, warp, fu, fv, i, j, H, W, planes);
 }
 
+__device__ __forceinline__ double bicubic_hermite(double fA, double fB, double fC, double fD, double xA, double xB, double xC,
+                                                  double xD, double yA, double yB, double yC, double yD, double zA, double zB,
+                                                  double zC, double zD, double dx, double dy, double dx2, double dy2,
+                                                  double dx3, double dy3) {
+    const double c00 = fA;
+    const double c10 = xA;
+    const double c20 = -3 * fA + 3 * fB - 2 * xA - xB;
+    const double c30 = 2 * fA - 2 * fB + xA + xB;
+    const double c01 = yA;
+    const double c11 = zA;
+    const double c21 = -3 * yA + 3 * yB - 2 * zA - zB;
+    const double c31 = 2 * yA - 2 * yB + zA + zB;
+    const double c02 = -3 * fA + 3 * fC - 2 * yA - yC;
+    const double c12 = -3 * xA + 3 * xC - 2 * zA - zC;
+    const double c22 = 9 * fA - 9 * fB - 9 * fC + 9 * fD + 6 * xA + 3 * xB - 6 * xC - 3 * xD + 6 * yA - 6 * yB +
+                       3 * yC - 3 * yD + 4 * zA + 2 * zB + 2 * zC + zD;
+    const double c32 = -6 * fA + 6 * fB + 6 * fC - 6 * fD - 3 * xA - 3 * xB + 3 * xC + 3 * xD - 4 * yA + 4 * yB -
+                       2 * yC + 2 * yD - 2 * zA - 2 * zB - zC - zD;
+    const double c03 = 2 * fA - 2 * fC + yA + yC;
+    const double c13 = 2 * xA - 2 * xC + zA + zC;
+    const double c23 = -6 * fA + 6 * fB + 6 * fC - 6 * fD - 4 * xA - 2 * xB + 4 * xC + 2 * xD - 3 * yA + 3 * yB -
+                       3 * yC + 3 * yD - 2 * zA - zB - 2 * zC - zD;
+    const double c33 = 4 * fA - 4 * fB - 4 * fC + 4 * fD + 2 * xA + 2 * xB - 2 * xC - 2 * xD + 2 * yA - 2 * yB +
+                       2 * yC - 2 * yD + zA + zB + zC + zD;
+    return c00 + c01 * dy + c02 * dy2 + c03 * dy3 + c10 * dx + c11 * dx * dy + c12 * dx * dy2 +
+           c13 * dx * dy3 + c20 * dx2 + c21 * dx2 * dy + c22 * dx2 * dy2 + c23 * dx2 * dy3 + c30 * dx3 +
+           c31 * dx3 * dy + c32 * dx3 * dy2 + c33 * dx3 * dy3;
+}
+
 template <bool BATCH>
 __global__ void k_bicubic(const double* __restrict__ im1, const double* __restrict__ im2,
                           const double* __restrict__ gx, const double* __restrict__ gy,
@@ -1422,34 +1468,74 @@
         const double xA = px[a], xB = px[b], xC = px[c], xD = px[d];
         const double yA = py[a], yB = py[b], yC = py[c], yD = py[d];
         const double zA = pz[a], zB = pz[b], zC = pz[c], zD = pz[d];
-        const double c00 = fA;
-        const double c10 = xA;
-        const double c20 = -3 * fA + 3 * fB - 2 * xA - xB;
-        const double c30 = 2 * fA - 2 * fB + xA + xB;
-        const double c01 = yA;
-        const double c11 = zA;
-        const double c21 = -3 * yA + 3 * yB - 2 * zA - zB;
-        const double c31 = 2 * yA - 2 * yB + zA + zB;
-        const double c02 = -3 * fA + 3 * fC - 2 * yA - yC;
-        const double c12 = -3 * xA + 3 * xC - 2 * zA - zC;
-        const double c22 = 9 * fA - 9 * fB - 9 * fC + 9 * fD + 6 * xA + 3 * xB - 6 * xC - 3 * xD + 6 * yA - 6 * yB +
-                           3 * yC - 3 * yD + 4 * zA + 2 * zB + 2 * zC + zD;
-        const double c32 = -6 * fA + 6 * fB + 6 * fC - 6 * fD - 3 * xA - 3 * xB + 3 * xC + 3 * xD - 4 * yA + 4 * yB -
-                           2 * yC + 2 * yD - 2 * zA - 2 * zB - zC - zD;
-        const double c03 = 2 * fA - 2 * fC + yA + yC;
-        const double c13 = 2 * xA - 2 * xC + zA + zC;
-        const double c23 = -6 * fA + 6 * fB + 6 * fC - 6 * fD - 4 * xA - 2 * xB + 4 * xC + 2 * xD - 3 * yA + 3 * yB -
-                           3 * yC + 3 * yD - 2 * zA - zB - 2 * zC - zD;
-        const double c33 = 4 * fA - 4 * fB - 4 * fC + 4 * fD + 2 * xA + 2 * xB - 2 * xC - 2 * xD + 2 * yA - 2 * yB +
-                           2 * yC - 2 * yD + zA + zB + zC + zD;
-        double r = c00 + c01 * dy + c02 * dy2 + c03 * dy3 + c10 * dx + c11 * dx * dy + c12 * dx * dy2 +
-                   c13 * dx * dy3 + c20 * dx2 + c21 * dx2 * dy + c22 * dx2 * dy2 + c23 * dx2 * dy3 + c30 * dx3 +
-                   c31 * dx3 * dy + c32 * dx3 * dy2 + c33 * dx3 * dy3;
+        double r = bicubic_hermite(fA, fB, fC, fD, xA, xB, xC, xD, yA, yB, yC, yD, zA, zB, zC, zD, dx, dy, dx2, dy2, dx3, dy3);
         if (clamp) {
             r = r < 0 ? 0.0 : r;
             r = r > 1 ? 1.0 : r;
         }
         out[obase + k * ostride] = r;
+    }
+}
+
+__global__ void k_bicubic_direct(const double* __restrict__ im1, const double* __restrict__ im2,
+                                 const double* __restrict__ vx, const double* __restrict__ vy, double* __restrict__ out,
+                                 int H, int W, int C, Rect rc, unsigned long long* stamp, Taps c3) {
+    stamp_now(stamp);
+    int tbx, tby;
+    if (!xcd_tile((rc.x1 - rc.x0 + BX - 1) / BX, (rc.y1 - rc.y0 + BY - 1) / BY, tbx, tby)) return;
+    const int j = rc.x0 + tbx * BX + threadIdx.x, i = rc.y0 + tby * BY + threadIdx.y;
+    if (j >= rc.x1 || i >= rc.y1) return;
+    const size_t np = (size_t)H * W, o = (size_t)i * W + j, obase = o * C;
+    const double x = j + vx[o];
+    const double y = i + vy[o];
+    if (x < 0 || x > W - 1 || y < 0 || y > H - 1) {
+        for (int k = 0; k < C; k++) {
+            double r = im1[k * np + o];
+            r = r < 0 ? 0.0 : r;
+            r = r > 1 ? 1.0 : r;
+            out[obase + k] = r;
+        }
+        return;
+    }
+    int x0 = (int)x, y0 = (int)y;
+    int x1 = x0 + 1, y1 = y0 + 1;
+    x0 = clampi(x0, W);
+    x1 = clampi(x1, W);
+    y0 = clampi(y0, H);
+    y1 = clampi(y1, H);
+    const double dx = x - x0, dy = y - y0;
+    const double dx2 = dx * dx, dy2 = dy * dy;
+    const double dx3 = dx * dx2, dy3 = dy * dy2;
+    const int col[4] = {clampi(x0 - 1, W), x0, x1, clampi(x1 + 1, W)};
+    const size_t row[4] = {(size_t)clampi(y0 - 1, H) * W, (size_t)y0 * W, (size_t)y1 * W, (size_t)clampi(y1 + 1, H) * W};
+    const bool xs = x1 != x0, ys = y1 != y0;
+    for (int k = 0; k < C; k++) {
+        const double* f = im2 + k * np;
+        double t[4][4];
+#pragma unroll
+        for (int r = 0; r < 4; r++)
+#pragma unroll
+            for (int c = 0; c < 4; c++) t[r][c] = f[row[r] + col[c]];
+        double h0[4], h1[4];
+#pragma unroll
+        for (int r = 0; r < 4; r++) {
+            h0[r] = central3_acc(t[r][0], t[r][1], t[r][2], c3);
+            h1[r] = central3_acc(xs ? t[r][1] : t[r][0], t[r][2], t[r][3], c3);
+        }
+        const double fA = t[1][1], fB = t[1][2], fC = t[2][1], fD = t[2][2];
+        const double xA = h0[1], xB = h1[1], xC = h0[2], xD = h1[2];
+        const double yA = central3_acc(t[0][1], t[1][1], t[2][1], c3);
+        const double yB = central3_acc(t[0][2], t[1][2], t[2][2], c3);
+        const double yC = central3_acc(ys ? t[1][1] : t[0][1], t[2][1], t[3][1], c3);
+        const double yD = central3_acc(ys ? t[1][2] : t[0][2], t[2][2], t[3][2], c3);
+        const double zA = central3_acc(h0[0], h0[1], h0[2], c3);
+        const double zB = central3_acc(h1[0], h1[1], h1[2], c3);
+        const double zC = central3_acc(ys ? h0[1] : h0[0], h0[2], h0[3], c3);
+        const double zD = central3_acc(ys ? h1[1] : h1[0], h1[2], h1[3], c3);
+        double r = bicubic_hermite(fA, fB, fC, fD, xA, xB, xC, xD, yA, yB, yC, yD, zA, zB, zC, zD, dx, dy, dx2, dy2, dx3, dy3);
+        r = r < 0 ? 0.0 : r;
+        r = r > 1 ? 1.0 : r;
+        out[obase + k] = r;
     }
 }
 
@@ -1823,8 +1909,9 @@
 
 int flow_system(papof_handle* h, const double* im1, const double* im2, const double* u, const double* v, const double* im1s,
                 int H, int W, int planes, double alpha, double omega, const SorPlanes& out, unsigned* wit, int row0, int row1,
-                int batch, const BatchK* bk) {
+                int batch, const BatchK* bk, void* clear, size_t clear_n16) {
     if (planes != 5 && planes != 3) return PAPOF_EINVAL;
+    if (clear && clear_n16 && (!out.skew || batch > 1 || ((uintptr_t)clear & 15) || clear_n16 >= (size_t(1) << 28))) return PAPOF_EINVAL;
     if (row1 < 0) row1 = H;
     if (row0 < 0 || row1 > H) return PAPOF_EINVAL;
     if (row1 <= row0) return PAPOF_OK;
@@ -1838,7 +1925,8 @@
                                             : (planes == 5 ? k_flow_system<5, false> : k_flow_system<3, false>));
     hipLaunchKernelGGL(kern, grid, dim3(kFT * kFT), 0, h->stream, im1, im2, u, v, im1s, H, W, alpha, omega,
                        out.skew ? skew_idx(out) : SkewIdx{0, 0, 0, 0, 0, 0, 0, 0, 0}, six, smooth5_taps(), deriv5_taps(),
-                       take_stamp(h), wit, 2e-20 * (double)H * (double)W, h->lap_epoch, row0, row1, bk ? *bk : bk0);
+                       take_stamp(h), wit, 2e-20 * (double)H * (double)W, h->lap_epoch, row0, row1, bk ? *bk : bk0,
+                       clear && clear_n16 ? (uint4*)clear : (uint4*)nullptr, (unsigned)clear_n16);
     LAUNCH_CHECK();
     return PAPOF_OK;
 }
@@ -1932,6 +2020,16 @@
     return PAPOF_OK;
 }
 
+int bicubic_warp_direct(papof_handle* h, const double* im1, const double* im2, const double* vx, const double* vy,
+                        double* out_hwc, int H, int W, int C, const Rect* rc) {
+    const Rect r = region(rc, W, H);
+    if (r.empty()) return PAPOF_OK;
+    hipLaunchKernelGGL(k_bicubic_direct, dim3(xcd_grid((r.x1 - r.x0 + BX - 1) / BX, (r.y1 - r.y0 + BY - 1) / BY)), dim3(BX, BY), 0,
+                       h->stream, im1, im2, vx, vy, out_hwc, H, W, C, r, take_stamp(h), central3_taps());
+    LAUNCH_CHECK();
+    return PAPOF_OK;
+}
+
 constexpr int kGmBlocks = 256, kGmThreads = 256, kGmMaxC = 8;
 static __global__ __launch_bounds__(kGmThreads) void k_gm_partial(const double* __restrict__ im1,
                                                            const double* __restrict__ im2, size_t np, int C,
diff --git a/papteam_opticalflow_amd/csrc/sor.hip b/papteam_opticalflow_amd/csrc/sor.hip
--- a/papteam_opticalflow_amd/csrc/sor.hip
+++ b/papteam_opticalflow_amd/csrc/sor.hip
@@ -1620,6 +1620,8 @@
     const double nalpha = -alpha, om1 = 1 - omega;
     if (n_sor <= 0) return PAPOF_EINVAL;
     const int batch = bt ? bt->n : 1;
+    const bool dudv_cleared = h->sor_dudv_clear_next;
+    h->sor_dudv_clear_next = false;
     if (batch < 1 || (bt && mode != PAPOF_SOR_EXACT)) return PAPOF_EINVAL;
     const auto mark = [&](int on) {
         if (h->sor_mark) h->sor_mark(h->sor_mark_ctx, on);
@@ -1699,7 +1701,7 @@
         if (std::getenv("PAPOF_SOR_INJECT_ABORT")) PAPOF_HIP(hipMemsetAsync(h->sync_words, 1, sizeof(unsigned), h->stream));
         if (bt) {
             PAPOF_TRY(fill_pairs(h, sp.du, bt->d * sizeof(double), sd.nd * 16, batch));
-        } else {
+        } else if (!dudv_cleared || sd.nd + sd.nh != sp.sd.nd + sp.sd.nh) {
             PAPOF_HIP(hipMemsetAsync(sp.du, 0, (sd.nd + sd.nh) * 16, h->stream));
         }
         mark(1);
```
